# marbl/Mash

Hardware: AMD Instinct MI355X
Metric: pairwise Mash distances/sec (s=1000) (higher is better)
Workload: dtype u64; 1 GPU; mash triangle all-vs-all, 100000 clustered synthetic sketches, k=21 s=1000, 4999950000 pairs/step, per-table job (index build + discover + fill + merge each step), row-block sharded x1; parallelism=rowblock1, rccl_ranks=0

## Files before the change

mash_amd/csrc/compare_dense.hip:

```cpp
#ifdef MG_HIP_EMU
#include "hipemu.h"
#else
#include <hip/hip_runtime.h>
#define MG_DYN_SHARED(T, name)                                   \
    extern __shared__ __align__(16) unsigned char name##_raw[]; \
    T *name = reinterpret_cast<T *>(name##_raw)
#endif
#include <stdint.h>

#include <cstdlib>

#ifndef MG_HIP_EMU
#include <rocprim/device/device_radix_sort.hpp>
#include <rocprim/device/device_select.hpp>
#include <rocprim/iterator/counting_iterator.hpp>
#endif

#include "compare_internal.h"

namespace mg {

#ifndef MG_HIP_EMU
__global__ __launch_bounds__(256) void dn_neighbor_kernel(const uint64_t *hashes, uint64_t stride, const uint32_t *cnt, uint32_t n,
                                                          uint8_t *link)
{
    const uint32_t row = blockIdx.x * 4u + (threadIdx.x >> 6), lane = threadIdx.x & 63u;
    if (row >= n) return;
    uint32_t hit = 0;
    uint32_t ci = 0, cj = 0;
    if (row > 0) {
        ci = cnt[row];
        cj = cnt[row - 1];
        const uint32_t take = ci < 64u ? ci : 64u, span = cj < 256u ? cj : 256u;
        if (lane < take && span > 0) {
            const uint64_t v = hashes[(uint64_t)row * stride + lane];
            const uint64_t *q = hashes + (uint64_t)(row - 1) * stride;
            uint32_t lo = 0, hi = span;
            while (lo < hi) {
                const uint32_t mid = (lo + hi) >> 1;
                if (q[mid] < v) lo = mid + 1; else hi = mid;
            }
            hit = (lo < span && q[lo] == v) ? 1u : 0u;
        }
    }
    const uint32_t hits = (uint32_t)__popcll(__ballot(hit != 0));
    const uint32_t take = ci < 64u ? ci : 64u;
    if (lane == 0) link[row] = (row > 0 && take >= 16u && cj >= 16u && 2u * hits >= take) ? 1 : 0;
}

hipError_t launch_dense_neighbors(const uint64_t *hashes, uint64_t stride, const uint32_t *cnt, uint32_t n, uint8_t *link,
                                  hipStream_t stream)
{
    if (n == 0) return hipSuccess;
    hipLaunchKernelGGL(dn_neighbor_kernel, dim3((n + 3u) / 4u), dim3(256), 0, stream, hashes, stride, cnt, n, link);
    return hipGetLastError();
}

constexpr uint32_t DN_SUBLISTS = 1024;

__global__ __launch_bounds__(256) void dn_leaders_kernel(const uint32_t *sorted_rows, const uint32_t *gs_of, const uint32_t *gend,
                                                         const uint32_t *grp_of, const DenseGroup *groups, uint32_t E,
                                                         unsigned long long *key, uint32_t *val, uint32_t cap_sub, uint32_t *cnt)
{
    const uint32_t pos = blockIdx.x * 256u + threadIdx.x;
    bool lead = false;
    uint32_t g = 0xFFFFFFFFu, gs = 0;
    if (pos < E) {
        g = grp_of[sorted_rows[pos]];
        if (g != 0xFFFFFFFFu) {
            const uint32_t g0 = groups[g].g0, g1 = groups[g].g1;
            gs = gs_of[pos];
            const bool first = pos == gs || sorted_rows[pos - 1] < g0;
            const bool more = pos + 1u < gend[gs] && sorted_rows[pos + 1] < g1;
            lead = first && more;
        }
    }
    const uint64_t bal = __ballot(lead);
    if (bal == 0) return;
    const uint32_t lane = threadIdx.x & 63u, sub = blockIdx.x & (DN_SUBLISTS - 1u);
    uint32_t base = 0;
    if (lane == (uint32_t)__builtin_ctzll(bal)) base = atomicAdd(&cnt[sub], (uint32_t)__popcll(bal));
    base = (uint32_t)__builtin_amdgcn_readlane((int)base, __builtin_ctzll(bal));
    if (lead) {
        const uint32_t k = base + (uint32_t)__popcll(bal & ((1ull << lane) - 1ull));
        if (k < cap_sub) {
            const uint64_t slot = (uint64_t)sub * cap_sub + k;
            key[slot] = ((unsigned long long)g << 32) | gs;
            val[slot] = pos;
        }
    }
}

__global__ __launch_bounds__(DN_SUBLISTS) void dn_sublists_scan_kernel(const uint32_t *cnt, uint32_t cap_sub, uint32_t *off, uint32_t *total)
{
    __shared__ uint32_t s_w[DN_SUBLISTS / 64];
    const uint32_t t = threadIdx.x, lane = t & 63u, wid = t >> 6;
    const uint32_t want = cnt[t], c = want < cap_sub ? want : cap_sub;
    uint32_t incl = c;
#pragma unroll
    for (int d = 1; d < 64; d <<= 1) {
        const uint32_t x = __shfl_up(incl, d);
        if (lane >= (uint32_t)d) incl += x;
    }
    if (lane == 63u) s_w[wid] = incl;
    __syncthreads();
    uint32_t base = 0;
    for (uint32_t k = 0; k < wid; k++) base += s_w[k];
    off[t] = base + incl - c;
    if (t == DN_SUBLISTS - 1u) total[0] = base + incl;
    atomicMax(&total[1], want);
}

__global__ __launch_bounds__(256) void dn_sublists_copy_kernel(const unsigned long long *key, const uint32_t *val, const uint32_t *cnt,
                                                               const uint32_t *off, uint32_t cap_sub, unsigned long long *key_out,
                                                               uint32_t *val_out)
{
    const uint32_t sub = blockIdx.x;
    const uint32_t c = cnt[sub] < cap_sub ? cnt[sub] : cap_sub, o = off[sub];
    for (uint32_t k = threadIdx.x; k < c; k += 256u) {
        key_out[o + k] = key[(uint64_t)sub * cap_sub + k];
        val_out[o + k] = val[(uint64_t)sub * cap_sub + k];
    }
}

__global__ __launch_bounds__(256) void dn_universe_split_kernel(const unsigned long long *key_sorted, uint32_t m, uint32_t *ulist,
                                                                uint32_t *ustart, uint32_t *uend)
{
    const uint32_t i = blockIdx.x * 256u + threadIdx.x;
    if (i >= m) return;
    const unsigned long long k = key_sorted[i];
    const uint32_t g = (uint32_t)(k >> 32);
    ulist[i] = (uint32_t)k;
    if (i == 0 || (uint32_t)(key_sorted[i - 1] >> 32) != g) ustart[g] = i;
    if (i + 1u == m || (uint32_t)(key_sorted[i + 1] >> 32) != g) uend[g] = i + 1u;
}

size_t dense_universe_temp_bytes(uint32_t cap)
{
    size_t b = 0;
    rocprim::radix_sort_pairs(nullptr, b, (const unsigned long long *)nullptr, (unsigned long long *)nullptr, (const uint32_t *)nullptr,
                              (uint32_t *)nullptr, (size_t)cap, 0u, 64u, (hipStream_t) nullptr);
    return b;
}

uint32_t dense_sublists() { return DN_SUBLISTS; }

hipError_t dense_find_leaders(const uint32_t *sorted_rows, const uint32_t *gs_of, const uint32_t *gend, const uint32_t *grp_of,
                              const DenseGroup *groups, uint32_t E, unsigned long long *key, uint32_t *val, uint32_t cap_sub,
                              unsigned long long *key_out, uint32_t *val_out, uint32_t *cnt, uint32_t *off, uint32_t *total,
                              hipStream_t stream)
{
    if (E == 0) return hipSuccess;
    hipError_t e = hipMemsetAsync(cnt, 0, DN_SUBLISTS * 4, stream);
    if (e == hipSuccess) e = hipMemsetAsync(total, 0, 8, stream);
    if (e != hipSuccess) return e;
    hipLaunchKernelGGL(dn_leaders_kernel, dim3((E + 255u) / 256u), dim3(256), 0, stream, sorted_rows, gs_of, gend, grp_of, groups, E, key, val, cap_sub,
                       cnt);
    e = hipGetLastError();
    if (e != hipSuccess) return e;
    return dense_join_leaders(key, val, cap_sub, key_out, val_out, cnt, off, total, stream);
}

hipError_t dense_join_leaders(const unsigned long long *key, const uint32_t *val, uint32_t cap_sub, unsigned long long *key_out, uint32_t *val_out,
                              const uint32_t *cnt, uint32_t *off, uint32_t *total, hipStream_t stream)
{
    hipLaunchKernelGGL(dn_sublists_scan_kernel, dim3(1), dim3(DN_SUBLISTS), 0, stream, cnt, cap_sub, off, total);
    hipLaunchKernelGGL(dn_sublists_copy_kernel, dim3(DN_SUBLISTS), dim3(256), 0, stream, key, val, cnt, (const uint32_t *)off, cap_sub, key_out, val_out);
    return hipGetLastError();
}

hipError_t dense_sort_universes(const unsigned long long *key, const uint32_t *val, uint32_t m, void *temp, size_t temp_bytes,
                                unsigned long long *key_sorted, uint32_t *ulist, uint32_t *upos, uint32_t *ustart, uint32_t *uend,
                                uint32_t group_bits, hipStream_t stream)
{
    if (m == 0) return hipSuccess;
    hipError_t e = rocprim::radix_sort_pairs(temp, temp_bytes, key, key_sorted, val, upos, (size_t)m, 0u, 32u + group_bits, stream);
    if (e != hipSuccess) return e;
    hipLaunchKernelGGL(dn_universe_split_kernel, dim3((m + 255u) / 256u), dim3(256), 0, stream, (const unsigned long long *)key_sorted, m, ulist,
                       ustart, uend);
    return hipGetLastError();
}

#endif

constexpr uint32_t DN_CX_MASK = 0x7FFFu, DN_CX_FLAG = 0x8000u;

template <uint32_t DN_EK>
__global__ __launch_bounds__(256) void dn_encode_kernel(const uint32_t *off, const uint32_t *code_img, uint32_t *pos_img, uint32_t rs,
                                                        const uint32_t *grp_of, const DenseGroup *groups, const uint32_t *ulist,
                                                        const uint32_t *upos, unsigned long long *gdata, uint32_t wstride, uint16_t *ext,
                                                        uint32_t xs, uint32_t n, uint32_t ul_in_lds)
{
    MG_DYN_SHARED(uint32_t, lds);
    const uint32_t bid = blockIdx.x;
    const uint32_t row = (bid & ~63u) | ((bid & 7u) << 3) | ((bid >> 3) & 7u);
    const uint32_t tid = threadIdx.x, lane = tid & 63u, wid = tid >> 6;
    if (row >= n) return;
    const uint32_t g = grp_of[row];
    if (g == 0xFFFFFFFFu) return;
    const DenseGroup G = groups[g];
    const uint32_t W = G.W, u = G.u;
    uint32_t *mask32 = lds, *hist = lds + 2u * W, *gap8 = hist + W + 1u, *ovf = gap8 + 16u * W, *pl32 = ovf + W, *scr = pl32 + 8u * W;
    uint32_t *ull = lds + 28u * wstride + 9u;
    for (uint32_t i = tid; i < 28u * W + 1u; i += 256u) lds[i] = 0;
    const uint32_t *ulg = ulist + G.ustart, *up = upos + G.ustart;
    if (ul_in_lds)
        for (uint32_t i = tid; i < u; i += 256u) ull[i] = ulg[i];
    const uint32_t *ul = ul_in_lds ? ull : ulg;
    __syncthreads();
    const uint32_t cnt = off[row + 1] - off[row];
    uint16_t *xrow = ext + (uint64_t)(G.xrow0 + (row - G.g0)) * xs;
    uint32_t nx = 0;
    if constexpr (DN_EK == 1) {
        for (uint32_t base = 0; base < cnt; base += 256u) {
            const uint32_t p = base + tid;
            uint32_t idx = 0;
            bool extra = false;
            if (p < cnt) {
                const uint64_t img = (uint64_t)row * rs + p;
                const uint32_t gs = code_img[img] >> 1;
                uint32_t lo = 0, hi = u;
                while (lo < hi) {
                    const uint32_t mid = (lo + hi) >> 1;
                    if (ul[mid] < gs) lo = mid + 1; else hi = mid;
                }
                idx = lo;
                if (lo < u && ul[lo] == gs) {
                    atomicOr(&mask32[idx >> 5], 1u << (idx & 31u));
                    pos_img[img] = up[idx];
                } else {
                    extra = true;
                }
            }
            const uint64_t bal = __ballot(extra);
            const uint32_t before = (uint32_t)__popcll(bal & ((1ull << lane) - 1ull));
            if (lane == 0) scr[wid] = (uint32_t)__popcll(bal);
            __syncthreads();
            uint32_t woff = 0;
            for (uint32_t k = 0; k < wid; k++) woff += scr[k];
            const uint32_t total = scr[0] + scr[1] + scr[2] + scr[3];
            if (extra) {
                xrow[nx + woff + before] = (uint16_t)idx;
                atomicAdd(&hist[idx >> 6], 1u);
                atomicAdd(&gap8[idx >> 2], 1u << (8u * (idx & 3u)));
            }
            nx += total;
            __syncthreads();
        }
    } else {
        for (uint32_t base = 0; base < cnt; base += 256u * DN_EK) {
            const uint32_t p0 = base + tid * DN_EK;
            const uint32_t nv = p0 < cnt ? (cnt - p0 < DN_EK ? cnt - p0 : DN_EK) : 0u;
            uint32_t xidx[DN_EK];
            uint32_t nxt = 0;
            if (nv) {
                const uint64_t img0 = (uint64_t)row * rs + p0;
                const uint4 c0 = *reinterpret_cast<const uint4 *>(code_img + img0), c1 = *reinterpret_cast<const uint4 *>(code_img + img0 + 4u);
                const uint32_t code[DN_EK] = {c0.x, c0.y, c0.z, c0.w, c1.x, c1.y, c1.z, c1.w};
                uint4 *pp = reinterpret_cast<uint4 *>(pos_img + img0);
                const uint4 q0 = pp[0], q1 = pp[1];
                uint32_t pv[DN_EK] = {q0.x, q0.y, q0.z, q0.w, q1.x, q1.y, q1.z, q1.w};
                uint32_t pos = 0;
                {
                    const uint32_t gs0 = code[0] >> 1;
                    uint32_t lo = 0, hi = u;
                    while (lo < hi) {
                        const uint32_t mid = (lo + hi) >> 1;
                        if (ul[mid] < gs0) lo = mid + 1; else hi = mid;
                    }
                    pos = lo;
                }
    #pragma unroll
                for (uint32_t e = 0; e < DN_EK; e++) {
                    if (e < nv) {
                        const uint32_t gs = code[e] >> 1;
                        {
                            uint32_t lo = pos, hi = pos, step = 1;
                            while (hi < u && ul[hi] < gs) {
                                lo = hi + 1u;
                                hi += step;
                                step <<= 1;
                            }
                            hi = hi < u ? hi : u;
                            while (lo < hi) {
                                const uint32_t mid = (lo + hi) >> 1;
                                if (ul[mid] < gs) lo = mid + 1u; else hi = mid;
                            }
                            pos = lo;
                        }
                        if (pos < u && ul[pos] == gs) {
                            atomicOr(&mask32[pos >> 5], 1u << (pos & 31u));
                            pv[e] = up[pos];
                        } else {
    #pragma unroll
                            for (uint32_t j = 0; j < DN_EK; j++)
                                if (j == nxt) xidx[j] = pos;
                            nxt++;
                        }
                    }
                }
                pp[0] = make_uint4(pv[0], pv[1], pv[2], pv[3]);
                pp[1] = make_uint4(pv[4], pv[5], pv[6], pv[7]);
            }
            uint32_t incl = nxt;
    #pragma unroll
            for (uint32_t d = 1; d < 64u; d <<= 1) {
                const uint32_t y = __shfl_up(incl, d);
                if (lane >= d) incl += y;
            }
            if (lane == 63u) scr[wid] = incl;
            __syncthreads();
            uint32_t woff = 0;
            for (uint32_t k = 0; k < wid; k++) woff += scr[k];
            const uint32_t total = scr[0] + scr[1] + scr[2] + scr[3];
            const uint32_t at0 = nx + woff + incl - nxt;
    #pragma unroll
            for (uint32_t j = 0; j < DN_EK; j++) {
                if (j < nxt) {
                    const uint32_t idx = xidx[j];
                    xrow[at0 + j] = (uint16_t)idx;
                    atomicAdd(&hist[idx >> 6], 1u);
                    atomicAdd(&gap8[idx >> 2], 1u << (8u * (idx & 3u)));
                }
            }
            nx += total;
            __syncthreads();
        }
    }
    __syncthreads();
    const uint32_t jb = (row - G.g0) >> 7, bl = (row - G.g0) & 127u;
    const uint64_t bw = dense_block_words(W);
    unsigned long long *blk = gdata + G.data_off + (uint64_t)jb * bw;
    uint16_t *cxp = reinterpret_cast<uint16_t *>(blk + 128ull * W), *totp = cxp + (W + 1u) * 128u;
    unsigned long long *xpl = blk + dense_block_planes(W);
    for (uint32_t i = tid; i < 16u * W; i += 256u) {
        const uint32_t four = gap8[i], w = i >> 4, q = i & 15u;
        uint32_t bits[4] = {0u, 0u, 0u, 0u}, over = 0;
#pragma unroll
        for (uint32_t e = 0; e < 4u; e++) {
            const uint32_t c = (four >> (8u * e)) & 255u;
            over |= c >= 16u ? 1u : 0u;
#pragma unroll
            for (uint32_t j = 0; j < 4u; j++) bits[j] |= ((c >> j) & 1u) << ((4u * q + e) & 31u);
        }
        if (over || (q == 0 && hist[w] >= 256u)) ovf[w] = 1u;
#pragma unroll
        for (uint32_t j = 0; j < 4u; j++)
            if (bits[j]) atomicOr(&pl32[2u * (4u * w + j) + (q >> 3)], bits[j]);
    }
    __syncthreads();
    for (uint32_t i = tid; i < 4u * W; i += 256u) xpl[i * 128u + bl] = (unsigned long long)pl32[2u * i] | ((unsigned long long)pl32[2u * i + 1u] << 32);
    if (tid == 0) {
        uint32_t run = 0, all = 0;
        for (uint32_t w = 0; w <= W; w++) {
            cxp[w * 128u + bl] = (uint16_t)(run | ((w > 0 && ovf[w - 1u]) ? DN_CX_FLAG : 0u));
            totp[w * 128u + bl] = (uint16_t)all;
            if (w < W) {
                run += hist[w];
                all += hist[w] + (uint32_t)__popc(mask32[2u * w]) + (uint32_t)__popc(mask32[2u * w + 1u]);
            }
        }
    }
    for (uint32_t w = tid; w < W; w += 256u)
        blk[w * 128u + bl] = (unsigned long long)mask32[2u * w] | ((unsigned long long)mask32[2u * w + 1u] << 32);
}

hipError_t launch_dense_encode(const uint32_t *off, const uint32_t *code_img, uint32_t *pos_img, uint32_t rs, const uint32_t *grp_of,
                               const DenseGroup *groups, const uint32_t *ulist, const uint32_t *upos, unsigned long long *gdata,
                               uint16_t *ext, uint32_t xs, uint32_t n, uint32_t wmax, hipStream_t stream, int ul_mode)
{
    if (n == 0) return hipSuccess;
    const size_t fixed = ((size_t)28 * wmax + 9) * 4, with_ul = fixed + (size_t)wmax * 64 * 4;
    const bool ul_in_lds = ul_mode == 0 ? false : ul_mode == 1 ? with_ul <= 150 * 1024 : with_ul <= 40 * 1024;
    const size_t smem = ul_in_lds ? with_ul : fixed;
    auto go = [&](auto kern) -> hipError_t {
        hipError_t e = hipFuncSetAttribute(reinterpret_cast<const void *>(kern), hipFuncAttributeMaxDynamicSharedMemorySize, (int)smem);
        if (e != hipSuccess) return e;
        hipLaunchKernelGGL(kern, dim3((n + 63u) & ~63u), dim3(256), smem, stream, off, code_img, pos_img, rs, grp_of, groups, ulist, upos, gdata, wmax, ext, xs,
                           n, ul_in_lds ? 1u : 0u);
        return hipGetLastError();
    };
    return rs >= 4096u ? go(dn_encode_kernel<8>) : go(dn_encode_kernel<1>);
}



__device__ __forceinline__ uint32_t dn_count_add(uint32_t x, uint32_t acc)
{
#ifdef MG_HIP_EMU
    return (uint32_t)__popc(x) + acc;
#else
    uint32_t d;
    asm("v_bcnt_u32_b32 %0, %1, %2" : "=v"(d) : "v"(x), "v"(acc));
    return d;
#endif
}

__device__ __forceinline__ uint32_t dn_low_bits(uint32_t x, uint32_t y)
{
#ifdef MG_HIP_EMU
    return x & ((1u << y) - 1u);
#else
    return __builtin_amdgcn_ubfe(x, 0u, y);
#endif
}

template <uint32_t NP>
__device__ __forceinline__ uint32_t dn_descend(uint32_t base, uint32_t s, uint32_t u1, uint32_t A0, uint32_t B0, uint32_t A1, uint32_t B1,
                                               uint32_t A2, uint32_t B2, uint32_t A3, uint32_t B3)
{
    uint32_t pos = 0;
#pragma unroll
    for (uint32_t bit = 16u; bit != 0u; bit >>= 1) {
        const uint32_t y = pos + bit;
        uint32_t c = dn_count_add(dn_low_bits(B0, y), dn_count_add(dn_low_bits(A0, y), dn_count_add(dn_low_bits(u1, y), base)));
        if (NP >= 1u) c += 2u * dn_count_add(dn_low_bits(B1, y), (uint32_t)__popc(dn_low_bits(A1, y)));
        if (NP >= 3u)
            c += 4u * dn_count_add(dn_low_bits(B2, y), (uint32_t)__popc(dn_low_bits(A2, y))) +
                 8u * dn_count_add(dn_low_bits(B3, y), (uint32_t)__popc(dn_low_bits(A3, y)));
        pos = c < s ? y : pos;
    }
    return pos;
}

__device__ __forceinline__ uint32_t dn_resolve(unsigned long long un, unsigned long long mab, uint32_t fprev, uint32_t s, uint32_t w, bool lists,
                                               const unsigned long long *xpa, const unsigned long long *xpb, const uint16_t *xa,
                                               const uint16_t *xb, uint32_t ca0, uint32_t na, uint32_t cb0, uint32_t nb)
{
    if (__ballot(lists) == 0) {
        const unsigned long long a0 = xpa[512u * w], a1 = xpa[512u * w + 128u], a2 = xpa[512u * w + 256u], a3 = xpa[512u * w + 384u];
        const unsigned long long b0 = xpb[512u * w], b1 = xpb[512u * w + 128u], b2 = xpb[512u * w + 256u], b3 = xpb[512u * w + 384u];
        const bool p1 = __ballot((a1 | b1) != 0ull) != 0, p23 = __ballot((a2 | a3 | b2 | b3) != 0ull) != 0;
        const uint32_t ulo = (uint32_t)un, uhi = (uint32_t)(un >> 32);
        uint32_t c31 = dn_count_add((uint32_t)b0, dn_count_add((uint32_t)a0, dn_count_add(ulo & 0x7FFFFFFFu, fprev)));
        if (p1 || p23) c31 += 2u * dn_count_add((uint32_t)b1, (uint32_t)__popc((uint32_t)a1));
        if (p23)
            c31 += 4u * dn_count_add((uint32_t)b2, (uint32_t)__popc((uint32_t)a2)) + 8u * dn_count_add((uint32_t)b3, (uint32_t)__popc((uint32_t)a3));
        const bool upper = c31 < s;
        const uint32_t base = upper ? c31 + (ulo >> 31) : fprev;
        const uint32_t u1 = (upper ? uhi : ulo) << 1;
        const uint32_t A0 = upper ? (uint32_t)(a0 >> 32) : (uint32_t)a0, B0 = upper ? (uint32_t)(b0 >> 32) : (uint32_t)b0;
        uint32_t pos;
        if (!p1 && !p23) {
            pos = dn_descend<0>(base, s, u1, A0, B0, 0, 0, 0, 0, 0, 0);
        } else {
            const uint32_t A1 = upper ? (uint32_t)(a1 >> 32) : (uint32_t)a1, B1 = upper ? (uint32_t)(b1 >> 32) : (uint32_t)b1;
            if (!p23) {
                pos = dn_descend<1>(base, s, u1, A0, B0, A1, B1, 0, 0, 0, 0);
            } else {
                const uint32_t A2 = upper ? (uint32_t)(a2 >> 32) : (uint32_t)a2, B2 = upper ? (uint32_t)(b2 >> 32) : (uint32_t)b2;
                const uint32_t A3 = upper ? (uint32_t)(a3 >> 32) : (uint32_t)a3, B3 = upper ? (uint32_t)(b3 >> 32) : (uint32_t)b3;
                pos = dn_descend<3>(base, s, u1, A0, B0, A1, B1, A2, B2, A3, B3);
            }
        }
        const uint32_t mlo = (uint32_t)mab, mhi = (uint32_t)(mab >> 32);
        return upper ? dn_count_add(dn_low_bits(mhi, pos), (uint32_t)__popc(mlo)) : (uint32_t)__popc(dn_low_bits(mlo, pos));
    }
    uint32_t lo = 0, hi = 63;
    const uint32_t wbase = w << 6;
    while (lo < hi) {
        const uint32_t mid = (lo + hi) >> 1;
        uint32_t c = fprev + (uint32_t)__popcll(un & ((1ull << mid) - 1ull));
        for (uint32_t k = 0; k < na; k++) c += ((uint32_t)xa[ca0 + k] - wbase <= mid) ? 1u : 0u;
        for (uint32_t k = 0; k < nb; k++) c += ((uint32_t)xb[cb0 + k] - wbase <= mid) ? 1u : 0u;
        if (c >= s) hi = mid; else lo = mid + 1u;
    }
    return (uint32_t)__popcll(mab & ((1ull << lo) - 1ull));
}

template <uint32_t DN_ROWS, uint32_t DN_IL>
__global__ __launch_bounds__(128) void dn_pairs_kernel(const DenseTile *tiles, const DenseGroup *groups, const unsigned long long *gdata,
                                                       uint32_t use_lists,
                                                       const uint16_t *ext, uint32_t xs, uint32_t s, uint32_t row_begin, uint32_t row_end,
                                                       uint64_t out_base, const uint32_t *inv, uint2 *out, DenseList list)
{
    MG_DYN_SHARED(unsigned long long, dl);
    const DenseTile T = tiles[blockIdx.x];
    const DenseGroup G = groups[T.group];
    const uint32_t W = G.W, tid = threadIdx.x;
    const uint64_t bw = dense_block_words(W);
    const unsigned long long *Bm = gdata + G.data_off + (uint64_t)T.cblk * bw;
    const uint16_t *Bcx = reinterpret_cast<const uint16_t *>(Bm + 128ull * W);
    const uint16_t *Btot = Bcx + (W + 1u) * 128u;
    unsigned long long *Am = dl;
    uint16_t *Acx = reinterpret_cast<uint16_t *>(Am + (uint64_t)DN_ROWS * W);
    uint16_t *Atot = Acx + (W + 1u) * DN_ROWS;
    const uint32_t ra = T.row0 - G.g0;
    const unsigned long long *asrc = gdata + G.data_off + (uint64_t)(ra >> 7) * bw;
    const uint32_t la0 = ra & 127u;
    for (uint32_t i = tid; i < W * DN_ROWS; i += 128u) Am[i] = asrc[(i / DN_ROWS) * 128u + la0 + (i % DN_ROWS)];
    {
        const uint16_t *acs = reinterpret_cast<const uint16_t *>(asrc + 128ull * W);
        for (uint32_t i = tid; i < 2u * (W + 1u) * DN_ROWS; i += 128u) Acx[i] = acs[(i / DN_ROWS) * 128u + la0 + (i % DN_ROWS)];
    }
    __syncthreads();
    constexpr uint32_t DN_NB = DN_ROWS / DN_IL;
    uint16_t *Amax = Atot + (W + 1u) * DN_ROWS;
    for (uint32_t i = tid; i < DN_NB * (W + 1u); i += 128u) {
        const uint32_t bt = i / (W + 1u), w = i - bt * (W + 1u);
        uint32_t m = 0;
        for (uint32_t k = 0; k < DN_IL; k++)
            if (T.row0 + bt * DN_IL + k < G.g1) {
                const uint32_t v = Atot[w * DN_ROWS + bt * DN_IL + k];
                m = v > m ? v : m;
            }
        Amax[i] = (uint16_t)m;
    }
    __syncthreads();
    const uint32_t b = G.g0 + T.cblk * 128u + tid;
    const uint32_t lb = b < G.g1 ? tid : G.g1 - 1u - (G.g0 + T.cblk * 128u);
    const uint16_t *xb = ext + (uint64_t)(G.xrow0 + (b < G.g1 ? b - G.g0 : 0u)) * xs;
    const unsigned long long *xpb = Bm + dense_block_planes(W) + lb;
    const uint32_t colrow = inv ? inv[G.g0 + T.cblk * 128u + lb] : G.g0 + T.cblk * 128u + lb;
    const uint64_t tri_col = (colrow ? (uint64_t)colrow * (colrow - 1u) / 2u : 0ull) - out_base;
    for (uint32_t ai = 0; ai < DN_ROWS; ai += DN_IL) {
        if (T.row0 + ai >= G.g1 || T.row0 + ai >= row_end) break;
        const uint16_t *amax = Amax + (ai / DN_IL) * (W + 1u);
        uint32_t common[DN_IL], nle[DN_IL];
#pragma unroll
        for (uint32_t k = 0; k < DN_IL; k++) common[k] = nle[k] = 0;
        unsigned long long mb_next = Bm[lb];
        uint32_t tb_next = Btot[128u + lb];
        uint32_t wi = 0;
        for (; wi < W; wi++) {
            if (__ballot((uint32_t)amax[wi + 1u] + tb_next > s) != 0) break;
            const unsigned long long mb = mb_next;
            if (wi + 1u < W) {
                mb_next = Bm[(wi + 1u) * 128u + lb];
                tb_next = Btot[(wi + 2u) * 128u + lb];
            }
            const uint32_t mlo = (uint32_t)mb, mhi = (uint32_t)(mb >> 32);
#pragma unroll
            for (uint32_t k = 0; k < DN_IL; k++) {
                const unsigned long long am = Am[wi * DN_ROWS + ai + k];
                common[k] = dn_count_add((uint32_t)am & mlo, dn_count_add((uint32_t)(am >> 32) & mhi, common[k]));
            }
        }
        const uint32_t nfast = wi;
        for (; wi < W; wi++) {
            const unsigned long long mb = mb_next;
            const int32_t tbs = (int32_t)tb_next - (int32_t)s;
            if (wi + 1u < W) {
                mb_next = Bm[(wi + 1u) * 128u + lb];
                tb_next = Btot[(wi + 2u) * 128u + lb];
            }
            const uint32_t mlo = (uint32_t)mb, mhi = (uint32_t)(mb >> 32);
            bool any = false;
#pragma unroll
            for (uint32_t k = 0; k < DN_IL; k++) {
                const unsigned long long am = Am[wi * DN_ROWS + ai + k];
                const uint32_t cnew = dn_count_add((uint32_t)am & mlo, dn_count_add((uint32_t)(am >> 32) & mhi, common[k]));
                const bool before = (int32_t)Atot[(wi + 1u) * DN_ROWS + ai + k] + tbs <= (int32_t)cnew;
                common[k] = before ? cnew : common[k];
                nle[k] += before ? 1u : 0u;
                any = any || before;
            }
            if (__ballot(any) == 0) break;
        }
#pragma unroll
        for (uint32_t k = 0; k < DN_IL; k++) {
            const uint32_t a = T.row0 + ai + k;
            const bool present = a < G.g1 && a < row_end && a >= row_begin && G.g0 + T.cblk * 128u < a;
            if (!present) continue;
            const bool valid = b < a;
            uint32_t denom = s;
            const uint32_t w = nfast + nle[k];
            const bool need = valid && w < W;
            if (__ballot(need) != 0) {
                const uint32_t wc = need ? w : 0u;
                const unsigned long long ma = Am[wc * DN_ROWS + ai + k], mb = Bm[wc * 128u + lb];
                const uint32_t ca0 = Acx[wc * DN_ROWS + ai + k] & DN_CX_MASK, ca1r = Acx[(wc + 1u) * DN_ROWS + ai + k];
                const uint32_t cb0 = Bcx[wc * 128u + lb] & DN_CX_MASK, cb1r = Bcx[(wc + 1u) * 128u + lb];
                const uint32_t fprev = (uint32_t)Atot[wc * DN_ROWS + ai + k] + (uint32_t)Btot[wc * 128u + lb] - common[k];
                const bool lists = need && (use_lists || ((ca1r | cb1r) & DN_CX_FLAG) != 0);
                const uint32_t add = dn_resolve(ma | mb, ma & mb, fprev, s, wc, lists, asrc + dense_block_planes(W) + la0 + ai + k, xpb,
                                               ext + (uint64_t)(G.xrow0 + (a - G.g0)) * xs, xb, ca0, need ? (ca1r & DN_CX_MASK) - ca0 : 0u, cb0,
                                               need ? (cb1r & DN_CX_MASK) - cb0 : 0u);
                if (need) common[k] += add;
            }
            if (!valid) continue;
            if (w >= W) {
                const uint32_t total = (uint32_t)Atot[W * DN_ROWS + ai + k] + (uint32_t)Btot[W * 128u + lb] - common[k];
                denom = total < s ? total : s;
            }
            if (list.rc) {
                const uint32_t ra = a - list.row_first;
                const uint32_t at = list.row_base[ra] + list.row_cnt[ra] - (a - b);
                list.rc[at] = make_uint2(a, b);
                list.counts[at] = make_uint2(common[k], denom);
            } else {
                const uint32_t arow = inv ? inv[a] : a;
                const uint64_t tri_a = (uint64_t)arow * (arow - 1u) / 2u - out_base;
                out[arow > colrow ? tri_a + colrow : tri_col + arow] = make_uint2(common[k], denom);
            }
        }
    }
}

uint32_t dense_max_words() { return 400; }

size_t dense_pairs_lds(uint32_t W, uint32_t rows) { return (size_t)rows * W * 8 + (size_t)(W + 1u) * rows * 4 + (size_t)(W + 1u) * 8 * 2 + 16; }

uint32_t dense_rows_per_tile(uint64_t wave_rows) { return wave_rows / 32u >= 16384u ? 32u : 8u; }

hipError_t launch_dense_pairs(const DenseTile *tiles, uint32_t ntiles, uint32_t rows_per_tile, const DenseGroup *groups,
                              const unsigned long long *gdata, bool use_lists, const uint16_t *ext, uint32_t xs,
                              uint32_t s, uint32_t wmax, uint32_t row_begin, uint32_t row_end, uint64_t out_base, const uint32_t *inv, uint2 *out,
                              hipStream_t stream, const DenseList *list)
{
    if (ntiles == 0) return hipSuccess;
    const size_t smem = dense_pairs_lds(wmax, rows_per_tile);
    auto go = [&](auto kern) -> hipError_t {
        hipError_t e = hipFuncSetAttribute(reinterpret_cast<const void *>(kern), hipFuncAttributeMaxDynamicSharedMemorySize, (int)smem);
        if (e != hipSuccess) return e;
        hipLaunchKernelGGL(kern, dim3(ntiles), dim3(128), smem, stream, tiles, groups, gdata, use_lists ? 1u : 0u, ext, xs, s, row_begin, row_end,
                           out_base, inv, out, list ? *list : DenseList());
        return hipGetLastError();
    };
    const uint32_t il = 8;
    if (rows_per_tile == 32u) return il >= 16u ? go(dn_pairs_kernel<32, 16>) : il >= 8u ? go(dn_pairs_kernel<32, 8>) : go(dn_pairs_kernel<32, 4>);
    return il >= 8u ? go(dn_pairs_kernel<8, 8>) : go(dn_pairs_kernel<8, 4>);
}

#ifndef MG_HIP_EMU
constexpr uint32_t CL_FIRST = 4;

__global__ __launch_bounds__(256) void cl_emit_kernel(const uint64_t *hashes, uint64_t stride, const uint32_t *cnt, uint32_t n,
                                                      unsigned long long *key, uint32_t *row_out, uint32_t *label)
{
    const uint32_t i = blockIdx.x * 256u + threadIdx.x;
    if (i >= n * CL_FIRST) return;
    const uint32_t row = i / CL_FIRST, f = i % CL_FIRST;
    key[i] = f < cnt[row] ? (unsigned long long)hashes[(uint64_t)row * stride + f] : ~0ull;
    row_out[i] = row;
    if (f == 0) label[row] = row;
}

__global__ __launch_bounds__(256) void cl_minrow_kernel(const unsigned long long *key_sorted, const uint32_t *row_sorted, uint32_t m,
                                                        uint32_t *label)
{
    const uint32_t i = blockIdx.x * 256u + threadIdx.x;
    if (i >= m) return;
    const unsigned long long k = key_sorted[i];
    if (k == ~0ull) return;
    uint32_t lo = 0, hi = i;
    while (lo < hi) {
        const uint32_t mid = (lo + hi) >> 1;
        if (key_sorted[mid] < k) lo = mid + 1; else hi = mid;
    }
    atomicMin(&label[row_sorted[i]], row_sorted[lo]);
}

__global__ __launch_bounds__(256) void cl_jump_kernel(const uint32_t *in, uint32_t *out, uint32_t n)
{
    const uint32_t i = blockIdx.x * 256u + threadIdx.x;
    if (i < n) out[i] = in[in[i]];
}

__global__ __launch_bounds__(256) void cl_order_keys_kernel(const uint32_t *label, uint32_t n, uint32_t split, unsigned long long *key)
{
    const uint32_t i = blockIdx.x * 256u + threadIdx.x;
    if (i < n) key[i] = ((unsigned long long)(i >= split ? 1u : 0u) << 63) | ((unsigned long long)label[i] << 32) | i;
}

__global__ __launch_bounds__(256) void cl_split_keys_kernel(const unsigned long long *key_sorted, uint32_t n, uint32_t *inv, uint32_t *label_sorted)
{
    const uint32_t i = blockIdx.x * 256u + threadIdx.x;
    if (i < n) {
        inv[i] = (uint32_t)(key_sorted[i] & 0xFFFFFFFFull);
        label_sorted[i] = (uint32_t)(key_sorted[i] >> 32) & 0x7FFFFFFFu;
    }
}

size_t dense_cluster_temp_bytes(uint32_t n)
{
    size_t a = 0, b = 0;
    rocprim::radix_sort_pairs(nullptr, a, (const unsigned long long *)nullptr, (unsigned long long *)nullptr, (const uint32_t *)nullptr,
                              (uint32_t *)nullptr, (size_t)n * CL_FIRST, 0u, 64u, (hipStream_t) nullptr);
    rocprim::radix_sort_keys(nullptr, b, (const unsigned long long *)nullptr, (unsigned long long *)nullptr, (size_t)n, 0u, 64u,
                             (hipStream_t) nullptr);
    return a > b ? a : b;
}

hipError_t dense_cluster_rows(const uint64_t *hashes, uint64_t stride, const uint32_t *cnt, uint32_t n, void *temp, size_t temp_bytes,
                              unsigned long long *key_a, unsigned long long *key_b, uint32_t *row_a, uint32_t *row_b, uint32_t *lab_a,
                              uint32_t *lab_b, uint32_t *inv, uint32_t *label_sorted, hipStream_t stream, uint32_t split)
{
    if (n == 0) return hipSuccess;
    const uint32_t m = n * CL_FIRST;
    hipLaunchKernelGGL(cl_emit_kernel, dim3((m + 255u) / 256u), dim3(256), 0, stream, hashes, stride, cnt, n, key_a, row_a, lab_a);
    hipError_t e = hipGetLastError();
    if (e != hipSuccess) return e;
    e = rocprim::radix_sort_pairs(temp, temp_bytes, (const unsigned long long *)key_a, key_b, (const uint32_t *)row_a, row_b, (size_t)m, 0u, 64u,
                                  stream);
    if (e != hipSuccess) return e;
    hipLaunchKernelGGL(cl_minrow_kernel, dim3((m + 255u) / 256u), dim3(256), 0, stream, (const unsigned long long *)key_b, (const uint32_t *)row_b, m,
                       lab_a);
    hipLaunchKernelGGL(cl_jump_kernel, dim3((n + 255u) / 256u), dim3(256), 0, stream, (const uint32_t *)lab_a, lab_b, n);
    hipLaunchKernelGGL(cl_jump_kernel, dim3((n + 255u) / 256u), dim3(256), 0, stream, (const uint32_t *)lab_b, lab_a, n);
    hipLaunchKernelGGL(cl_order_keys_kernel, dim3((n + 255u) / 256u), dim3(256), 0, stream, (const uint32_t *)lab_a, n, split, key_a);
    e = hipGetLastError();
    if (e != hipSuccess) return e;
    e = rocprim::radix_sort_keys(temp, temp_bytes, (const unsigned long long *)key_a, key_b, (size_t)n, 0u, 64u, stream);
    if (e != hipSuccess) return e;
    hipLaunchKernelGGL(cl_split_keys_kernel, dim3((n + 255u) / 256u), dim3(256), 0, stream, (const unsigned long long *)key_b, n, inv, label_sorted);
    return hipGetLastError();
}

__global__ __launch_bounds__(256) void cl_gather_rows_kernel(const uint64_t *hashes, uint64_t stride, const uint32_t *inv, uint64_t *out)
{
    const uint32_t a = blockIdx.x;
    const uint64_t *src = hashes + (uint64_t)inv[a] * stride;
    uint64_t *dst = out + (uint64_t)a * stride;
    for (uint64_t p = threadIdx.x; p < stride; p += 256u) dst[p] = src[p];
}

hipError_t launch_dense_gather_rows(const uint64_t *hashes, uint64_t stride, const uint32_t *inv, uint32_t n, uint64_t *out, hipStream_t stream)
{
    if (n == 0) return hipSuccess;
    hipLaunchKernelGGL(cl_gather_rows_kernel, dim3(n), dim3(256), 0, stream, hashes, stride, inv, out);
    return hipGetLastError();
}

#endif

__global__ __launch_bounds__(256) void dn_group_rows_kernel(const DenseGroup *groups, uint32_t ng, uint32_t n, uint32_t *grp_of, uint4 *lead_rows)
{
    const uint32_t r = blockIdx.x * 256u + threadIdx.x;
    if (r >= n) return;
    uint32_t lo = 0, hi = ng;
    while (lo < hi) {
        const uint32_t mid = (lo + hi) >> 1;
        if (groups[mid].g0 <= r) lo = mid + 1u;
        else hi = mid;
    }
    uint32_t g = 0xFFFFFFFFu, g0 = 0, g1 = 0;
    if (lo > 0 && r < groups[lo - 1u].g1) {
        g = lo - 1u;
        g0 = groups[g].g0;
        g1 = groups[g].g1;
    }
    grp_of[r] = g;
    lead_rows[r] = make_uint4(g, g0, g1, 0u);
}

hipError_t launch_dense_group_rows(const DenseGroup *groups, uint32_t ng, uint32_t n, uint32_t *grp_of, uint32_t *lead_rows, hipStream_t stream)
{
    if (n == 0) return hipSuccess;
    hipLaunchKernelGGL(dn_group_rows_kernel, dim3((n + 255u) / 256u), dim3(256), 0, stream, groups, ng, n, grp_of, reinterpret_cast<uint4 *>(lead_rows));
    return hipGetLastError();
}

}
```

mash_amd/csrc/host_index.cpp:

```cpp
#include "host_internal.h"
#include "index_build.h"
#ifdef IX_PHASE_CLOCKS
namespace mg { void index_dump_clocks(); }
#endif
#include "sort_bits.h"

namespace {

const uint64_t kTilesLongestRun = 6144;
static const uint64_t kSplitMinRun = 128;

uint64_t longest_label_run(const uint32_t *lab_sorted, uint64_t n)
{
    if (!lab_sorted || n == 0) return 0;
    uint64_t run = 1, longest = 1;
    for (uint64_t a = 1; a < n; a++) {
        run = lab_sorted[a] == lab_sorted[a - 1] ? run + 1 : 1;
        longest = std::max(longest, run);
    }
    return longest;
}

struct Carve {
    unsigned char *base = nullptr;
    size_t at = 0;
    template <class T> T *take(size_t count)
    {
        const size_t from = (at + alignof(T) - 1) & ~(alignof(T) - 1);
        at = from + count * sizeof(T);
        return base ? reinterpret_cast<T *>(base + from) : nullptr;
    }
};

struct LeaderLists {
    DevBuf<unsigned long long> key, keyj;
    DevBuf<uint32_t> val, valj, cnt_sub, off_sub, nlead;
    uint32_t lists = mg::dense_sublists(), cap = 0, tot[2] = {0, 0};
    explicit LeaderLists(mg_ctx *c) : key(c), keyj(c), val(c), valj(c), cnt_sub(c), off_sub(c), nlead(c) {}

    hipError_t alloc(uint32_t room)
    {
        key.free(); val.free(); keyj.free(); valj.free();
        const uint64_t all = (uint64_t)lists * room;
        if (!(nlead.p && cnt_sub.p && off_sub.p) && (nlead.alloc(2) != hipSuccess || cnt_sub.alloc(lists) != hipSuccess || off_sub.alloc(lists) != hipSuccess))
            return hipErrorOutOfMemory;
        if (key.alloc(all) != hipSuccess || val.alloc(all) != hipSuccess || keyj.alloc(all) != hipSuccess || valj.alloc(all) != hipSuccess) return hipErrorOutOfMemory;
        cap = room;
        return hipSuccess;
    }
    hipError_t reset(hipStream_t st) { const hipError_t e = hipMemsetAsync(cnt_sub, 0, lists * 4, st); return e != hipSuccess ? e : hipMemsetAsync(nlead, 0, 8, st); }
    hipError_t join(hipStream_t st)
    {
        const hipError_t e = mg::dense_join_leaders(key, val, cap, keyj, valj, cnt_sub, off_sub, nlead, st);
        return e != hipSuccess ? e : hipMemcpyAsync(tot, nlead, 8, hipMemcpyDeviceToHost, st);
    }
    mg::IxLeaders view(const uint32_t *lead_rows) const { return mg::IxLeaders{lead_rows, key, val, cnt_sub, cap, lists}; }
    bool overflowed() const { return tot[1] > cap; }
};

struct SparseIndexBuild {
    mg_ctx *ctx;
    const mg_table *t;
    const uint32_t s;
    const bool clustered;
    const uint32_t split;
    mg_table::Sparse *sp;
    const uint64_t n;
    const std::chrono::steady_clock::time_point t_begin = std::chrono::steady_clock::now();
    bool stop = false;

    bool need_classes = false, dedup = true, want_dense = true, try_cluster = false, try_links = false;
    DevBuf<uint8_t> dc_cls, d_link;
    DevBuf<unsigned long long> dc_last, d_dig, d_dig_sorted, k_a, k_b;
    DevBuf<uint32_t> d_cnt, d_rows_sorted, d_flags, d_nflag, r_a, r_b, l_a, l_b, d_inv, d_lab;
    DevBuf<unsigned char> d_tmp_dup, d_tmp_cl;
    std::vector<uint8_t> hc_cls, link;
    std::vector<uint64_t> hc_last;
    std::vector<uint32_t> hc_nh, inv_v, lab_v;
    const uint32_t *inv = nullptr, *lab_sorted = nullptr;
    uint32_t nflag = 0, gate_suspects = 0;
    size_t tb_dup = 0, tb_cl = 0;
    bool cluster_q = false, links_q = false;

    const char *ix_mode = nullptr;
    bool ix_verify = false, ix_tiles = true;
    std::vector<uint32_t> cnt_true, cnt_perm;
    uint32_t max_cnt = 0;
    uint64_t maxv = 0, E_all = 0;
    double dens[65] = {0};
    double dens0 = 0;
    std::vector<uint32_t> rep;
    const uint64_t *H = nullptr;
    const uint32_t *rowmap = nullptr;
    uint64_t label_run = 0;
    mg::IxPlan early_plan;
    DevBuf<unsigned char> d_lb;
    bool lb_made = false;
    DevBuf<unsigned char> d_tcnt;
    bool cnt_made = false;
    bool cnt_stale = false;

    std::vector<uint32_t> cls_of, cls_off, cls_rows, cls_first;

    uint32_t E = 0, end_bit = 0, sort_begin_bit = 0;
    std::vector<mg::DenseGroup> cand_groups;
    std::vector<uint32_t> grp_of_h;
    DevBuf<mg::DenseGroup> d_groups;
    DevBuf<uint32_t> d_grp_of, d_lead_rows;
    LeaderLists lead;
    bool lead_ready = false, cand_prepared = false;
    mg::IxPlan plan;
    size_t temp_bytes = 0;
    DevBuf<unsigned char> temp;
    DevBuf<uint32_t> gs_of;
    DevBuf<unsigned long long> key64_a, key64_b;
    struct Stat { unsigned long long shared; uint32_t max_group, groups, bad, tie_overflow; uint32_t ixf[4]; } h_stat = {0, 0, 0, 0, 0, {0, 0, 0, 0}};
    DevBuf<Stat> d_stat;
    DevBuf<unsigned char> d_slots;
    bool want_order = true;
    std::vector<uint32_t> short_cnt;

    bool built = false;
    uint64_t dn_xrows = 0, dn_words = 0;

    SparseIndexBuild(mg_ctx *c, const mg_table *tab, uint32_t sketch_size, bool clustered_variant, mg_table::Sparse *index, uint32_t split_row)
        : ctx(c), t(tab), s(sketch_size), clustered(clustered_variant), split(split_row), sp(index), n(tab->n), dc_cls(c), d_link(c), dc_last(c), d_dig(c), d_dig_sorted(c),
          k_a(c), k_b(c), d_cnt(c), d_rows_sorted(c), d_flags(c), d_nflag(c), r_a(c), r_b(c), l_a(c), l_b(c), d_inv(c), d_lab(c), d_tmp_dup(c), d_tmp_cl(c), d_lb(c), d_tcnt(c),
          d_groups(c), d_grp_of(c), d_lead_rows(c), lead(c), temp(c), gs_of(c), key64_a(c), key64_b(c), d_stat(c), d_slots(c)
    {}

    int unusable(const char *why) { sp->usable = false; sp->why = why; stop = true; return MG_OK; }


    bool counts_with_offsets()
    {
        const char *o = ctx_opt(ctx, "MASHGPU_IX_COUNTS");
        if ((o && strcmp(o, "tiles") == 0) || !mg::index_offsets_counts_fits(early_plan.g)) return false;
        if (d_tcnt.alloc(early_plan.cnt_bytes) != hipSuccess || d_stat.alloc(1) != hipSuccess ||
            hipMemsetAsync(d_stat, 0, sizeof(Stat), ctx->stream) != hipSuccess) {
            (void)hipGetLastError();
            d_tcnt.free();
            return false;
        }
        return cnt_made = true;
    }

    hipError_t counts_to_device()
    {
            if (!cnt_stale) return hipSuccess;
            cnt_stale = false;
            return hipMemcpyAsync(d_cnt, cnt_true.data(), n * 4, hipMemcpyHostToDevice, ctx->stream);
    }

    template <class T> bool take(T **p, size_t count)
    {
        void *q = nullptr;
        if (ctx_malloc(ctx, &q, std::max<size_t>(count, 1) * sizeof(T)) != hipSuccess) return false;
        *p = static_cast<T *>(q);
        return true;
    }

    void drop()
    {
            for (void **q : {(void **)&sp->off, (void **)&sp->keys_sorted, (void **)&sp->gend, (void **)&sp->sorted_rows, (void **)&sp->code_img,
                             (void **)&sp->pos_img, (void **)&sp->short_rows, (void **)&sp->short_cnt, (void **)&sp->counters, (void **)&sp->order,
                             (void **)&sp->rep, (void **)&sp->cls_of, (void **)&sp->cls_off, (void **)&sp->cls_rows, (void **)&sp->cls_first})
                if (*q) { ctx_free(ctx, *q); *q = nullptr; }
    }

    int no_memory() { (void)hipGetLastError(); drop(); return unusable("no device memory for the index"); }
    int lost(hipError_t e) { drop(); return fail(ctx, MG_ERR_HIP, std::string("compare (index build): ") + hipGetErrorString(e)); }

    void drop_dense()
    {
        for (void **q : {(void **)&sp->dgroups, (void **)&sp->grp_of, (void **)&sp->gdata, (void **)&sp->ext, (void **)&sp->ulist, (void **)&sp->upos})
            if (*q) { ctx_free(ctx, *q); *q = nullptr; }
        sp->dgroups_host.clear();
    }

    struct TileScratch {
        DevBuf<unsigned char> start, big, pk, tc;
        explicit TileScratch(mg_ctx *c) : start(c), big(c), pk(c), tc(c) {}
    };

    hipError_t tiles(const TileScratch &w, int stages)
    {
        const mg::IxLeaders lv = lead.view(d_lead_rows);
        return mg::index_build_mapped(plan, H, rowmap, sp->off, d_lb, d_tcnt, w.start, w.big, w.pk, w.tc, sp->keys_sorted, sp->sorted_rows, sp->gend, gs_of, sp->code_img,
                               sp->pos_img, d_slots, &d_stat.p->shared, &d_stat.p->max_group, &d_stat.p->groups, d_stat.p->ixf, lead_ready ? &lv : nullptr,
                               ctx->stream, stages);
    }
    hipError_t sort_buckets(const TileScratch &w)
    {
        hipError_t e = tiles(w, 2);
        if (e == hipSuccess && lead_ready) e = lead.join(ctx->stream);
        return e != hipSuccess ? e : hipMemcpyAsync(&h_stat, d_stat, sizeof(Stat), hipMemcpyDeviceToHost, ctx->stream);
    }
    hipError_t row_order()
    {
        return mg::launch_sparse_row_order(sp->off, sp->code_img, sp->gend, sp->rep, (uint32_t)n, sp->rs, temp, temp_bytes, key64_a, key64_b, sp->order, ctx->stream);
    }

    int scan_rows();
    int copy_rows();
    int order_rows();
    int find_copies();
    int lay_out();
    void prepare_candidates();
    hipError_t tile_passes();
    int build_by_tiles();
    int build_by_sort();
    int check_build();
    bool search_leaders();
    bool sort_universes(std::vector<uint32_t> &us, std::vector<uint32_t> &ue);
    bool choose_groups(const std::vector<uint32_t> &us, const std::vector<uint32_t> &ue);
    int encode_groups();
    int dense_groups();
    int run();
};

int SparseIndexBuild::scan_rows()
{
    need_classes = t->cls.size() != n;
    dedup = !ctx_opt(ctx, "MASHGPU_SPARSE_NO_DEDUP");
    want_dense = true;
    if (const char *v = ctx_opt(ctx, "MASHGPU_COMPARE_DENSE")) want_dense = atoi(v) != 0;
    try_cluster = clustered && n >= 16;
    try_links = !try_cluster && want_dense && n >= 8 && s <= 16384;
    tb_dup = mg::sparse_dup_temp_bytes((uint32_t)n);
    tb_cl = mg::dense_cluster_temp_bytes((uint32_t)n);
    if (d_cnt.alloc(n) != hipSuccess || (need_classes && (dc_cls.alloc(n) != hipSuccess || dc_last.alloc(n) != hipSuccess)) ||
        (dedup && (d_dig.alloc(n) != hipSuccess || d_dig_sorted.alloc(n) != hipSuccess || d_rows_sorted.alloc(n) != hipSuccess ||
                   d_flags.alloc(n) != hipSuccess || d_nflag.alloc(1) != hipSuccess || d_tmp_dup.alloc(std::max<size_t>(tb_dup, 16)) != hipSuccess))) {
        (void)hipGetLastError();
        return unusable("no device memory for the index");
    }
    {
        hipError_t e = hipSuccess;
        if (need_classes) {
            hc_cls.resize(n);
            hc_last.resize(n);
            hc_nh.resize(n);
            e = mg::launch_row_classes(t->hashes, t->nhash, n, t->s, dc_cls, dc_last, ctx->stream);
        }
        if (e == hipSuccess) e = mg::launch_sparse_row_counts(t->nhash, (uint32_t)n, (uint32_t)std::min<uint64_t>(t->s, s), d_cnt, ctx->stream);
        if (e == hipSuccess && dedup) {
            e = mg::launch_sparse_row_gate(t->hashes, t->s, d_cnt, (uint32_t)n, d_dig, ctx->stream);
            if (e == hipSuccess)
                e = mg::launch_sparse_dup_suspects(d_dig, d_cnt, (uint32_t)n, d_tmp_dup, tb_dup, d_dig_sorted, d_rows_sorted, d_flags, d_nflag, ctx->stream);
        }
        if (e == hipSuccess && try_cluster) {
            if (k_a.alloc(4 * n) == hipSuccess && k_b.alloc(4 * n) == hipSuccess && r_a.alloc(4 * n) == hipSuccess && r_b.alloc(4 * n) == hipSuccess &&
                l_a.alloc(n) == hipSuccess && l_b.alloc(n) == hipSuccess && d_inv.alloc(n) == hipSuccess && d_lab.alloc(n) == hipSuccess &&
                d_tmp_cl.alloc(std::max<size_t>(tb_cl, 16)) == hipSuccess) {
                e = mg::dense_cluster_rows(t->hashes, t->s, d_cnt, (uint32_t)n, d_tmp_cl, tb_cl, k_a, k_b, r_a, r_b, l_a, l_b, d_inv, d_lab, ctx->stream, split);
                cluster_q = true;
            } else {
                (void)hipGetLastError();
            }
        }
        if (e == hipSuccess && try_links) {
            if (d_link.alloc(n) == hipSuccess) {
                link.resize(n);
                e = mg::launch_dense_neighbors(t->hashes, t->s, d_cnt, (uint32_t)n, d_link, ctx->stream);
                links_q = true;
            } else {
                (void)hipGetLastError();
            }
        }
        unsigned long long *p_last = nullptr;
        uint32_t *p_nh = nullptr, *p_inv = nullptr, *p_lab = nullptr, *p_nflag = nullptr;
        uint8_t *p_cls = nullptr, *p_link = nullptr;
        auto carve = [&](unsigned char *block) {
            Carve c{block};
            p_last = c.take<unsigned long long>(n); p_nh = c.take<uint32_t>(n); p_inv = c.take<uint32_t>(n); p_lab = c.take<uint32_t>(n);
            p_nflag = c.take<uint32_t>(2); p_cls = c.take<uint8_t>(n); p_link = c.take<uint8_t>(n);
            return c.at + 64;
        };
        unsigned char *pin = static_cast<unsigned char *>(ctx_pinned(ctx, carve(nullptr)));
        if (pin) {
            carve(pin);
        } else {
            p_nflag = &nflag;
            if (cluster_q) { inv_v.resize(n); lab_v.resize(n); p_inv = inv_v.data(); p_lab = lab_v.data(); }
            p_nh = hc_nh.data(); p_cls = hc_cls.data(); p_last = reinterpret_cast<unsigned long long *>(hc_last.data()); p_link = link.data();
        }
        if (e == hipSuccess && need_classes) {
            e = hipMemcpyAsync(p_nh, t->nhash, n * 4, hipMemcpyDeviceToHost, ctx->stream);
            if (e == hipSuccess) e = hipMemcpyAsync(p_cls, dc_cls, n, hipMemcpyDeviceToHost, ctx->stream);
            if (e == hipSuccess) e = hipMemcpyAsync(p_last, dc_last, n * 8, hipMemcpyDeviceToHost, ctx->stream);
        }
        if (e == hipSuccess && dedup) e = hipMemcpyAsync(p_nflag, d_nflag, 4, hipMemcpyDeviceToHost, ctx->stream);
        if (e == hipSuccess && cluster_q) {
            e = hipMemcpyAsync(p_inv, d_inv, n * 4, hipMemcpyDeviceToHost, ctx->stream);
            if (e == hipSuccess) e = hipMemcpyAsync(p_lab, d_lab, n * 4, hipMemcpyDeviceToHost, ctx->stream);
        }
        if (e == hipSuccess && links_q) e = hipMemcpyAsync(p_link, d_link, n, hipMemcpyDeviceToHost, ctx->stream);
        const hipError_t es = hipStreamSynchronize(ctx->stream);
        if (e == hipSuccess) e = es;
        if (e == hipSuccess && pin) {
            if (need_classes) {
                memcpy(hc_nh.data(), p_nh, n * 4);
                memcpy(hc_cls.data(), p_cls, n);
                memcpy(hc_last.data(), p_last, n * 8);
            }
            if (dedup) nflag = *p_nflag;
            if (links_q) memcpy(link.data(), p_link, n);
        }
        if (cluster_q) { inv = p_inv; lab_sorted = p_lab; }
        if (e != hipSuccess) return fail(ctx, MG_ERR_HIP, std::string("compare (index: rows, copies, order): ") + hipGetErrorString(e));
    }
    gate_suspects = nflag;
    if (need_classes) {
        t->cls.swap(hc_cls);
        t->last.swap(hc_last);
        t->nh.swap(hc_nh);
    }
    if (!links_q) link.clear();
    return MG_OK;
}

int SparseIndexBuild::order_rows()
{
    ix_mode = ctx_opt(ctx, "MASHGPU_SPARSE_INDEX");
    ix_verify = ix_mode && strcmp(ix_mode, "verify") == 0;
    ix_tiles = !ix_mode || strcmp(ix_mode, "sort") != 0;
    cnt_true.assign(n, 0);
    for (uint64_t i = 0; i < n; i++) {
        const uint32_t c = (uint32_t)std::min<uint64_t>(std::min<uint64_t>(t->nh[i], t->s), s);
        cnt_true[i] = c;
        E_all += c;
        max_cnt = std::max(max_cnt, c);
        if (c) {
            const uint64_t last = t->last[i];
            if (last == MG_HASH_PAD) return unusable("a hash equals the padding value");
            maxv = std::max(maxv, last);
            const double d = (double)c / ((double)last + 1.0);
            dens[64 - __builtin_clzll(last | 1ull)] += d;
            dens0 += d;
        }
    }
    H = t->hashes;
    bool keep_table_order = false;
    const uint64_t run = cluster_q ? longest_label_run(lab_sorted, n) : 0;
    if (cluster_q && split != 0 && lab_sorted && !ctx_opt(ctx, "MASHGPU_SPLIT_ALWAYS") && run * (uint64_t)s < kSplitMinRun * 1000ull) {
        keep_table_order = true;
        lab_sorted = nullptr;
    }
    if (cluster_q) {
        bool identity = true;
        for (uint64_t a = 0; a < n && identity; a++) identity = inv[a] == a;
        if (!identity && !keep_table_order) {
            const char *fc = ctx_opt(ctx, "MASHGPU_COMPARE_ROWCOPY");
            const bool copy_now = fc && atoi(fc) != 0;
            void *pi = nullptr, *ph = nullptr;
            if (ctx_malloc(ctx, &pi, n * 4) != hipSuccess || (copy_now && ctx_malloc(ctx, &ph, std::max<uint64_t>(n * t->s, 1) * 8) != hipSuccess)) {
                (void)hipGetLastError();
                ctx_free(ctx, pi);
                lab_sorted = nullptr;
            } else {
                sp->inv = static_cast<uint32_t *>(pi);
                sp->phashes = static_cast<uint64_t *>(ph);
                HIP_TRY(ctx, hipMemcpyAsync(sp->inv, d_inv, n * 4, hipMemcpyDeviceToDevice, ctx->stream));
                if (ix_tiles && !(dedup && nflag) && E_all > 0 && E_all < (1ull << 31) && run <= kTilesLongestRun) {
                    early_plan = mg::index_plan((uint32_t)n, (uint32_t)E_all, s, sp->rs, t->s, maxv, dens0, ix_verify);
                    if (early_plan.ok && d_lb.alloc(early_plan.lb_bytes) == hipSuccess) {
                        if (copy_now) HIP_TRY(ctx, mg::index_gather_rows(early_plan, t->hashes, sp->inv, d_cnt, sp->phashes, d_lb, ctx->stream));
                        else if (counts_with_offsets()) HIP_TRY(ctx, mg::index_offsets_counts(early_plan, t->hashes, sp->inv, d_cnt, d_lb, d_tcnt, d_stat.p->ixf, ctx->stream));
                        else HIP_TRY(ctx, mg::index_window_offsets(early_plan, t->hashes, sp->inv, d_cnt, d_lb, ctx->stream));
                        lb_made = true;
                    } else {
                        (void)hipGetLastError();
                    }
                }
                if (copy_now) {
                    if (!lb_made) HIP_TRY(ctx, mg::launch_dense_gather_rows(t->hashes, t->s, sp->inv, (uint32_t)n, sp->phashes, ctx->stream));
                    H = sp->phashes;
                } else {
                    rowmap = sp->inv;
                }
                cnt_perm.resize(n);
                for (uint64_t a = 0; a < n; a++) cnt_perm[a] = cnt_true[inv[a]];
                cnt_true.swap(cnt_perm);
                cnt_stale = true;
            }
        }
    } else {
        lab_sorted = nullptr;
    }
    label_run = lab_sorted ? run : 0;
    if (want_dense && n >= 8 && s <= 16384 && lab_sorted) {
        link.assign(n, 0);
        for (uint64_t a = 1; a < n; a++) link[a] = (a != split && lab_sorted[a] == lab_sorted[a - 1] && cnt_true[a] && cnt_true[a - 1]) ? 1 : 0;
    } else if (cluster_q && want_dense && n >= 8 && s <= 16384 && d_link.alloc(n) == hipSuccess) {
        const int rc = copy_rows();
        if (rc != MG_OK || stop) return rc;
        link.resize(n);
        HIP_TRY(ctx, counts_to_device());
        HIP_TRY(ctx, mg::launch_dense_neighbors(H, t->s, d_cnt, (uint32_t)n, d_link, ctx->stream));
        HIP_TRY(ctx, hipMemcpyAsync(link.data(), d_link, n, hipMemcpyDeviceToHost, ctx->stream));
        HIP_TRY(ctx, hipStreamSynchronize(ctx->stream));
    } else if (!links_q) {
        (void)hipGetLastError();
        link.clear();
    }
    return MG_OK;
}

int SparseIndexBuild::copy_rows()
{
    if (!rowmap) return MG_OK;
    void *ph = nullptr;
    if (ctx_malloc(ctx, &ph, std::max<uint64_t>(n * t->s, 1) * 8) != hipSuccess) return no_memory();
    sp->phashes = static_cast<uint64_t *>(ph);
    HIP_TRY(ctx, mg::launch_dense_gather_rows(t->hashes, t->s, rowmap, (uint32_t)n, sp->phashes, ctx->stream));
    H = sp->phashes;
    rowmap = nullptr;
    return MG_OK;
}

int SparseIndexBuild::find_copies()
{
    if (dedup && nflag) {
        const int rc = copy_rows();
        if (rc != MG_OK || stop) return rc;
        HIP_TRY(ctx, counts_to_device());
        HIP_TRY(ctx, mg::launch_sparse_row_digest(H, t->s, d_cnt, (uint32_t)n, d_dig, ctx->stream));
        HIP_TRY(ctx, mg::launch_sparse_dup_suspects(d_dig, d_cnt, (uint32_t)n, d_tmp_dup, tb_dup, d_dig_sorted, d_rows_sorted, d_flags, d_nflag, ctx->stream));
        HIP_TRY(ctx, hipMemcpyAsync(&nflag, d_nflag, 4, hipMemcpyDeviceToHost, ctx->stream));
        HIP_TRY(ctx, hipStreamSynchronize(ctx->stream));
        if (nflag) {
            std::vector<uint32_t> rows_sorted(n), flags(n);
            HIP_TRY(ctx, hipMemcpyAsync(rows_sorted.data(), d_rows_sorted, n * 4, hipMemcpyDeviceToHost, ctx->stream));
            HIP_TRY(ctx, hipMemcpyAsync(flags.data(), d_flags, n * 4, hipMemcpyDeviceToHost, ctx->stream));
            HIP_TRY(ctx, hipStreamSynchronize(ctx->stream));
            std::vector<uint2> pairs;
            pairs.reserve(nflag);
            for (uint64_t k = 1, g0 = 0; k < n; k++) {
                if (flags[k]) pairs.push_back(make_uint2(rows_sorted[k], rows_sorted[g0]));
                else g0 = k;
            }
            DevBuf<uint2> d_pairs(ctx);
            DevBuf<uint32_t> d_eq(ctx);
            if (d_pairs.alloc(pairs.size()) != hipSuccess || d_eq.alloc(pairs.size()) != hipSuccess) { (void)hipGetLastError(); return unusable("no device memory for the index"); }
            std::vector<uint32_t> eq(pairs.size());
            HIP_TRY(ctx, hipMemcpyAsync(d_pairs, pairs.data(), pairs.size() * sizeof(uint2), hipMemcpyHostToDevice, ctx->stream));
            HIP_TRY(ctx, mg::launch_sparse_row_equal(H, t->s, d_cnt, d_pairs, (uint32_t)pairs.size(), d_eq, ctx->stream));
            HIP_TRY(ctx, hipMemcpyAsync(eq.data(), d_eq, pairs.size() * 4, hipMemcpyDeviceToHost, ctx->stream));
            HIP_TRY(ctx, hipStreamSynchronize(ctx->stream));
            for (size_t k = 0; k < pairs.size(); k++)
                if (eq[k]) {
                    if (rep.empty()) { rep.resize(n); for (uint64_t i = 0; i < n; i++) rep[i] = (uint32_t)i; }
                    rep[pairs[k].x] = pairs[k].y;
                    sp->copies++;
                }
        }
    }
    if (sp->copies) {
        cls_of.assign(n, 0xFFFFFFFFu);
        std::vector<uint32_t> size(n, 0);
        for (uint64_t i = 0; i < n; i++) size[rep[i]]++;
        uint32_t ncls = 0, tot = 0;
        for (uint64_t i = 0; i < n; i++)
            if (size[i] >= 2) { cls_of[i] = ncls++; cls_off.push_back(tot); tot += size[i]; }
        cls_off.push_back(tot);
        cls_rows.resize(tot);
        std::vector<uint32_t> fillp(cls_off.begin(), cls_off.end() - 1);
        for (uint64_t i = 0; i < n; i++) {
            const uint32_t k = cls_of[rep[i]];
            if (k != 0xFFFFFFFFu) cls_rows[fillp[k]++] = (uint32_t)i;
        }
        cls_first.resize(tot);
        for (uint32_t k = 0; k < ncls; k++) {
            const uint64_t m = cls_off[k + 1] - cls_off[k];
            sp->cls_pairs += m * (m - 1) / 2;
            for (uint32_t u = cls_off[k]; u < cls_off[k + 1]; u++) cls_first[u] = cls_off[k];
        }
        sp->cls_members = tot;
        if (ncls == 1 && tot == n && cnt_true[0] > 0) sp->one_class = (uint32_t)cnt_true[0];
        if (sp->one_class && ctx->aside_all_copies) ctx->aside_all_copies(sp->one_class);
    }
    return MG_OK;
}

int SparseIndexBuild::lay_out()
{
    uint64_t E64 = 0;
    sp->off_host.resize(n + 1);
    for (uint64_t i = 0; i < n; i++) {
        sp->off_host[i] = (uint32_t)E64;
        const uint64_t c = cnt_true[i];
        if (rep.empty() || rep[i] == i) E64 += c;
        if (E64 >= (1ull << 31)) return unusable("2^31 entries or more");
        if (c < s) sp->short_rows_host.push_back((uint32_t)i);
        if (c == 0) sp->has_empty = true;
    }
    sp->off_host[n] = (uint32_t)E64;
    if (E64 == 0) return unusable("no hashes");
    E = (uint32_t)E64;
    sp->E = E;
    end_bit = (uint32_t)(64 - __builtin_clzll(maxv | 1ull));
    sort_begin_bit = mg::sparse_sort_begin_bit(E, end_bit, ctx_opt(ctx, "MASHGPU_SPARSE_SORT_BITS"), ctx_opt(ctx, "MASHGPU_SPARSE_SORT_ALL_BITS") != nullptr);
    if (sort_begin_bit > 0 && !ctx_opt(ctx, "MASHGPU_SPARSE_SORT_BITS")) sort_begin_bit = mg::sort_begin_bit_from_density(dens, end_bit, sort_begin_bit);
    const bool tiles_hopeless = ix_tiles && !ix_verify && lab_sorted && !ctx_opt(ctx, "MASHGPU_SPARSE_INDEX") &&
                                label_run > kTilesLongestRun;
    if (ix_tiles && !tiles_hopeless) plan = mg::index_plan((uint32_t)n, E, s, sp->rs, t->s, maxv, dens0, ix_verify);
    else if (tiles_hopeless) plan.why = "a clade of more rows than a bucket's sort takes";
    if (lb_made && !(plan.ok && memcmp(&plan.g, &early_plan.g, sizeof plan.g) == 0)) lb_made = cnt_made = false;
    temp_bytes = std::max(std::max(mg::sparse_order_temp_bytes((uint32_t)n), mg::sparse_order_slice_temp_bytes((uint32_t)n)),
                          mg::sparse_offsets_temp_bytes((uint32_t)n));
    want_order = !ctx_opt(ctx, "MASHGPU_SPARSE_NO_ORDER");
    bool ok = temp.alloc(std::max<size_t>(temp_bytes, 16)) == hipSuccess && gs_of.alloc(E) == hipSuccess && (d_stat.p || d_stat.alloc(1) == hipSuccess) &&
              d_slots.alloc(std::max(mg::sparse_stat_scratch_bytes(), mg::index_stat_scratch_bytes())) == hipSuccess &&
              (!want_order || (key64_a.alloc(n) == hipSuccess && key64_b.alloc(n) == hipSuccess));
    ok = ok && take(&sp->off, n + 1) && take(&sp->keys_sorted, E) && take(&sp->gend, E) && take(&sp->sorted_rows, E) &&
         take(&sp->code_img, (size_t)n * sp->rs + 64) && take(&sp->pos_img, (size_t)n * sp->rs) && take(&sp->counters, 4) &&
         (!want_order || take(&sp->order, n));
    const size_t nshort = sp->short_rows_host.size();
    short_cnt.assign(nshort, 0);
    for (size_t k = 0; k < nshort; k++) short_cnt[k] = cnt_true[sp->short_rows_host[k]];
    if (ok && nshort) ok = take(&sp->short_rows, nshort) && take(&sp->short_cnt, nshort);
    if (ok && sp->copies)
        ok = take(&sp->rep, n) && take(&sp->cls_of, n) && take(&sp->cls_off, cls_off.size()) && take(&sp->cls_rows, cls_rows.size()) &&
             take(&sp->cls_first, cls_first.size());
    if (!ok) return no_memory();
    hipError_t e = hipSuccess;
    auto upload = [&](uint32_t *dst, const std::vector<uint32_t> &v) {
        if (e == hipSuccess && !v.empty()) e = hipMemcpyAsync(dst, v.data(), v.size() * 4, hipMemcpyHostToDevice, ctx->stream);
    };
    if (sp->copies) { upload(sp->rep, rep); upload(sp->cls_of, cls_of); upload(sp->cls_off, cls_off); upload(sp->cls_rows, cls_rows); upload(sp->cls_first, cls_first); }
    if (!rep.empty()) upload(sp->off, sp->off_host);
    else if (e == hipSuccess) e = mg::launch_sparse_offsets(d_cnt, cnt_stale ? sp->inv : nullptr, (uint32_t)n, temp, sp->off, ctx->stream);
    upload(sp->short_rows, sp->short_rows_host); upload(sp->short_cnt, short_cnt);
    return e == hipSuccess ? MG_OK : lost(e);
}

void SparseIndexBuild::prepare_candidates()
{
    if (cand_prepared) return;
    cand_prepared = true;
    if (link.empty() || sp->copies != 0) return;
    for (uint64_t i = 1; i < n;) {
        if (!link[i]) { i++; continue; }
        uint64_t j = i;
        while (j < n && link[j]) j++;
        if (j - (i - 1) >= 8) {
            mg::DenseGroup g{};
            g.g0 = (uint32_t)(i - 1); g.g1 = (uint32_t)j;
            cand_groups.push_back(g);
        }
        i = j + 1;
    }
    if (cand_groups.empty()) return;
    const uint32_t ng = (uint32_t)cand_groups.size();
    grp_of_h.assign(n, 0xFFFFFFFFu);
    for (uint32_t g = 0; g < ng; g++)
        for (uint32_t r = cand_groups[g].g0; r < cand_groups[g].g1; r++) grp_of_h[r] = g;
    uint32_t room = std::max<uint32_t>(E / 4u / lead.lists + 64u, 256u);
    if (const char *ev = ctx_opt(ctx, "MASHGPU_DENSE_LEAD_CAP")) room = std::max<uint32_t>((uint32_t)atoi(ev), 1u);
    if (d_groups.alloc(ng) == hipSuccess && d_grp_of.alloc(n) == hipSuccess && d_lead_rows.alloc(4 * n) == hipSuccess && lead.alloc(room) == hipSuccess &&
        hipMemcpyAsync(d_groups, cand_groups.data(), ng * sizeof(mg::DenseGroup), hipMemcpyHostToDevice, ctx->stream) == hipSuccess &&
        mg::launch_dense_group_rows(d_groups, ng, (uint32_t)n, d_grp_of, d_lead_rows, ctx->stream) == hipSuccess && lead.reset(ctx->stream) == hipSuccess) {
        lead_ready = true;
    } else {
        (void)hipGetLastError();
        cand_groups.clear();
    }
}

hipError_t SparseIndexBuild::tile_passes()
{
    TileScratch w(ctx);
    if (!((lb_made || d_lb.alloc(plan.lb_bytes) == hipSuccess) && (cnt_made || d_tcnt.alloc(plan.cnt_bytes) == hipSuccess) && w.start.alloc(plan.start_bytes) == hipSuccess &&
          w.big.alloc(plan.big_bytes) == hipSuccess && w.pk.alloc(plan.pk_bytes) == hipSuccess && w.tc.alloc(plan.tc_bytes) == hipSuccess)) {
        (void)hipGetLastError();
        return hipSuccess;
    }
    hipError_t e = cnt_made ? hipSuccess : hipMemsetAsync(d_stat, 0, sizeof(Stat), ctx->stream);
    if (e == hipSuccess) e = tiles(w, cnt_made ? 1 | 8 | 16 : lb_made ? 1 | 8 : 1);
    DevBuf<uint32_t> d_swapped(ctx);
    if (e == hipSuccess && ctx_opt(ctx, "MASHGPU_IX_DEBUG_SWAP") && d_swapped.alloc(1) == hipSuccess) {
        e = hipMemsetAsync(d_swapped, 0, 4, ctx->stream);
        if (e == hipSuccess) e = mg::index_debug_swap(plan, w.pk, w.start, d_swapped, ctx->stream);
    }
    if (e == hipSuccess) prepare_candidates();
    if (e == hipSuccess && ctx->aside_at_sort) ctx->aside_at_sort();
    if (e == hipSuccess) e = sort_buckets(w);
    hipEvent_t ev_stats = nullptr;
    if (e == hipSuccess) e = hipEventCreateWithFlags(&ev_stats, hipEventDisableTiming);
    if (e == hipSuccess) e = hipEventRecord(ev_stats, ctx->stream);
    if (e == hipSuccess) e = tiles(w, 4);
    if (e == hipSuccess && want_order) e = row_order();
    const hipError_t ew = e == hipSuccess ? hipEventSynchronize(ev_stats) : hipStreamSynchronize(ctx->stream);
    if (e == hipSuccess) e = ew;
    if (ev_stats) (void)hipEventDestroy(ev_stats);
    built = e == hipSuccess && !h_stat.ixf[mg::IXF_DEGENERATE];
    if (built && lead_ready && lead.overflowed() && h_stat.ixf[mg::IXF_NBIG] == 0) {
        e = hipStreamSynchronize(ctx->stream);
        const uint32_t want_cap = lead.tot[1];
        if (e == hipSuccess && lead.alloc(want_cap) == hipSuccess) {
            e = lead.reset(ctx->stream);
            if (e == hipSuccess) e = hipMemsetAsync(d_stat.p, 0, offsetof(Stat, bad), ctx->stream);
            if (e == hipSuccess) e = sort_buckets(w);
            if (e == hipSuccess) e = hipStreamSynchronize(ctx->stream);
            built = e == hipSuccess && !h_stat.ixf[mg::IXF_DEGENERATE];
            if (ctx_opt(ctx, "MASHGPU_SPARSE_DBG"))
                fprintf(stderr, "compare dense: a list of leaders asked for %u entries: found again with that room (%u leaders)\n", want_cap, lead.tot[0]);
        } else {
            (void)hipGetLastError();
        }
    }
    if (ctx_opt(ctx, "MASHGPU_SPARSE_DBG"))
        fprintf(stderr, "compare sparse: index by tiles: shift %u, %u buckets (%u per window, %u windows), fullest %u, %u beyond the LDS (%u values streamed)%s\n",
                plan.g.shift, plan.g.Bp, plan.g.BW, plan.g.NW, h_stat.ixf[mg::IXF_MAXBUCKET], h_stat.ixf[mg::IXF_NBIG], h_stat.ixf[mg::IXF_NSTREAMED],
                h_stat.ixf[mg::IXF_DEGENERATE] ? " -- clumped values: sorted instead" : "");
    if (ctx_opt(ctx, "MASHGPU_SPARSE_DBG"))
        fprintf(stderr, "compare sparse: block counts %s\n", cnt_made ? "made with the window offsets (one read of the table)" : "by the tiles (K1)");
    return e;
}

int SparseIndexBuild::build_by_tiles()
{
    hipError_t e = hipSuccess;
    if (plan.ok) e = tile_passes();
    else if (ix_tiles && ctx_opt(ctx, "MASHGPU_SPARSE_DBG")) fprintf(stderr, "compare sparse: index by tiles refused: %s\n", plan.why);
    if (e != hipSuccess) return lost(e);
    sp->by_tiles = built;
    prepare_candidates();
#ifdef IX_PHASE_CLOCKS
    if (built && ctx_opt(ctx, "MASHGPU_IX_CLOCKS")) mg::index_dump_clocks();
#endif
    if (ix_verify && !built && !ctx_opt(ctx, "MASHGPU_SPARSE_INDEX_MAY_REFUSE"))
        return fail(ctx, MG_ERR_INVALID, std::string("index verify: the tile build refused this table (") + (plan.ok ? "bucket flags" : plan.why) + ")");
    return MG_OK;
}

int SparseIndexBuild::build_by_sort()
{
    if (built && !ix_verify) return MG_OK;
    const size_t sort_bytes = mg::sparse_sort_temp_bytes(E, end_bit, sort_begin_bit);
    DevBuf<unsigned char> temp_sort(ctx), d_ties(ctx);
    DevBuf<uint64_t> keys_a(ctx), v_keys(ctx);
    DevBuf<uint32_t> idx_a(ctx), idx_sorted(ctx), v_rows(ctx), v_gend(ctx), v_gs(ctx), v_code(ctx), v_pos(ctx);
    DevBuf<unsigned long long> d_diff(ctx);
    bool ok = temp_sort.alloc(std::max<size_t>(sort_bytes, 16)) == hipSuccess && keys_a.alloc(E) == hipSuccess && idx_a.alloc(E) == hipSuccess &&
              idx_sorted.alloc(E) == hipSuccess && d_ties.alloc(mg::sparse_tie_scratch_bytes()) == hipSuccess;
    if (ok && built)
        ok = v_keys.alloc(E) == hipSuccess && v_rows.alloc(E) == hipSuccess && v_gend.alloc(E) == hipSuccess && v_gs.alloc(E) == hipSuccess &&
             v_code.alloc((size_t)n * sp->rs + 64) == hipSuccess && v_pos.alloc((size_t)n * sp->rs) == hipSuccess && d_diff.alloc(16) == hipSuccess;
    if (!ok) return no_memory();
    const Stat tiles_stat = h_stat;
    uint64_t *o_keys = built ? v_keys.p : sp->keys_sorted;
    uint32_t *o_rows = built ? v_rows.p : sp->sorted_rows, *o_gend = built ? v_gend.p : sp->gend, *o_gs = built ? v_gs.p : gs_of.p,
             *o_code = built ? v_code.p : sp->code_img, *o_pos = built ? v_pos.p : sp->pos_img;
    hipError_t e = hipSuccess;
    for (uint32_t begin_bit = sort_begin_bit;; begin_bit = 0) {
        e = hipMemsetAsync(d_stat, 0, sizeof(Stat), ctx->stream);
        if (e == hipSuccess)
            e = mg::sparse_build_index(H, t->s, sp->off, (uint32_t)n, E, sp->rs, end_bit, temp_sort, sort_bytes, keys_a, idx_a, o_keys, idx_sorted,
                                       idx_a, o_gs, o_rows, o_gend, o_code, o_pos, d_slots, begin_bit, d_ties, &d_stat.p->shared,
                                       &d_stat.p->max_group, &d_stat.p->groups, &d_stat.p->bad, &d_stat.p->tie_overflow, ctx->stream, rowmap);
        if (e == hipSuccess && !built && want_order) e = row_order();
        if (e == hipSuccess) e = hipMemcpyAsync(&h_stat, d_stat, sizeof(Stat), hipMemcpyDeviceToHost, ctx->stream);
        if (e == hipSuccess) e = hipStreamSynchronize(ctx->stream);
        if (e != hipSuccess) return lost(e);
        if ((!h_stat.tie_overflow && !h_stat.bad) || begin_bit == 0) break;
        if (ctx_opt(ctx, "MASHGPU_SPARSE_DBG"))
            fprintf(stderr, "compare sparse: sort on bits [%u, %u) %s: every bit again\n", begin_bit, end_bit,
                    h_stat.bad ? "left values out of order" : "left ties the repair could not take");
    }
    if (!built) return MG_OK;
    unsigned long long diff[16];
    for (int k = 0; k < 8; k++) { diff[2 * k] = 0; diff[2 * k + 1] = ~0ull; }
    e = hipMemcpyAsync(d_diff, diff, sizeof diff, hipMemcpyHostToDevice, ctx->stream);
    const uint64_t img = (uint64_t)n * sp->rs;
    const struct { const char *name; const uint32_t *tiles, *sort, *ref; uint32_t mode; uint64_t words; } arrays[6] = {
        {"values (32-bit words)", (const uint32_t *)sp->keys_sorted, (const uint32_t *)v_keys.p, nullptr, 0, 2ull * E}, {"rows", sp->sorted_rows, v_rows, nullptr, 0, E},
        {"group starts", gs_of, v_gs, nullptr, 0, E}, {"group ends", sp->gend, v_gend, v_gs, 1, E}, {"code image", sp->code_img, v_code, nullptr, 0, img},
        {"position image", sp->pos_img, v_pos, v_code, 2, img}};
    for (int k = 0; k < 6 && e == hipSuccess; k++)
        e = mg::index_verify_words(arrays[k].tiles, arrays[k].sort, arrays[k].ref, arrays[k].mode, arrays[k].words, d_diff.p + 2 * k, ctx->stream);
    if (e == hipSuccess) e = hipMemcpyAsync(diff, d_diff, sizeof diff, hipMemcpyDeviceToHost, ctx->stream);
    if (e == hipSuccess) e = hipStreamSynchronize(ctx->stream);
    if (e != hipSuccess) return lost(e);
    std::string msg;
    for (int k = 0; k < 6; k++)
        if (diff[2 * k]) msg += std::string(msg.empty() ? "" : "; ") + arrays[k].name + ": " + std::to_string(diff[2 * k]) + " differ, first at " + std::to_string(diff[2 * k + 1]);
    if (h_stat.shared != tiles_stat.shared || h_stat.max_group != tiles_stat.max_group || h_stat.groups != tiles_stat.groups)
        msg += std::string(msg.empty() ? "" : "; ") + "statistics: shared " + std::to_string(tiles_stat.shared) + " / " + std::to_string(h_stat.shared) +
               ", largest group " + std::to_string(tiles_stat.max_group) + " / " + std::to_string(h_stat.max_group) + ", groups " +
               std::to_string(tiles_stat.groups) + " / " + std::to_string(h_stat.groups);
    if (!msg.empty()) {
        char geom[160];
        snprintf(geom, sizeof geom, " [n %llu, E %u, shift %u, %u buckets, %u per window, %u windows]", (unsigned long long)n, E, plan.g.shift, plan.g.Bp, plan.g.BW, plan.g.NW);
        sp->usable = false;
        return fail(ctx, MG_ERR_INVALID, "index verify: tiles / sort -- " + msg + geom);
    }
    return MG_OK;
}

int SparseIndexBuild::check_build()
{
    if (h_stat.bad) { drop(); return unusable("sort order inside a value not by row"); }
    sp->G = h_stat.groups;
    sp->shared = h_stat.shared;
    sp->max_group = h_stat.max_group;
    sp->build_ms = std::chrono::duration<double, std::milli>(std::chrono::steady_clock::now() - t_begin).count();
    sp->usable = true;
    return MG_OK;
}

bool SparseIndexBuild::search_leaders()
{
    for (int attempt = 0;; attempt++) {
        hipError_t e = mg::dense_find_leaders(sp->sorted_rows, gs_of, sp->gend, d_grp_of, d_groups, E, lead.key, lead.val, lead.cap, lead.keyj, lead.valj,
                                              lead.cnt_sub, lead.off_sub, lead.nlead, ctx->stream);
        if (e == hipSuccess) e = hipMemcpyAsync(lead.tot, lead.nlead, 8, hipMemcpyDeviceToHost, ctx->stream);
        if (e == hipSuccess) e = hipStreamSynchronize(ctx->stream);
        if (e != hipSuccess) return false;
        if (!lead.overflowed() || attempt >= 1) return true;
        if (lead.alloc(lead.tot[1]) != hipSuccess) return false;
    }
}

bool SparseIndexBuild::sort_universes(std::vector<uint32_t> &us, std::vector<uint32_t> &ue)
{
    const uint32_t ng = (uint32_t)cand_groups.size(), nlead = lead.tot[0];
    uint32_t gbits = 1;
    while ((1u << gbits) < ng) gbits++;
    const size_t tb = mg::dense_universe_temp_bytes(nlead);
    DevBuf<uint32_t> d_us(ctx), d_ue(ctx);
    DevBuf<unsigned long long> d_key2(ctx);
    DevBuf<unsigned char> d_utmp(ctx);
    bool ok = d_us.alloc(ng) == hipSuccess && d_ue.alloc(ng) == hipSuccess && d_key2.alloc(nlead) == hipSuccess && d_utmp.alloc(std::max<size_t>(tb, 16)) == hipSuccess;
    if (!ok || !take(&sp->ulist, nlead) || !take(&sp->upos, nlead)) return false;
    hipError_t e = hipMemsetAsync(d_us, 0, ng * 4, ctx->stream);
    if (e == hipSuccess) e = hipMemsetAsync(d_ue, 0, ng * 4, ctx->stream);
    if (e == hipSuccess) e = mg::dense_sort_universes(lead.keyj, lead.valj, nlead, d_utmp, tb, d_key2, sp->ulist, sp->upos, d_us, d_ue, gbits, ctx->stream);
    if (e == hipSuccess) e = hipMemcpyAsync(us.data(), d_us, ng * 4, hipMemcpyDeviceToHost, ctx->stream);
    if (e == hipSuccess) e = hipMemcpyAsync(ue.data(), d_ue, ng * 4, hipMemcpyDeviceToHost, ctx->stream);
    if (e == hipSuccess) e = hipStreamSynchronize(ctx->stream);
    return e == hipSuccess;
}

bool SparseIndexBuild::choose_groups(const std::vector<uint32_t> &us, const std::vector<uint32_t> &ue)
{
    const uint32_t kMaxWords = mg::dense_max_words();
    std::fill(grp_of_h.begin(), grp_of_h.end(), 0xFFFFFFFFu);
    for (uint32_t g = 0; g < (uint32_t)cand_groups.size(); g++) {
        mg::DenseGroup G = cand_groups[g];
        G.u = ue[g] > us[g] ? ue[g] - us[g] : 0u;
        G.ustart = us[g];
        G.W = (G.u >> 6) + 1u;
        if (G.u < 32u || G.W > kMaxWords) continue;
        G.xrow0 = (uint32_t)dn_xrows;
        G.data_off = dn_words;
        const uint64_t m = G.g1 - G.g0;
        dn_xrows += m;
        dn_words += ((m + 127) / 128) * mg::dense_block_words(G.W);
        sp->dn_wmax = std::max(sp->dn_wmax, G.W);
        for (uint32_t r = G.g0; r < G.g1; r++) grp_of_h[r] = (uint32_t)sp->dgroups_host.size();
        sp->dgroups_host.push_back(G);
    }
    return !sp->dgroups_host.empty();
}

int SparseIndexBuild::encode_groups()
{
    sp->dn_xs = ((s + 7u) & ~7u) + 8u;
    if (!take(&sp->dgroups, sp->dgroups_host.size()) || !take(&sp->grp_of, n) || !take(&sp->gdata, dn_words) || !take(&sp->ext, dn_xrows * sp->dn_xs)) {
        (void)hipGetLastError();
        sp->dgroups_host.clear();
        return MG_OK;
    }
    hipError_t e = hipMemcpyAsync(sp->dgroups, sp->dgroups_host.data(), sp->dgroups_host.size() * sizeof(mg::DenseGroup), hipMemcpyHostToDevice, ctx->stream);
    if (e == hipSuccess) e = hipMemcpyAsync(sp->grp_of, grp_of_h.data(), n * 4, hipMemcpyHostToDevice, ctx->stream);
    if (e == hipSuccess)
        e = mg::launch_dense_encode(sp->off, sp->code_img, sp->pos_img, sp->rs, sp->grp_of, sp->dgroups, sp->ulist, sp->upos, sp->gdata, sp->ext, sp->dn_xs,
                                    (uint32_t)n, sp->dn_wmax, ctx->stream, ctx_opt(ctx, "MASHGPU_DENSE_UL_LDS") ? atoi(ctx_opt(ctx, "MASHGPU_DENSE_UL_LDS")) : -1);
    sp->grp_of_host.swap(grp_of_h);
    if (e != hipSuccess) {
        drop();
        drop_dense();
        sp->usable = false;
        return fail(ctx, MG_ERR_HIP, std::string("compare (index build, dense groups): ") + hipGetErrorString(e));
    }
    sp->dn_lists = ctx_opt(ctx, "MASHGPU_DENSE_LISTS") != nullptr;
    return MG_OK;
}

int SparseIndexBuild::dense_groups()
{
    if (!cand_groups.empty()) {
        auto t_dense = std::chrono::steady_clock::now();
        if (built && lead_ready && lead.overflowed() && ctx_opt(ctx, "MASHGPU_SPARSE_DBG"))
            fprintf(stderr, "compare dense: a list of leaders asked for %u entries, room for %u: no dense groups for this table\n", lead.tot[1], lead.cap);
        std::vector<uint32_t> us(cand_groups.size(), 0), ue(cand_groups.size(), 0);
        const int rc = [&] {
            if (!lead_ready || (!built && !search_leaders())) return (int)MG_OK;
            if (lead.tot[0] == 0 || lead.overflowed()) return (int)MG_OK;
            return sort_universes(us, ue) && choose_groups(us, ue) ? encode_groups() : (int)MG_OK;
        }();
        if (rc != MG_OK) return rc;
        if (sp->dgroups_host.empty()) { (void)hipGetLastError(); drop_dense(); }
        sp->build_ms += std::chrono::duration<double, std::milli>(std::chrono::steady_clock::now() - t_dense).count();
        if (ctx_opt(ctx, "MASHGPU_SPARSE_DBG")) {
            uint64_t rows_in = 0;
            for (auto &G : sp->dgroups_host) rows_in += G.g1 - G.g0;
            fprintf(stderr, "compare dense: %zu chains of related rows, %zu groups kept (%llu rows, widest universe %u words)\n", cand_groups.size(),
                    sp->dgroups_host.size(), (unsigned long long)rows_in, sp->dn_wmax);
        }
    }
    if (ctx_opt(ctx, "MASHGPU_SPARSE_DBG")) {
        fprintf(stderr, "compare sparse: index of %llu rows (%llu copies of earlier rows), s %u: %u entries, %u distinct, shared %llu, largest run %u, %.2f ms\n",
                (unsigned long long)n, (unsigned long long)sp->copies, s, E, sp->G, (unsigned long long)sp->shared, sp->max_group, sp->build_ms);
        fprintf(stderr, "compare sparse: rows %s; the copy gate had %u suspects\n",
                !sp->inv ? "in the table's order" : sp->phashes ? "in clustered order, copied" : "in clustered order, read in place", gate_suspects);
    }
    return MG_OK;
}

int SparseIndexBuild::run()
{
    int rc = MG_OK;
    if ((rc = scan_rows()) != MG_OK || stop) return rc;
    if ((rc = order_rows()) != MG_OK || stop) return rc;
    if ((rc = find_copies()) != MG_OK || stop) return rc;
    if ((rc = lay_out()) != MG_OK || stop) return rc;
    if ((rc = build_by_tiles()) != MG_OK || stop) return rc;
    if ((rc = build_by_sort()) != MG_OK || stop) return rc;
    if ((rc = check_build()) != MG_OK || stop) return rc;
    return dense_groups();
}

}

int table_sparse_index(mg_ctx *ctx, const mg_table *t, uint32_t s, bool clustered, mg_table::Sparse **out, uint32_t split)
{
    if (!clustered) split = 0;
    for (mg_table::Sparse *sp : t->sparse)
        if (sp->s == s && sp->clustered == clustered && sp->split == split) { *out = sp; return MG_OK; }
    mg_table::Sparse *sp = new mg_table::Sparse;
    sp->s = s;
    sp->clustered = clustered;
    sp->split = split;
    t->sparse.push_back(sp);
    *out = sp;
    auto unusable = [&](const char *why) { sp->usable = false; sp->why = why; return MG_OK; };
    const uint64_t n = t->n;
    if (n == 0) return unusable("empty table");
    if (n >= (1ull << 31)) return unusable("too many rows");
    sp->rs = mg::sparse_img_stride(s);
    if (n * sp->rs >= (1ull << 32)) return unusable("image index beyond 32 bits");
    HIP_TRY(ctx, hipSetDevice(ctx->device));
    SparseIndexBuild build(ctx, t, s, clustered, sp, split);
    prof_begin(ctx, ctx->prof_index);
    struct ProfEnd { mg_ctx *c; ~ProfEnd() { prof_end(c, c->prof_index); } } prof_end_guard{ctx};
    return build.run();
}
```

mash_amd/csrc/index_build.h:

```cpp
#pragma once
#include <stdint.h>

namespace mg {

struct IxGeom {
    uint32_t n, nblk, E;
    uint32_t shift;
    uint32_t bw_log, BW;
    uint32_t NW, Bp;
    uint32_t rb;
    uint32_t npass;
    uint32_t wgrp;
    uint32_t nseq;
    uint32_t rs;
    uint32_t want_gs;
    uint64_t stride;
};

struct IxLeaders {
    const uint32_t *grp_of = nullptr;
    unsigned long long *key = nullptr;
    uint32_t *val = nullptr;
    uint32_t *cnt = nullptr;
    uint32_t cap_sub = 0, nsub = 0;
};

struct IxPlan {
    IxGeom g;
    bool ok = false;
    const char *why = "";
    size_t lb_bytes = 0, cnt_bytes = 0, start_bytes = 0, big_bytes = 0, pk_bytes = 0, tc_bytes = 0;
};

enum { IXF_NSTREAMED = 0, IXF_DEGENERATE = 1, IXF_MAXBUCKET = 2, IXF_NBIG = 3 };

IxPlan index_plan(uint32_t n, uint32_t E, uint32_t s, uint32_t rs, uint64_t stride, uint64_t maxv, double dens0, bool want_gs);
size_t index_stat_scratch_bytes();
hipError_t index_debug_swap(const IxPlan &plan, void *pk, const void *start, uint32_t *done, hipStream_t stream);
hipError_t index_build(const IxPlan &plan, const uint64_t *hashes, const uint32_t *off, void *lb, void *cnt, void *start, void *big, void *pk, void *tc,
                       uint64_t *keys_sorted, uint32_t *sorted_rows, uint32_t *gend, uint32_t *gs_of, uint32_t *code_img, uint32_t *pos_img,
                       void *stat_scratch, unsigned long long *incidences, uint32_t *max_group, uint32_t *groups, uint32_t *flags,
                       const IxLeaders *leaders, hipStream_t stream, int stages = 7);
hipError_t index_build_mapped(const IxPlan &plan, const uint64_t *hashes, const uint32_t *rowmap, const uint32_t *off, void *lb, void *cnt, void *start,
                              void *big, void *pk, void *tc, uint64_t *keys_sorted, uint32_t *sorted_rows, uint32_t *gend, uint32_t *gs_of,
                              uint32_t *code_img, uint32_t *pos_img, void *stat_scratch, unsigned long long *incidences, uint32_t *max_group,
                              uint32_t *groups, uint32_t *flags, const IxLeaders *leaders, hipStream_t stream, int stages = 7);
hipError_t index_window_offsets(const IxPlan &plan, const uint64_t *hashes, const uint32_t *rowmap, const uint32_t *cnt_table, void *lb, hipStream_t stream);
bool index_offsets_counts_fits(const IxGeom &g);
hipError_t index_offsets_counts(const IxPlan &plan, const uint64_t *hashes, const uint32_t *rowmap, const uint32_t *cnt_table, void *lb, void *cnt,
                                uint32_t *flags, hipStream_t stream);
hipError_t index_gather_rows(const IxPlan &plan, const uint64_t *hashes, const uint32_t *inv, const uint32_t *cnt_table, uint64_t *out, void *lb,
                             hipStream_t stream);

hipError_t index_verify_words(const uint32_t *a, const uint32_t *b, const uint32_t *cond, uint32_t mode, uint64_t count, unsigned long long *out2,
                              hipStream_t stream);

}
```

mash_amd/csrc/index_build.hip:

```cpp
#ifdef MG_HIP_EMU
#include "hipemu.h"
#else
#include <hip/hip_runtime.h>
#define MG_DYN_SHARED(T, name)                                   \
    extern __shared__ __align__(16) unsigned char name##_raw[]; \
    T *name = reinterpret_cast<T *>(name##_raw)
#endif
#include <stdint.h>

#include <cstdio>
#include <cstdlib>
#include <cstring>

#include "index_build.h"

#ifdef MG_HIP_EMU
#define IX_IN_LANE_ORDER(stmt)                                   \
    for (uint32_t l_ = 0; l_ < 64u; l_++) {                     \
        if ((threadIdx.x & 63u) == l_) { stmt; }                \
        hipemu::wave_sync();                                     \
    }
#else
#define IX_IN_LANE_ORDER(stmt) { stmt; }
#endif

namespace mg {

#if defined(IX_PHASE_CLOCKS) && !defined(MG_HIP_EMU)
__device__ unsigned long long ix_clk[64];
#define IX_CLK_BEGIN() unsigned long long clk_prev_ = threadIdx.x == 0 ? clock64() : 0ull
#define IX_CLK(i)                                                          \
    if (threadIdx.x == 0) {                                               \
        const unsigned long long t_ = clock64();                          \
        atomicAdd(&ix_clk[i], t_ - clk_prev_);                            \
        clk_prev_ = t_;                                                   \
    }
#else
#define IX_CLK_BEGIN() ((void)0)
#define IX_CLK(i) ((void)0)
#endif

constexpr uint32_t IX_RB = 512;
constexpr uint32_t IX_NT = 512;
constexpr uint32_t IX_M = 7;
constexpr uint32_t IX_PCAP = IX_NT * IX_M;
constexpr uint32_t IX_LPR = 8;
constexpr uint32_t IX_BW_MAX = 512;
constexpr uint32_t IX_CAP = 6144;
constexpr uint32_t IX_NT4 = 512;
constexpr uint32_t IX_SUBBITS = 13;
constexpr uint32_t IX_NSUB = 1u << IX_SUBBITS;
constexpr uint32_t IX_SUBLOW = IX_SUBBITS - 3u;
static_assert(IX_SUBBITS == 13 && IX_NT4 == 512, "the ticket slots hold 3 + 13 bits");
constexpr double IX_TMAX = 2560.0;
constexpr double IX_TILE_TARGET = 3072.0;
constexpr uint32_t IX_STAT_SLOTS = 1024;

struct IxStatSlot { unsigned long long inc; uint32_t max_group, groups; };


__device__ __forceinline__ uint32_t ix_block_scan_sum(uint32_t x, uint32_t *part, uint32_t &total)
{
    const uint32_t lane = threadIdx.x & 63u, wid = threadIdx.x >> 6, nw = blockDim.x >> 6;
    uint32_t incl = x;
#pragma unroll
    for (uint32_t d = 1; d < 64u; d <<= 1) {
        const uint32_t y = __shfl_up(incl, d);
        if (lane >= d) incl += y;
    }
    if (lane == 63u) part[wid] = incl;
    __syncthreads();
    uint32_t base = 0, tot = 0;
    for (uint32_t k = 0; k < nw; k++) {
        const uint32_t p = part[k];
        if (k < wid) base += p;
        tot += p;
    }
    __syncthreads();
    total = tot;
    return base + incl - x;
}

__device__ __forceinline__ uint32_t ix_block_scan_max(uint32_t x, uint32_t *part)
{
    const uint32_t lane = threadIdx.x & 63u, wid = threadIdx.x >> 6;
    uint32_t incl = x;
#pragma unroll
    for (uint32_t d = 1; d < 64u; d <<= 1) {
        const uint32_t y = __shfl_up(incl, d);
        if (lane >= d && y > incl) incl = y;
    }
    if (lane == 63u) part[wid] = incl;
    __syncthreads();
    uint32_t base = 0;
    for (uint32_t k = 0; k < wid; k++) base = part[k] > base ? part[k] : base;
    __syncthreads();
    const uint32_t before = __shfl_up(incl, 1u);
    uint32_t ex = lane > 0 ? before : 0u;
    return ex > base ? ex : base;
}

__device__ __forceinline__ bool ix_tile_id(const IxGeom &g, uint32_t &blk, uint32_t &w)
{
    const uint32_t per = gridDim.x >> 3;
    const uint32_t q = (blockIdx.x & 7u) * per + (blockIdx.x >> 3);
    if (q >= g.nseq) return false;
    const uint32_t gsz = g.nblk * g.wgrp;
    const uint32_t wg = q / gsz, rem = q - wg * gsz;
    blk = rem / g.wgrp;
    w = wg * g.wgrp + (rem - blk * g.wgrp);
    return w < g.NW;
}

__global__ __launch_bounds__(256) void ix_gather_offsets_kernel(IxGeom g, const uint64_t *__restrict__ H, const uint32_t *__restrict__ inv,
                                                                const uint32_t *__restrict__ cnt_table, uint64_t *__restrict__ out,
                                                                uint16_t *__restrict__ lb)
{
    const uint32_t a = blockIdx.x, tid = threadIdx.x;
    const uint32_t r = inv[a];
    const uint32_t cnt = cnt_table[r];
    const uint64_t *src = H + (uint64_t)r * g.stride;
    uint64_t *dst = out + (uint64_t)a * g.stride;
    uint16_t *o = lb + (uint64_t)a * (g.NW + 1u);
    const uint32_t wsh = g.shift + g.bw_log;
    for (uint64_t p = tid; p < g.stride; p += 256u) {
        const uint64_t v = src[p];
        dst[p] = v;
        if (p < cnt) {
            const int w = (int)(uint32_t)(v >> wsh);
            const int wp = p > 0 ? (int)(uint32_t)(src[p - 1] >> wsh) : -1;
            for (int x = wp + 1; x <= w; x++) o[x] = (uint16_t)p;
        }
    }
    const int wl = cnt > 0 ? (int)(uint32_t)(src[cnt - 1] >> wsh) : -1;
    for (uint32_t x = (uint32_t)(wl + 1) + tid; x <= g.NW; x += 256u) o[x] = (uint16_t)cnt;
}

__global__ __launch_bounds__(256) void ix_window_offsets_kernel(IxGeom g, const uint64_t *H, const uint32_t *rowmap, const uint32_t *off,
                                                                const uint32_t *cnt_table, uint16_t *lb)
{
    const uint32_t row = blockIdx.x * 4u + (threadIdx.x >> 6), lane = threadIdx.x & 63u;
    if (row < g.n) {
        const uint32_t trow = rowmap ? rowmap[row] : row;
        const uint32_t cnt = cnt_table ? cnt_table[trow] : off[row + 1] - off[row];
        const uint64_t *src = H + (uint64_t)trow * g.stride;
        uint16_t *out = lb + (uint64_t)row * (g.NW + 1u);
        const uint32_t wsh = g.shift + g.bw_log;
        for (uint32_t p = lane; p < cnt; p += 64u) {
            const int w = (int)(uint32_t)(src[p] >> wsh);
            const int wp = p > 0 ? (int)(uint32_t)(src[p - 1] >> wsh) : -1;
            for (int x = wp + 1; x <= w; x++) out[x] = (uint16_t)p;
        }
        const int wl = cnt > 0 ? (int)(uint32_t)(src[cnt - 1] >> wsh) : -1;
        for (uint32_t x = (uint32_t)(wl + 1) + lane; x <= g.NW; x += 64u) out[x] = (uint16_t)cnt;
    }
}

constexpr uint32_t IX_ROUNDS = IX_RB / (IX_NT / IX_LPR);

__global__ __launch_bounds__(IX_NT) void ix_tile_count_kernel(IxGeom g, const uint64_t *__restrict__ H, const uint32_t *__restrict__ rowmap,
                                                              const uint16_t *__restrict__ lb, uint32_t *__restrict__ cnt)
{
    __shared__ uint32_t s_hist[IX_BW_MAX];
    uint32_t blk = 0, w = 0;
    if (!ix_tile_id(g, blk, w)) return;
    const uint32_t tid = threadIdx.x, sub = tid % IX_LPR;
    const uint32_t row0 = blk * IX_RB, nrows = g.n - row0 < IX_RB ? g.n - row0 : IX_RB;
    if (tid < g.BW) s_hist[tid] = 0;
    uint32_t lo[IX_ROUNDS], hi[IX_ROUNDS], tr[IX_ROUNDS];
    const uint32_t trow0 = rowmap ? rowmap[row0] : row0;
#pragma unroll
    for (uint32_t it = 0; it < IX_ROUNDS; it++) {
        const uint32_t r = it * (IX_NT / IX_LPR) + tid / IX_LPR, rc = r < nrows ? r : 0u;
        const uint16_t *p = lb + (uint64_t)(row0 + rc) * (g.NW + 1u) + w;
        const uint32_t a = p[0], b = p[1];
        tr[it] = rowmap ? rowmap[row0 + rc] : row0 + rc;
        lo[it] = a;
        hi[it] = r < nrows ? b : a;
    }
    uint64_t v[IX_ROUNDS];
#pragma unroll
    for (uint32_t it = 0; it < IX_ROUNDS; it++) {
        const bool in = lo[it] + sub < hi[it];
        v[it] = H[in ? (uint64_t)tr[it] * g.stride + lo[it] + sub : (uint64_t)trow0 * g.stride];
    }
    __syncthreads();
#pragma unroll
    for (uint32_t it = 0; it < IX_ROUNDS; it++) {
        if (lo[it] + sub < hi[it]) {
            atomicAdd(&s_hist[(uint32_t)(v[it] >> g.shift) & (g.BW - 1u)], 1u);
            const uint64_t *src = H + (uint64_t)tr[it] * g.stride;
            for (uint32_t k = lo[it] + sub + IX_LPR; k < hi[it]; k += IX_LPR) atomicAdd(&s_hist[(uint32_t)(src[k] >> g.shift) & (g.BW - 1u)], 1u);
        }
    }
    __syncthreads();
    if (tid < g.BW) cnt[(uint64_t)blk * g.Bp + (uint64_t)w * g.BW + tid] = s_hist[tid];
}

constexpr uint32_t IXOC_NT = 1024;
constexpr uint32_t IXOC_UN = 16;
constexpr uint32_t IXOC_SCRATCH = 64;
constexpr uint32_t IXOC_LDS_MAX = 160u * 1024u;
static_assert(IXOC_LDS_MAX <= 160u * 1024u, "a CU of gfx950 has 160 KB of LDS: the counters of one workgroup must fit it");
static_assert(IX_RB % (IXOC_NT / 64u) == 0, "every wave takes the same number of rows of a full block");

__host__ __device__ inline uint32_t ixoc_words(uint32_t Bp) { return (Bp + 1u) >> 1; }
__host__ __device__ inline uint64_t ixoc_lds_bytes(uint32_t Bp) { return (uint64_t)ixoc_words(Bp) * 4u + IXOC_SCRATCH; }

template <uint32_t MODE>
__device__ __forceinline__ uint32_t ixoc_stream_rows(const IxGeom &g, const uint64_t *__restrict__ H, const uint32_t *__restrict__ rowmap,
                                                     const uint32_t *__restrict__ cnt_table, uint16_t *__restrict__ lb, uint32_t *s_w, uint32_t row0,
                                                     uint32_t nrows)
{
    const uint32_t lane = threadIdx.x & 63u, wave = threadIdx.x >> 6, nw = blockDim.x >> 6;
    const uint32_t wsh = g.shift + g.bw_log;
    uint32_t entries = 0;
    if (wave >= nrows) return 0;
    auto table_row = [&](uint32_t r) -> uint32_t { return rowmap ? rowmap[row0 + r] : row0 + r; };
    uint32_t trow = table_row(wave);
    uint32_t trow_n = table_row(wave + nw < nrows ? wave + nw : wave);
    uint32_t cnt = cnt_table[trow];
    for (uint32_t r = wave; r < nrows; r += nw) {
        const uint32_t cnt_n = cnt_table[trow_n];
        const uint32_t trow_nn = table_row(r + 2u * nw < nrows ? r + 2u * nw : r);
        const uint64_t *src = H + (uint64_t)trow * g.stride;
        uint16_t *out = lb + (uint64_t)(row0 + r) * (g.NW + 1u);
        entries += cnt;
        int wlast = -1;
        for (uint32_t p0 = 0; p0 < cnt; p0 += 64u * IXOC_UN) {
            uint64_t v[IXOC_UN];
#pragma unroll
            for (uint32_t u = 0; u < IXOC_UN; u++) {
                const uint32_t p = p0 + 64u * u + lane;
                v[u] = src[p < cnt ? p : 0u];
            }
#pragma unroll
            for (uint32_t u = 0; u < IXOC_UN; u++) {
                const uint32_t c0 = p0 + 64u * u, p = c0 + lane;
                const int w = (int)(uint32_t)(v[u] >> wsh);
                int wp = __shfl_up(w, 1u);
                if (lane == 0) wp = wlast;
                const int wl = __shfl(w, cnt - 1u - c0 < 64u ? cnt - 1u - c0 : 63u);
                if (c0 < cnt) wlast = wl;
                if (p < cnt) {
                    if (MODE == 0)
                        for (int x = wp + 1; x <= w; x++) out[x] = (uint16_t)p;
                    const uint32_t b = (uint32_t)(v[u] >> g.shift);
                    if (b < g.Bp) {
                        if (MODE == 0) atomicAdd(&s_w[b >> 1], 1u << (16u * (b & 1u)));
                        else if ((b & 1u) == MODE - 1u) atomicAdd(&s_w[b >> 1], 1u);
                    }
                }
            }
        }
        if (MODE == 0)
            for (uint32_t x = (uint32_t)(wlast + 1) + lane; x <= g.NW; x += 64u) out[x] = (uint16_t)cnt;
        trow = trow_n;
        trow_n = trow_nn;
        cnt = cnt_n;
    }
    return entries;
}

__global__ __launch_bounds__(IXOC_NT) void ix_offsets_counts_kernel(IxGeom g, const uint64_t *__restrict__ H, const uint32_t *__restrict__ rowmap,
                                                                    const uint32_t *__restrict__ cnt_table, uint16_t *__restrict__ lb,
                                                                    uint32_t *__restrict__ cnt, uint32_t *flags)
{
    MG_DYN_SHARED(uint32_t, s_w);
    const uint32_t nwords = ixoc_words(g.Bp);
    uint32_t *s_part = s_w + nwords;
    const uint32_t tid = threadIdx.x, blk = blockIdx.x;
    const uint32_t row0 = blk * IX_RB, nrows = g.n - row0 < IX_RB ? g.n - row0 : IX_RB;
    uint32_t *o = cnt + (uint64_t)blk * g.Bp;
    for (uint32_t x = tid; x < nwords; x += IXOC_NT) s_w[x] = 0;
    __syncthreads();
    const uint32_t mine = ixoc_stream_rows<0>(g, H, rowmap, cnt_table, lb, s_w, row0, nrows);
    __syncthreads();
    uint32_t sum = 0;
    for (uint32_t x = tid; x < nwords; x += IXOC_NT) sum += (s_w[x] & 0xFFFFu) + (s_w[x] >> 16);
    uint32_t counted = 0, entries = 0;
    (void)ix_block_scan_sum(sum, s_part, counted);
    (void)ix_block_scan_sum((tid & 63u) == 0 ? mine : 0u, s_part, entries);
    if (counted == entries) {
        for (uint32_t b = tid; b < g.Bp; b += IXOC_NT) o[b] = (s_w[b >> 1] >> (16u * (b & 1u))) & 0xFFFFu;
        return;
    }
    if (tid == 0) flags[IXF_DEGENERATE] = 1u;
    for (uint32_t half = 0; half < 2u; half++) {
        __syncthreads();
        for (uint32_t x = tid; x < nwords; x += IXOC_NT) s_w[x] = 0;
        __syncthreads();
        if (half == 0) (void)ixoc_stream_rows<1>(g, H, rowmap, cnt_table, lb, s_w, row0, nrows);
        else (void)ixoc_stream_rows<2>(g, H, rowmap, cnt_table, lb, s_w, row0, nrows);
        __syncthreads();
        for (uint32_t b = half + 2u * tid; b < g.Bp; b += 2u * IXOC_NT) o[b] = s_w[b >> 1];
    }
}

__global__ __launch_bounds__(256) void ix_col_scan_kernel(IxGeom g, uint32_t *cnt, uint32_t *tot)
{
    const uint32_t b = blockIdx.x * 256u + threadIdx.x;
    if (b < g.Bp) {
        uint32_t run = 0;
        for (uint32_t blk0 = 0; blk0 < g.nblk; blk0 += 16u) {
            uint32_t c[16];
#pragma unroll
            for (uint32_t k = 0; k < 16u; k++) c[k] = blk0 + k < g.nblk ? cnt[(uint64_t)(blk0 + k) * g.Bp + b] : 0u;
#pragma unroll
            for (uint32_t k = 0; k < 16u; k++)
                if (blk0 + k < g.nblk) {
                    cnt[(uint64_t)(blk0 + k) * g.Bp + b] = run;
                    run += c[k];
                }
        }
        tot[b] = run;
    }
}

__global__ __launch_bounds__(1024) void ix_bucket_scan_kernel(IxGeom g, uint32_t *start, uint32_t *flags, uint32_t *biglist)
{
    __shared__ uint32_t s_part[16], s_max[16];
    const uint32_t tid = threadIdx.x;
    uint32_t carry = 0, mx = 0;
    for (uint32_t base = 0; base < g.Bp; base += 4096u) {
        const uint32_t b = base + 4u * tid;
        uint32_t c[4], sum = 0;
#pragma unroll
        for (uint32_t k = 0; k < 4u; k++) {
            c[k] = b + k < g.Bp ? start[b + k] : 0u;
            sum += c[k];
            mx = c[k] > mx ? c[k] : mx;
            if (c[k] > IX_CAP) biglist[atomicAdd(&flags[IXF_NBIG], 1u)] = b + k;
        }
        uint32_t total = 0;
        uint32_t run = carry + ix_block_scan_sum(sum, s_part, total);
#pragma unroll
        for (uint32_t k = 0; k < 4u; k++) {
            if (b + k < g.Bp) start[b + k] = run;
            run += c[k];
        }
        carry += total;
    }
    if (tid == 0) start[g.Bp] = carry;
#pragma unroll
    for (uint32_t d = 32; d > 0; d >>= 1) {
        const uint32_t o = __shfl_xor(mx, d);
        mx = o > mx ? o : mx;
    }
    if ((tid & 63u) == 0) s_max[tid >> 6] = mx;
    __syncthreads();
    if (tid == 0) {
        uint32_t m = 0;
        for (uint32_t k = 0; k < 16u; k++) m = s_max[k] > m ? s_max[k] : m;
        flags[IXF_MAXBUCKET] = m;
    }
}

__device__ __forceinline__ uint32_t *ix_tile_sort(uint32_t *src, uint32_t *dst, uint16_t *cnt, uint32_t *part, uint32_t np, uint32_t npass)
{
    const uint32_t tid = threadIdx.x, i0 = tid * IX_M;
    for (uint32_t pass = 0; pass < npass; pass++) {
        const uint32_t sh = 12u + 4u * pass;
#pragma unroll
        for (uint32_t d = 0; d < 16u; d++) cnt[d * IX_NT + tid] = 0;
        uint32_t e[IX_M];
#pragma unroll
        for (uint32_t k = 0; k < IX_M; k++) {
            e[k] = i0 + k < np ? src[i0 + k] : 0xFFFFFFFFu;
            if (i0 + k < np) cnt[((e[k] >> sh) & 15u) * IX_NT + tid]++;
        }
        __syncthreads();
        uint32_t c16[16], sum = 0;
#pragma unroll
        for (uint32_t x = 0; x < 16u; x++) {
            c16[x] = cnt[16u * tid + x];
            sum += c16[x];
        }
        uint32_t total = 0;
        uint32_t run = ix_block_scan_sum(sum, part, total);
#pragma unroll
        for (uint32_t x = 0; x < 16u; x++) {
            cnt[16u * tid + x] = (uint16_t)run;
            run += c16[x];
        }
        __syncthreads();
#pragma unroll
        for (uint32_t k = 0; k < IX_M; k++)
            if (i0 + k < np) {
                uint16_t *c = &cnt[((e[k] >> sh) & 15u) * IX_NT + tid];
                dst[*c] = e[k];
                *c = (uint16_t)(*c + 1u);
            }
        __syncthreads();
        uint32_t *t = src;
        src = dst;
        dst = t;
    }
    return src;
}

constexpr uint32_t IXL_PACK = 0, IXL_PA = IXL_PACK + IX_PCAP * 8u, IXL_PB = IXL_PA + IX_PCAP * 4u, IXL_CNT = IXL_PB + IX_PCAP * 4u,
                   IXL_ROWPRE = IXL_CNT + 16u * IX_NT * 2u, IXL_LO = IXL_ROWPRE + (IX_RB + 2u) * 4u, IXL_HIST = IXL_LO + IX_RB * 2u,
                   IXL_GBASE = IXL_HIST + (IX_BW_MAX + 2u) * 4u, IXL_PART = IXL_GBASE + IX_BW_MAX * 4u, IXL_BYTES = IXL_PART + 64u;

__global__ __launch_bounds__(IX_NT, 4) void ix_tile_partition_kernel(IxGeom g, const uint64_t *__restrict__ H, const uint32_t *__restrict__ rowmap,
                                                                  const uint16_t *__restrict__ lb,
                                                                  const uint32_t *__restrict__ colpre, const uint32_t *__restrict__ start,
                                                                  const uint32_t *__restrict__ flags, uint64_t *__restrict__ pk,
                                                                  uint32_t *__restrict__ slot_img)
{
    MG_DYN_SHARED(unsigned char, lds);
    uint64_t *s_pack = reinterpret_cast<uint64_t *>(lds + IXL_PACK);
    uint32_t *s_pa = reinterpret_cast<uint32_t *>(lds + IXL_PA), *s_pb = reinterpret_cast<uint32_t *>(lds + IXL_PB);
    uint16_t *s_cnt = reinterpret_cast<uint16_t *>(lds + IXL_CNT);
    uint32_t *s_rowpre = reinterpret_cast<uint32_t *>(lds + IXL_ROWPRE);
    uint16_t *s_lo = reinterpret_cast<uint16_t *>(lds + IXL_LO);
    uint32_t *s_hist = reinterpret_cast<uint32_t *>(lds + IXL_HIST);
    uint32_t *s_gbase = reinterpret_cast<uint32_t *>(lds + IXL_GBASE);
    uint32_t *s_part = reinterpret_cast<uint32_t *>(lds + IXL_PART);
    uint32_t *s_trow = reinterpret_cast<uint32_t *>(lds + IXL_CNT);
    static_assert(IX_RB * 4u <= 16u * IX_NT * 2u && IX_RB == IX_NT, "the block's row map fits the sort's counters, a row per work-item");
    uint32_t blk = 0, w = 0;
    if (!ix_tile_id(g, blk, w)) return;
    const uint32_t tid = threadIdx.x, sub = tid % IX_LPR;
    IX_CLK_BEGIN();
    const uint32_t row0 = blk * IX_RB, nrows = g.n - row0 < IX_RB ? g.n - row0 : IX_RB;
    uint32_t len = 0, gb = 0, trow = 0;
    if (tid < g.BW) {
        const uint32_t bg = w * g.BW + tid;
        gb = start[bg] + colpre[(uint64_t)blk * g.Bp + bg];
    }
    if (tid < nrows) {
        trow = rowmap ? rowmap[row0 + tid] : row0 + tid;
        const uint16_t *p = lb + (uint64_t)(row0 + tid) * (g.NW + 1u) + w;
        const uint32_t lo = p[0];
        len = (uint32_t)p[1] - lo;
        s_lo[tid] = (uint16_t)lo;
    }
    uint32_t total = 0;
    const uint32_t pre = ix_block_scan_sum(len, s_part, total);
    if (total == 0) return;
    s_rowpre[tid] = pre;
    s_trow[tid] = trow;
    if (tid == IX_NT - 1u) s_rowpre[IX_NT] = total;
    if (tid < g.BW) {
        s_gbase[tid] = gb;
        s_hist[tid] = 0;
    }
    __syncthreads();
    IX_CLK(0);
    const uint64_t lowmask = (1ull << g.shift) - 1ull;
    for (uint32_t i0 = 0; i0 < total; i0 += IX_PCAP) {
        const uint32_t np = total - i0 < IX_PCAP ? total - i0 : IX_PCAP;
        uint32_t at[IX_ROUNDS];
        uint64_t v[IX_ROUNDS];
#pragma unroll
        for (uint32_t it = 0; it < IX_ROUNDS; it++) {
            const uint32_t r = it * (IX_NT / IX_LPR) + tid / IX_LPR, rc = r < nrows ? r : 0u;
            const uint32_t rp = s_rowpre[rc], ln = r < nrows ? s_rowpre[rc + 1u] - rp : 0u;
            const uint32_t i = rp + sub;
            const bool in = sub < ln && i >= i0 && i < i0 + np;
            at[it] = in ? i - i0 : 0xFFFFFFFFu;
            v[it] = H[in ? (uint64_t)s_trow[rc] * g.stride + s_lo[rc] + sub : (uint64_t)s_trow[0] * g.stride];
        }
#pragma unroll
        for (uint32_t it = 0; it < IX_ROUNDS; it++) {
            const uint32_t r = it * (IX_NT / IX_LPR) + tid / IX_LPR;
            if (at[it] != 0xFFFFFFFFu) {
                const uint32_t bl = (uint32_t)(v[it] >> g.shift) & (g.BW - 1u);
                atomicAdd(&s_hist[bl], 1u);
                s_pack[at[it]] = ((v[it] & lowmask) << g.rb) | (uint64_t)(row0 + r);
                s_pa[at[it]] = (bl << 12) | at[it];
            }
        }
#pragma unroll 1
        for (uint32_t r = tid / IX_LPR; r < nrows; r += IX_NT / IX_LPR) {
            const uint32_t rp = s_rowpre[r], ln = s_rowpre[r + 1u] - rp;
            if (ln <= IX_LPR || rp + ln <= i0 || rp >= i0 + np) continue;
            const uint64_t *src = H + (uint64_t)s_trow[r] * g.stride + s_lo[r];
            for (uint32_t k = sub + IX_LPR; k < ln; k += IX_LPR) {
                const uint32_t i = rp + k;
                if (i < i0 || i >= i0 + np) continue;
                const uint64_t x = src[k];
                const uint32_t bl = (uint32_t)(x >> g.shift) & (g.BW - 1u);
                atomicAdd(&s_hist[bl], 1u);
                s_pack[i - i0] = ((x & lowmask) << g.rb) | (uint64_t)(row0 + r);
                s_pa[i - i0] = (bl << 12) | (i - i0);
            }
        }
        __syncthreads();
        IX_CLK(1);
        uint32_t *srt = ix_tile_sort(s_pa, s_pb, s_cnt, s_part, np, g.npass);
        IX_CLK(2);
        uint32_t *s_slot = srt == s_pa ? s_pb : s_pa;
        {
            const uint32_t c = tid < g.BW ? s_hist[tid] : 0u;
            uint32_t tot = 0;
            const uint32_t ex = ix_block_scan_sum(c, s_part, tot);
            if (tid < g.BW) s_hist[tid] = ex;
            if (tid == 0) s_hist[g.BW] = np;
        }
        __syncthreads();
        IX_CLK(3);
        for (uint32_t j = tid; j < np; j += IX_NT) {
            const uint32_t e = srt[j], b = e >> 12, idx = e & 4095u;
            const uint32_t slot = s_gbase[b] + (j - s_hist[b]);
            pk[slot] = s_pack[idx];
            s_slot[idx] = slot;
        }
        __syncthreads();
        IX_CLK(4);
        {
            uint32_t sl[IX_ROUNDS], lo8[IX_ROUNDS];
#pragma unroll
            for (uint32_t it = 0; it < IX_ROUNDS; it++) {
                const uint32_t r = it * (IX_NT / IX_LPR) + tid / IX_LPR;
                sl[it] = s_slot[at[it] != 0xFFFFFFFFu ? at[it] : 0u];
                lo8[it] = s_lo[r < nrows ? r : 0u];
            }
#pragma unroll
            for (uint32_t it = 0; it < IX_ROUNDS; it++) {
                const uint32_t r = it * (IX_NT / IX_LPR) + tid / IX_LPR;
                if (at[it] != 0xFFFFFFFFu) slot_img[(uint64_t)(row0 + r) * g.rs + lo8[it] + sub] = sl[it];
            }
        }
#pragma unroll 1
        for (uint32_t r = tid / IX_LPR; r < nrows; r += IX_NT / IX_LPR) {
            const uint32_t rp = s_rowpre[r], ln = s_rowpre[r + 1u] - rp;
            if (ln <= IX_LPR || rp + ln <= i0 || rp >= i0 + np) continue;
            const uint64_t at0 = (uint64_t)(row0 + r) * g.rs + s_lo[r];
            for (uint32_t k = sub + IX_LPR; k < ln; k += IX_LPR) {
                const uint32_t i = rp + k;
                if (i >= i0 && i < i0 + np) slot_img[at0 + k] = s_slot[i - i0];
            }
        }
        IX_CLK(5);
        uint32_t add = 0;
        if (tid < g.BW) add = s_hist[tid + 1] - s_hist[tid];
        __syncthreads();
        if (tid < g.BW) {
            s_gbase[tid] += add;
            s_hist[tid] = 0;
        }
        s_trow[tid] = trow;
        __syncthreads();
    }
}

constexpr uint32_t IX5_CH = 32;
constexpr uint32_t IX5_UNR = 4;

__global__ __launch_bounds__(256) void ix_images_kernel(IxGeom g, const uint32_t *__restrict__ off, const uint32_t *__restrict__ flags,
                                                        const uint2 *__restrict__ tc, uint32_t *__restrict__ code_img, uint32_t *pos_img, uint32_t nchunk)
{
    const uint32_t per = gridDim.x >> 3;
    const uint32_t q = (blockIdx.x & 7u) * per + (blockIdx.x >> 3);
    if (q >= g.nblk * nchunk) return;
    const uint32_t blk = q / nchunk, ch = q - blk * nchunk;
    const uint32_t tid = threadIdx.x, quad = tid & 7u, rsub = tid >> 3;
    const uint32_t p0 = ch * IX5_CH + quad * 4u;
    const uint32_t row0 = blk * IX_RB, nrows = g.n - row0 < IX_RB ? g.n - row0 : IX_RB;
    uint32_t cnt_n[IX5_UNR];
    uint32_t sl_n[IX5_UNR][4];
    auto slots = [&](uint32_t rb) {
#pragma unroll
        for (uint32_t u = 0; u < IX5_UNR; u++) {
            const uint32_t r = rb + 32u * u;
            const uint32_t row = row0 + (r < nrows ? r : 0u);
            const uint32_t c = r < nrows ? off[row + 1u] - off[row] : 0u;
            cnt_n[u] = c;
            const uint32_t *src = pos_img + (uint64_t)row * g.rs + (p0 < c ? p0 : 0u);
            sl_n[u][0] = src[0];
            sl_n[u][1] = src[1];
            sl_n[u][2] = src[2];
            sl_n[u][3] = src[3];
        }
    };
    if (rsub < nrows) slots(rsub);
    for (uint32_t rb = rsub; rb < nrows; rb += 32u * IX5_UNR) {
        uint32_t cnt[IX5_UNR];
        uint32_t sl[IX5_UNR][4];
#pragma unroll
        for (uint32_t u = 0; u < IX5_UNR; u++) {
            cnt[u] = cnt_n[u];
#pragma unroll
            for (uint32_t e = 0; e < 4u; e++) sl[u][e] = sl_n[u][e];
        }
        uint2 cp[IX5_UNR][4];
#pragma unroll
        for (uint32_t u = 0; u < IX5_UNR; u++)
#pragma unroll
            for (uint32_t e = 0; e < 4u; e++) cp[u][e] = tc[p0 + e < cnt[u] ? sl[u][e] : 0u];
        if (rb + 32u * IX5_UNR < nrows) slots(rb + 32u * IX5_UNR);
#pragma unroll
        for (uint32_t u = 0; u < IX5_UNR; u++) {
            const uint32_t r = rb + 32u * u;
            if (r < nrows && p0 < g.rs) {
                const uint64_t at = (uint64_t)(row0 + r) * g.rs + p0;
#pragma unroll
                for (uint32_t e = 0; e < 4u; e++) {
                    code_img[at + e] = p0 + e < cnt[u] ? cp[u][e].x : 0xFFFFFFFFu;
                    if (p0 + e < cnt[u]) pos_img[at + e] = cp[u][e].y;
                }
            }
        }
    }
}

__device__ __forceinline__ uint32_t ix_subshift(const IxGeom &g) { return g.shift >= IX_SUBBITS ? g.shift + g.rb - IX_SUBBITS : g.rb; }

constexpr uint32_t IX4_PK = 0, IX4_JX = IX4_PK + IX_CAP * 8u, IX4_H = IX4_JX + IX_CAP * 2u, IX4_MIX = IX4_H + IX_NSUB * 2u,
                   IX4_PART = IX4_MIX + IX_NSUB / 8u, IX4_BYTES = IX4_PART + 64u;

template <bool PART> struct IxBodyPtr { using In = const uint64_t *__restrict__; using Keys = uint64_t *__restrict__; using Rows = uint32_t *__restrict__; };
template <> struct IxBodyPtr<true> { using In = const uint64_t *; using Keys = uint64_t *; using Rows = uint32_t *; };

template <uint32_t PER, bool PART>
__device__ __forceinline__ bool ix_bucket_sort_body(const IxGeom &g, typename IxBodyPtr<PART>::In src, const uint32_t *arr, uint32_t tcbase, uint32_t subshift,
                                                    typename IxBodyPtr<PART>::Keys keys_sorted, typename IxBodyPtr<PART>::Rows sorted_rows, uint32_t *__restrict__ gend,
                                                    uint32_t *__restrict__ gs_of, uint2 *__restrict__ tc, IxStatSlot *stat, uint32_t *flags,
                                                    const IxLeaders &lead, uint64_t *s_pk, uint16_t *s_jx, uint32_t *s_h, uint32_t *s_mixed,
                                                    uint32_t *s_part, uint32_t b, uint32_t G0, uint32_t N)
{
    const uint32_t tid = threadIdx.x, lane = tid & 63u, wave = tid >> 6;
    IX_CLK_BEGIN();
    for (uint32_t x = tid; x < IX_NSUB / 2u; x += IX_NT4) s_h[x] = 0;
    if (tid < IX_NSUB / 32u) s_mixed[tid] = 0;
    uint64_t v[PER];
    uint32_t sa[PER];
    uint32_t am[PART ? PER : 1u];
#pragma unroll
    for (uint32_t k = 0; k < PER; k++) {
        const uint32_t j = tid + k * IX_NT4;
        const bool in = j < N;
        const uint64_t x = src[in ? j : 0u];
        v[k] = x;
        if constexpr (PART) am[k] = arr[in ? j : 0u];
        const uint32_t sub0 = (uint32_t)(x >> subshift) & (IX_NSUB - 1u);
        if (in) s_jx[j] = (uint16_t)(((sub0 >> IX_SUBLOW) << 13) | (sub0 & ((1u << IX_SUBLOW) - 1u)));
    }
    __syncthreads();
    IX_CLK(32);
    uint16_t *s_tk = s_jx;
    for (uint32_t j0 = 0; j0 < N; j0 += 256u) {
        uint32_t tag[4];
#pragma unroll
        for (uint32_t u = 0; u < 4u; u++) {
            const uint32_t j = j0 + 64u * u + lane;
            tag[u] = j < N ? (uint32_t)s_tk[j] : 0xFFFFu;
        }
        uint32_t old[4];
#pragma unroll
        for (uint32_t u = 0; u < 4u; u++) {
            const uint32_t j = j0 + 64u * u + lane;
            const bool mine = (tag[u] >> 13) == wave && j < N;
            const uint32_t sub = (wave << IX_SUBLOW) | (tag[u] & ((1u << IX_SUBLOW) - 1u));
            const uint32_t h16 = (sub & 1u) * 16u;
            uint32_t o = 0;
            IX_IN_LANE_ORDER(if (mine) o = atomicAdd(&s_h[sub >> 1], 1u << h16));
            old[u] = (o >> h16) & 0xFFFFu;
        }
#pragma unroll
        for (uint32_t u = 0; u < 4u; u++) {
            const uint32_t j = j0 + 64u * u + lane;
            if ((tag[u] >> 13) == wave && j < N) s_tk[j] = (uint16_t)((wave << 13) | old[u]);
        }
    }
    __syncthreads();
    IX_CLK(33);
    {
        uint32_t wv[8], sum = 0;
#pragma unroll
        for (uint32_t x = 0; x < 8u; x++) {
            wv[x] = s_h[8u * tid + x];
            sum += (wv[x] & 0xFFFFu) + (wv[x] >> 16);
        }
        uint32_t total = 0;
        uint32_t run = ix_block_scan_sum(sum, s_part, total);
#pragma unroll
        for (uint32_t x = 0; x < 8u; x++) {
            const uint32_t lo = wv[x] & 0xFFFFu, hi = wv[x] >> 16;
            s_h[8u * tid + x] = run | ((run + lo) << 16);
            run += lo + hi;
        }
    }
    const uint16_t *cs = reinterpret_cast<const uint16_t *>(s_h);
#pragma unroll
    for (uint32_t k = 0; k < PER; k++) {
        const uint32_t j = tid + k * IX_NT4;
        sa[k] = (uint32_t)s_tk[j < N ? j : 0u] & 0x1FFFu;
    }
    __syncthreads();
    IX_CLK(34);
#pragma unroll
    for (uint32_t k = 0; k < PER; k++) {
        const uint32_t j = tid + k * IX_NT4;
        if (j < N) {
            const uint32_t sub = (uint32_t)(v[k] >> subshift) & (IX_NSUB - 1u);
            const uint32_t q = (uint32_t)cs[sub] + sa[k];
            s_pk[q] = v[k];
            s_jx[q] = (uint16_t)j;
        }
    }
    __syncthreads();
    IX_CLK(35);
    {
        uint32_t diff = 0;
#pragma unroll
        for (uint32_t k = 0; k < PER; k++) {
            const uint32_t q = tid + k * IX_NT4;
            const uint64_t me = s_pk[q < N ? q : 0u];
            const uint32_t sub = (uint32_t)(me >> subshift) & (IX_NSUB - 1u);
            if (q < N && (s_pk[cs[sub]] >> g.rb) != (me >> g.rb)) diff |= 1u << k;
        }
        if (diff) {
#pragma unroll
            for (uint32_t k = 0; k < PER; k++)
                if ((diff >> k) & 1u) {
                    const uint32_t sub = (uint32_t)(s_pk[tid + k * IX_NT4] >> subshift) & (IX_NSUB - 1u);
                    atomicOr(&s_mixed[sub >> 5], 1u << (sub & 31u));
                }
        }
    }
    __syncthreads();
#pragma unroll
    for (uint32_t k = 0; k < PER; k++) {
        const uint32_t q = tid + k * IX_NT4;
        const bool in = q < N;
        const uint32_t qc = in ? q : 0u;
        const uint64_t me = s_pk[qc];
        const uint32_t jv = s_jx[qc];
        const uint32_t sub = (uint32_t)(me >> subshift) & (IX_NSUB - 1u);
        uint32_t nq = qc;
        if (in && ((s_mixed[sub >> 5] >> (sub & 31u)) & 1u)) {
            const uint32_t a = cs[sub], e = sub + 1u < IX_NSUB ? (uint32_t)cs[sub + 1u] : N;
            {
                uint32_t r = 0;
                if (subshift - g.rb <= 32u) {
                    const uint32_t low = (uint32_t)(me >> g.rb);
                    for (uint32_t x = a; x < e; x++) {
                        const uint32_t lx = (uint32_t)(s_pk[x] >> g.rb);
                        r += (lx < low || (lx == low && x < qc)) ? 1u : 0u;
                    }
                } else {
                    const uint64_t low = me >> g.rb;
                    for (uint32_t x = a; x < e; x++) {
                        const uint64_t lx = s_pk[x] >> g.rb;
                        r += (lx < low || (lx == low && x < qc)) ? 1u : 0u;
                    }
                }
                nq = a + r;
            }
        }
        v[k] = me;
        sa[k] = nq | (jv << 16);
    }
    __syncthreads();
#pragma unroll
    for (uint32_t k = 0; k < PER; k++) {
        const uint32_t q = tid + k * IX_NT4;
        if (q < N) {
            s_pk[sa[k] & 0xFFFFu] = v[k];
            s_jx[sa[k] & 0xFFFFu] = (uint16_t)(sa[k] >> 16);
        }
    }
    __syncthreads();
    IX_CLK(36);
    uint16_t *inv = reinterpret_cast<uint16_t *>(s_h);
    unsigned long long *s_hb = reinterpret_cast<unsigned long long *>(s_mixed);
    int unordered = 0;
#pragma unroll
    for (uint32_t k = 0; k < PER; k++) {
        const uint32_t q = tid + k * IX_NT4;
        const bool in = q < N;
        const uint32_t qc = in ? q : 0u;
        const uint64_t w = s_pk[qc], prev = s_pk[qc > 0 ? qc - 1u : 0u];
        const bool head = in && (q == 0 || (w >> g.rb) != (prev >> g.rb));
        if (in && q > 0 && w <= prev) unordered = 1;
        if (in) inv[s_jx[q]] = (uint16_t)q;
        const unsigned long long bal = __ballot(head);
        if (lane == 0 && q < N) s_hb[q >> 6] = bal;
    }
    unordered = __syncthreads_or(unordered);
    if (unordered) {
        if (tid == 0) flags[IXF_DEGENERATE] = 1u;
        return false;
    }
    IX_CLK(37);
    auto group_start = [&](uint32_t q) -> uint32_t {
        uint32_t w = q >> 6;
        unsigned long long m = s_hb[w] & (~0ull >> (63u - (q & 63u)));
        while (m == 0) m = s_hb[--w];
        return (w << 6) + 63u - (uint32_t)__builtin_clzll(m);
    };
    auto is_head = [&](uint32_t q) -> bool { return (s_hb[q >> 6] >> (q & 63u)) & 1ull; };
    const uint64_t rowmask = (1ull << g.rb) - 1ull;
    const uint64_t vbase = (uint64_t)b << g.shift;
    unsigned long long inc = 0;
    uint32_t heads = 0, glen = 0, lmask = 0;
    uint32_t gsr[PER], grpr[PER], g0r[PER], g1r[PER];
#pragma unroll
    for (uint32_t k = 0; k < PER; k++) {
        const uint32_t q = tid + k * IX_NT4;
        const bool in = q < N;
        const uint32_t qc = in ? q : 0u;
        const uint32_t gs = group_start(qc);
        const bool last = qc + 1u == N || is_head(qc + 1u);
        gsr[k] = gs;
        const bool look = lead.grp_of != nullptr && in && !(last && qc == gs);
        const uint32_t *gp = lead.grp_of + 4ull * (uint32_t)(s_pk[qc] & rowmask);
        grpr[k] = look ? gp[0] : 0xFFFFFFFFu;
        g0r[k] = look ? gp[1] : 0u;
        g1r[k] = look ? gp[2] : 0u;
        inc += in ? q - gs : 0u;
        heads += (in && q == gs) ? 1u : 0u;
        const uint32_t len = (in && last) ? q + 1u - gs : 0u;
        glen = len > glen ? len : glen;
    }
#pragma unroll
    for (uint32_t k = 0; k < PER; k++) {
        const uint32_t q = tid + k * IX_NT4;
        if (q < N) {
            const uint64_t w = s_pk[q];
            const uint32_t gs = gsr[k];
            const bool last = q + 1u == N || is_head(q + 1u);
            keys_sorted[G0 + q] = vbase | (w >> g.rb);
            sorted_rows[G0 + q] = (uint32_t)(w & rowmask);
            if (gs_of) gs_of[G0 + q] = G0 + gs;
            if (last) gend[G0 + gs] = G0 + q + 1u;
            if (grpr[k] != 0xFFFFFFFFu) {
                const bool first = q == gs || (uint32_t)(s_pk[q - 1u] & rowmask) < g0r[k];
                const bool more = !last && (uint32_t)(s_pk[q + 1u] & rowmask) < g1r[k];
                if (first && more) lmask |= 1u << k;
            }
        }
    }
    IX_CLK(38);
#pragma unroll
    for (uint32_t d = 32; d > 0; d >>= 1) {
        inc += __shfl_xor(inc, d);
        heads += __shfl_xor(heads, d);
        const uint32_t o = __shfl_xor(glen, d);
        glen = o > glen ? o : glen;
    }
    __shared__ unsigned long long s_inc[IX_NT4 / 64];
    __shared__ uint32_t s_len[IX_NT4 / 64], s_heads[IX_NT4 / 64];
    if (lane == 0) {
        s_inc[wave] = inc;
        s_len[wave] = glen;
        s_heads[wave] = heads;
    }
    uint32_t ltotal = 0, lbase = 0;
    if (lead.grp_of) lbase = ix_block_scan_sum((uint32_t)__popc(lmask), s_part, ltotal);
    else __syncthreads();
    if (tid == 0) {
        if (ltotal) s_part[15] = atomicAdd(&lead.cnt[b & (lead.nsub - 1u)], ltotal);
        unsigned long long t = 0;
        uint32_t m = 0, h = 0;
        for (uint32_t k = 0; k < IX_NT4 / 64u; k++) {
            t += s_inc[k];
            m = s_len[k] > m ? s_len[k] : m;
            h += s_heads[k];
        }
        IxStatSlot *sl = stat + (b & (IX_STAT_SLOTS - 1u));
        if (t) atomicAdd(&sl->inc, t);
        if (m > 1u) atomicMax(&sl->max_group, m);
        atomicAdd(&sl->groups, h);
    }
    IX_CLK(39);
#pragma unroll
    for (uint32_t k = 0; k < PER; k++) {
        const uint32_t j = tid + k * IX_NT4;
        if (j < N) {
            const uint32_t q = inv[j], gs = group_start(q);
            const bool last = q + 1u == N || is_head(q + 1u);
            const uint32_t shared = (gs == q && last) ? 0u : 1u;
            uint32_t at = j;
            if constexpr (PART) at = am[k];
            tc[tcbase + at] = make_uint2(((G0 + gs) << 1) | shared, G0 + q);
        }
    }
    IX_CLK(40);
    if (ltotal) {
        __syncthreads();
        const uint32_t sub = b & (lead.nsub - 1u);
        uint32_t at = s_part[15] + lbase;
#pragma unroll
        for (uint32_t k = 0; k < PER; k++) {
            if ((lmask >> k) & 1u) {
                const uint32_t q = tid + k * IX_NT4;
                if (at < lead.cap_sub) {
                    const uint64_t slot = (uint64_t)sub * lead.cap_sub + at;
                    lead.key[slot] = ((unsigned long long)grpr[k] << 32) | (unsigned long long)(G0 + gsr[k]);
                    lead.val[slot] = G0 + q;
                }
                at++;
            }
        }
    }
    IX_CLK(41);
    return true;
}

__global__ __launch_bounds__(IX_NT4, 4) void ix_bucket_sort_kernel(IxGeom g, const uint64_t *pk, const uint32_t *start, uint64_t *keys_sorted,
                                                                uint32_t *sorted_rows, uint32_t *gend, uint32_t *gs_of, uint2 *tc,
                                                                IxStatSlot *stat, uint32_t *flags, IxLeaders lead)
{
    MG_DYN_SHARED(unsigned char, lds);
    uint64_t *s_pk = reinterpret_cast<uint64_t *>(lds + IX4_PK);
    uint16_t *s_jx = reinterpret_cast<uint16_t *>(lds + IX4_JX);
    uint32_t *s_h = reinterpret_cast<uint32_t *>(lds + IX4_H);
    uint32_t *s_mixed = reinterpret_cast<uint32_t *>(lds + IX4_MIX);
    uint32_t *s_part = reinterpret_cast<uint32_t *>(lds + IX4_PART);
    const uint32_t b = blockIdx.x;
    const uint32_t G0 = start[b], N = start[b + 1] - G0;
    if (N == 0 || N > IX_CAP) return;
    const uint32_t per = (N + IX_NT4 - 1u) / IX_NT4;
    const uint32_t subshift = ix_subshift(g);
#define IX_BODY(P)                                                                                                                          \
    (void)ix_bucket_sort_body<P, false>(g, pk + G0, nullptr, G0, subshift, keys_sorted, sorted_rows, gend, gs_of, tc, stat, flags, lead, s_pk, s_jx, \
                                        s_h, s_mixed, s_part, b, G0, N)
    if (per <= 3u) IX_BODY(3);
    else if (per <= 4u) IX_BODY(4);
    else if (per <= 5u) IX_BODY(5);
    else if (per <= 6u) IX_BODY(6);
    else if (per <= 8u) IX_BODY(8);
    else IX_BODY(12);
#undef IX_BODY
}

constexpr uint32_t IXB_CS1 = IX4_BYTES, IXB_CS2 = IXB_CS1 + IX_NSUB * 4u, IXB_BYTES = IXB_CS2 + IX_NSUB * 4u;
constexpr uint32_t IXB_CH = 4096;
constexpr uint32_t IXB_W = 0, IXB_ARR = IXB_W + IXB_CH * 8u, IXB_TAG = IXB_ARR + IXB_CH * 4u;
static_assert(IXB_TAG + IXB_CH * 2u <= IX4_H, "the staging area lies in the body's entry arrays");

struct IxOut {
    uint64_t *keys_sorted;
    uint32_t *sorted_rows, *gend, *gs_of;
    uint2 *tc;
    IxStatSlot *stat;
    uint32_t *flags;
};

__device__ __forceinline__ uint32_t ix_big_first(const uint32_t *cs, uint32_t k) { return k ? cs[k - 1u] : 0u; }

__device__ __forceinline__ void ix_big_split(const uint64_t *src_w, const uint32_t *src_arr, uint64_t *dst_w, uint32_t *dst_arr, uint32_t count,
                                             uint32_t sshift, uint32_t *cs, unsigned char *lds, uint32_t *s_part)
{
    uint64_t *s_w = reinterpret_cast<uint64_t *>(lds + IXB_W);
    uint32_t *s_arr = reinterpret_cast<uint32_t *>(lds + IXB_ARR);
    uint16_t *s_tag = reinterpret_cast<uint16_t *>(lds + IXB_TAG);
    const uint32_t tid = threadIdx.x, lane = tid & 63u, wave = tid >> 6;
    for (uint32_t x = tid; x < IX_NSUB; x += IX_NT4) cs[x] = 0;
    __syncthreads();
    for (uint32_t j = tid; j < count; j += IX_NT4) atomicAdd(&cs[(uint32_t)(src_w[j] >> sshift) & (IX_NSUB - 1u)], 1u);
    __syncthreads();
    {
        constexpr uint32_t W = IX_NSUB / IX_NT4;
        uint32_t c[W], sum = 0;
#pragma unroll
        for (uint32_t x = 0; x < W; x++) {
            c[x] = cs[W * tid + x];
            sum += c[x];
        }
        uint32_t total = 0;
        uint32_t run = ix_block_scan_sum(sum, s_part, total);
#pragma unroll
        for (uint32_t x = 0; x < W; x++) {
            cs[W * tid + x] = run;
            run += c[x];
        }
    }
    for (uint32_t j0 = 0; j0 < count; j0 += IXB_CH) {
        __syncthreads();
        for (uint32_t x = tid; x < IXB_CH; x += IX_NT4) {
            const uint32_t j = j0 + x, jc = j < count ? j : 0u;
            const uint64_t w = src_w[jc];
            const uint32_t sub0 = (uint32_t)(w >> sshift) & (IX_NSUB - 1u);
            s_w[x] = w;
            s_arr[x] = src_arr ? src_arr[jc] : j;
            s_tag[x] = (uint16_t)(((sub0 >> IX_SUBLOW) << 13) | (sub0 & ((1u << IX_SUBLOW) - 1u)));
        }
        __syncthreads();
        const uint32_t xe = count - j0 < IXB_CH ? count - j0 : IXB_CH;
        for (uint32_t x0 = 0; x0 < xe; x0 += 256u) {
            uint32_t tag[4];
#pragma unroll
            for (uint32_t u = 0; u < 4u; u++) tag[u] = s_tag[x0 + 64u * u + lane];
#pragma unroll
            for (uint32_t u = 0; u < 4u; u++) {
                const uint32_t x = x0 + 64u * u + lane;
                const bool mine = (tag[u] >> 13) == wave && x < xe;
                const uint32_t sub = (wave << IX_SUBLOW) | (tag[u] & ((1u << IX_SUBLOW) - 1u));
                uint32_t at = 0;
                IX_IN_LANE_ORDER(if (mine) at = atomicAdd(&cs[sub], 1u));
                if (mine) {
                    dst_w[at] = s_w[x];
                    dst_arr[at] = s_arr[x];
                }
            }
        }
    }
    __threadfence();
    __syncthreads();
}

__device__ __forceinline__ bool ix_big_one_value(const IxGeom &g, const uint64_t *src_w, uint32_t m)
{
    const uint64_t low0 = src_w[0] >> g.rb;
    int bad = 0;
    for (uint32_t q = threadIdx.x; q < m; q += IX_NT4) bad |= (src_w[q] >> g.rb) != low0 ? 1 : 0;
    return __syncthreads_or(bad) == 0;
}

__device__ __forceinline__ bool ix_big_value(const IxGeom &g, const uint64_t *src_w, const uint32_t *src_arr, const IxOut &o, const IxLeaders &lead,
                                             uint32_t *s_row, uint32_t *s_part, uint32_t b, uint32_t tcbase, uint32_t gs, uint32_t m)
{
    const uint32_t tid = threadIdx.x;
    const uint64_t rowmask = (1ull << g.rb) - 1ull;
    const uint64_t vbase = (uint64_t)b << g.shift;
    int bad = 0;
    for (uint32_t q0 = 0; q0 < m; q0 += IX_NT4) {
        const uint32_t q = q0 + tid;
        const bool in = q < m, more_after = q + 1u < m;
        const uint64_t w = src_w[in ? q : 0u];
        const uint32_t ar = src_arr[in ? q : 0u];
        const uint32_t next_row = (uint32_t)(src_w[more_after ? q + 1u : 0u] & rowmask);
        const uint32_t row = (uint32_t)(w & rowmask);
        s_row[tid + 1u] = row;
        __syncthreads();
        const uint32_t prev_row = s_row[tid];
        if (in && q > 0 && prev_row >= row) bad = 1;
        bool isl = false;
        uint32_t grp = 0xFFFFFFFFu;
        if (lead.grp_of != nullptr && in) {
            const uint32_t *gp = lead.grp_of + 4ull * row;
            grp = gp[0];
            const bool first = q == 0 || prev_row < gp[1];
            isl = grp != 0xFFFFFFFFu && first && more_after && next_row < gp[2];
        }
        __syncthreads();
        if (tid == IX_NT4 - 1u) s_row[0] = row;
        if (in) {
            o.keys_sorted[gs + q] = vbase | (w >> g.rb);
            o.sorted_rows[gs + q] = row;
            if (o.gs_of) o.gs_of[gs + q] = gs;
            o.tc[tcbase + ar] = make_uint2((gs << 1) | 1u, gs + q);
        }
        if (lead.grp_of != nullptr) {
            uint32_t ltotal = 0;
            const uint32_t lbase = ix_block_scan_sum(isl ? 1u : 0u, s_part, ltotal);
            if (ltotal) {
                const uint32_t sub = b & (lead.nsub - 1u);
                if (tid == 0) s_part[15] = atomicAdd(&lead.cnt[sub], ltotal);
                __syncthreads();
                const uint32_t at = s_part[15] + lbase;
                if (isl && at < lead.cap_sub) {
                    const uint64_t slot = (uint64_t)sub * lead.cap_sub + at;
                    lead.key[slot] = ((unsigned long long)grp << 32) | (unsigned long long)gs;
                    lead.val[slot] = gs + q;
                }
                __syncthreads();
            }
        }
    }
    bad = __syncthreads_or(bad);
    if (bad) {
        if (tid == 0) o.flags[IXF_DEGENERATE] = 1u;
        return false;
    }
    if (tid == 0) {
        o.gend[gs] = gs + m;
        atomicAdd(&o.flags[IXF_NSTREAMED], 1u);
        IxStatSlot *sl = o.stat + (b & (IX_STAT_SLOTS - 1u));
        atomicAdd(&sl->inc, (unsigned long long)m * (unsigned long long)(m - 1u) / 2ull);
        atomicMax(&sl->max_group, m);
        atomicAdd(&sl->groups, 1u);
    }
    return true;
}

template <int LEVEL>
__device__ bool ix_big_walk(const IxGeom &g, const uint64_t *src_w, const uint32_t *src_arr, uint64_t *alt_w, uint32_t *alt_arr, uint32_t gpos,
                            uint32_t count, uint32_t sshift, const uint32_t *cs, uint32_t *cs_next, const IxOut &o, const IxLeaders &lead,
                            unsigned char *lds, uint32_t b, uint32_t tcbase)
{
    uint64_t *s_pk = reinterpret_cast<uint64_t *>(lds + IX4_PK);
    uint16_t *s_jx = reinterpret_cast<uint16_t *>(lds + IX4_JX);
    uint32_t *s_h = reinterpret_cast<uint32_t *>(lds + IX4_H);
    uint32_t *s_mixed = reinterpret_cast<uint32_t *>(lds + IX4_MIX);
    uint32_t *s_part = reinterpret_cast<uint32_t *>(lds + IX4_PART);
    const uint32_t sshift_next = sshift - g.rb >= IX_SUBBITS ? sshift - IX_SUBBITS : g.rb;
    uint32_t sub = 0;
    while (sub < IX_NSUB) {
        const uint32_t a = ix_big_first(cs, sub);
        if (a == count) break;
        uint32_t lo = sub, hi = IX_NSUB;
        if (count - a <= IX_CAP) lo = hi;
        while (hi - lo > 1u) {
            const uint32_t mid = (lo + hi) >> 1;
            if (ix_big_first(cs, mid) - a <= IX_CAP) lo = mid;
            else hi = mid;
        }
        bool ok = true;
        if (lo == sub) {
            const uint32_t m = cs[sub] - a;
            if (ix_big_one_value(g, src_w + a, m)) {
                ok = ix_big_value(g, src_w + a, src_arr + a, o, lead, reinterpret_cast<uint32_t *>(lds + IX4_PK), s_part, b, tcbase, gpos + a, m);
            } else if (LEVEL == 1 && sshift > g.rb) {
                if constexpr (LEVEL == 1) {
                    ix_big_split(src_w + a, src_arr + a, alt_w + a, alt_arr + a, m, sshift_next, cs_next, lds, s_part);
                    ok = ix_big_walk<2>(g, alt_w + a, alt_arr + a, nullptr, nullptr, gpos + a, m, sshift_next, cs_next, nullptr, o, lead, lds, b, tcbase);
                }
            } else {
                if (threadIdx.x == 0) o.flags[IXF_DEGENERATE] = 1u;
                ok = false;
            }
            sub++;
        } else {
            const uint32_t cnt = ix_big_first(cs, lo) - a;
            if (cnt)
                ok = ix_bucket_sort_body<IX_CAP / IX_NT4, true>(g, src_w + a, src_arr + a, tcbase, lo == sub + 1u ? sshift_next : sshift, o.keys_sorted,
                                                                o.sorted_rows, o.gend, o.gs_of, o.tc, o.stat, o.flags, lead, s_pk, s_jx, s_h, s_mixed, s_part,
                                                                b, gpos + a, cnt);
            sub = lo;
        }
        if (!ok) return false;
        __syncthreads();
    }
    return true;
}

__global__ __launch_bounds__(IX_NT4, 2) void ix_big_bucket_kernel(IxGeom g, uint64_t *pk, const uint32_t *start, const uint32_t *biglist,
                                                               uint64_t *keys_sorted, uint32_t *sorted_rows, uint32_t *gend, uint32_t *gs_of, uint2 *tc,
                                                               IxStatSlot *stat, uint32_t *flags, IxLeaders lead)
{
    MG_DYN_SHARED(unsigned char, lds);
    uint32_t *s_part = reinterpret_cast<uint32_t *>(lds + IX4_PART);
    uint32_t *cs1 = reinterpret_cast<uint32_t *>(lds + IXB_CS1), *cs2 = reinterpret_cast<uint32_t *>(lds + IXB_CS2);
    const IxOut o{keys_sorted, sorted_rows, gend, gs_of, tc, stat, flags};
    const uint32_t nbig = flags[IXF_NBIG];
    const uint32_t sshift = ix_subshift(g);
    for (uint32_t i = blockIdx.x; i < nbig; i += gridDim.x) {
        const uint32_t b = biglist[i];
        const uint32_t G0 = start[b], N = start[b + 1] - G0;
        ix_big_split(pk + G0, nullptr, keys_sorted + G0, sorted_rows + G0, N, sshift, cs1, lds, s_part);
        if (!ix_big_walk<1>(g, keys_sorted + G0, sorted_rows + G0, pk + G0, gend + G0, G0, N, sshift, cs1, cs2, o, lead, lds, b, G0)) return;
        __syncthreads();
    }
}

__global__ __launch_bounds__(256) void ix_stat_reduce_kernel(const IxStatSlot *stat, unsigned long long *incidences, uint32_t *max_group, uint32_t *groups)
{
    unsigned long long inc = 0;
    uint32_t m = 0, gr = 0;
    for (uint32_t i = threadIdx.x; i < IX_STAT_SLOTS; i += 256u) {
        inc += stat[i].inc;
        m = stat[i].max_group > m ? stat[i].max_group : m;
        gr += stat[i].groups;
    }
    if (inc) atomicAdd(incidences, inc);
    if (m) atomicMax(max_group, m);
    if (gr) atomicAdd(groups, gr);
}

__global__ __launch_bounds__(256) void ix_fill_u32_kernel(uint32_t *p, uint64_t count, uint32_t v)
{
    const uint64_t stride = (uint64_t)gridDim.x * 256u;
    for (uint64_t i = (uint64_t)blockIdx.x * 256u + threadIdx.x; i < count; i += stride) p[i] = v;
}

__global__ __launch_bounds__(256) void ix_verify_kernel(const uint32_t *a, const uint32_t *b, const uint32_t *cond, uint32_t mode, uint64_t count,
                                                        unsigned long long *out)
{
    const uint64_t stride = (uint64_t)gridDim.x * 256u;
    for (uint64_t i = (uint64_t)blockIdx.x * 256u + threadIdx.x; i < count; i += stride) {
        if (mode == 1u && cond[i] != (uint32_t)i) continue;
        if (mode == 2u && cond[i] == 0xFFFFFFFFu) continue;
        if (a[i] != b[i]) {
            atomicAdd(&out[0], 1ull);
            atomicMin(&out[1], (unsigned long long)i);
        }
    }
}

hipError_t index_verify_words(const uint32_t *a, const uint32_t *b, const uint32_t *cond, uint32_t mode, uint64_t count, unsigned long long *out2,
                              hipStream_t stream)
{
    if (count == 0) return hipSuccess;
    uint64_t blocks = (count + 1023u) / 1024u;
    if (blocks > 8192u) blocks = 8192u;
    hipLaunchKernelGGL(ix_verify_kernel, dim3((uint32_t)blocks), dim3(256), 0, stream, a, b, cond, mode, count, out2);
    return hipGetLastError();
}


size_t index_stat_scratch_bytes() { return sizeof(IxStatSlot) * IX_STAT_SLOTS; }

#if defined(IX_PHASE_CLOCKS) && !defined(MG_HIP_EMU)
void index_dump_clocks()
{
    unsigned long long h[64];
    if (hipMemcpyFromSymbol(h, HIP_SYMBOL(ix_clk), sizeof h) != hipSuccess) return;
    static const char *k3[] = {"prologue (lb, scan, gbase)", "loads + pack", "tile sort", "bucket scan", "pk + slots to LDS", "slot image"};
    static const char *k4[] = {"zero + load", "tickets", "counter scan + ticket read", "scatter", "mixed mark + fix-up + write back", "heads + inverse", "out by position + leaders", "statistics + leaders' scan", "tc by arrival", "leaders out"};
    unsigned long long t3 = 0, t4 = 0;
    for (int i = 0; i < 6; i++) t3 += h[i];
    for (int i = 0; i < 10; i++) t4 += h[32 + i];
    for (int i = 0; i < 6; i++) fprintf(stderr, "ix clocks K3 %-34s %6.2f %%\n", k3[i], 100.0 * h[i] / (t3 ? t3 : 1));
    for (int i = 0; i < 10; i++) fprintf(stderr, "ix clocks K4 %-34s %6.2f %%\n", k4[i], 100.0 * h[32 + i] / (t4 ? t4 : 1));
    memset(h, 0, sizeof h);
    (void)hipMemcpyToSymbol(HIP_SYMBOL(ix_clk), h, sizeof h);
}
#endif

IxPlan index_plan(uint32_t n, uint32_t E, uint32_t s, uint32_t rs, uint64_t stride, uint64_t maxv, double dens0, bool want_gs)
{
    IxPlan p;
    IxGeom &g = p.g;
    g = IxGeom{};
    if (n == 0 || E == 0) { p.why = "empty"; return p; }
    if (s > 65535u) { p.why = "sketch size beyond 16-bit positions"; return p; }
    g.n = n;
    g.E = E;
    g.rs = rs;
    g.stride = stride;
    g.want_gs = want_gs ? 1u : 0u;
    g.nblk = (n + IX_RB - 1u) / IX_RB;
    g.rb = 1;
    while (g.rb < 32u && (1ull << g.rb) < (uint64_t)n) g.rb++;
    if (!(dens0 > 0.0)) { p.why = "no density"; return p; }
    uint32_t shift = 0;
    while (shift < 63u && dens0 * (double)(1ull << (shift + 1u)) <= IX_TMAX) shift++;
    if (shift > 64u - g.rb) shift = 64u - g.rb;
    if (shift > 63u) shift = 63u;
    g.shift = shift;
    const uint64_t B = (maxv >> shift) + 1ull;
    if (B > (1ull << 22)) { p.why = "too many buckets (values far from evenly spread)"; return p; }
    uint32_t bw_log = 0;
    while (bw_log < 9u && (1ull << (bw_log + 1u)) <= IX_BW_MAX && shift + bw_log + 1u <= 63u && (1ull << bw_log) < B &&
           (double)E * (double)(2u << bw_log) / ((double)g.nblk * (double)B) <= IX_TILE_TARGET)
        bw_log++;
    g.bw_log = bw_log;
    g.BW = 1u << bw_log;
    g.NW = (uint32_t)((B + g.BW - 1u) / g.BW);
    g.Bp = g.NW * g.BW;
    g.npass = (bw_log + 3u) / 4u;
    g.wgrp = 8;
    const uint64_t nseq = (uint64_t)((g.NW + g.wgrp - 1u) / g.wgrp) * g.wgrp * g.nblk;
    if (nseq >= (1ull << 30)) { p.why = "too many tiles"; return p; }
    g.nseq = (uint32_t)nseq;
    p.lb_bytes = (size_t)n * (g.NW + 1u) * 2u;
    p.cnt_bytes = (size_t)g.nblk * g.Bp * 4u;
    p.start_bytes = ((size_t)g.Bp + 1u) * 4u;
    p.pk_bytes = (size_t)E * 8u;
    p.tc_bytes = (size_t)E * 8u;
    p.big_bytes = ((size_t)E / IX_CAP + 2u) * 4u;
    if (p.lb_bytes > ((size_t)2 << 30) || p.cnt_bytes > ((size_t)2 << 30)) { p.why = "scratch of the tiles too large"; return p; }
    p.ok = true;
    return p;
}

hipError_t index_gather_rows(const IxPlan &plan, const uint64_t *hashes, const uint32_t *inv, const uint32_t *cnt_table, uint64_t *out, void *lb_v,
                             hipStream_t stream)
{
    if (!plan.ok) return hipErrorInvalidValue;
    hipLaunchKernelGGL(ix_gather_offsets_kernel, dim3(plan.g.n), dim3(256), 0, stream, plan.g, hashes, inv, cnt_table, out, static_cast<uint16_t *>(lb_v));
    return hipGetLastError();
}

__global__ __launch_bounds__(64) void ix_debug_swap_kernel(IxGeom g, uint64_t *pk, const uint32_t *start, uint32_t *done)
{
    if (threadIdx.x != 0) return;
    for (uint32_t b = 0; b < g.Bp; b++) {
        const uint32_t a = start[b], e = start[b + 1];
        if (e - a < 2u || e - a > IX_CAP) continue;
        for (uint32_t j = a; j + 1u < e; j++) {
            if ((pk[j] >> g.rb) == (pk[j + 1] >> g.rb)) {
                const uint64_t t = pk[j];
                pk[j] = pk[j + 1];
                pk[j + 1] = t;
                done[0] = 1u;
                return;
            }
        }
    }
}

hipError_t index_debug_swap(const IxPlan &plan, void *pk_v, const void *start_v, uint32_t *done, hipStream_t stream)
{
    if (!plan.ok) return hipErrorInvalidValue;
    hipLaunchKernelGGL(ix_debug_swap_kernel, dim3(1), dim3(64), 0, stream, plan.g, static_cast<uint64_t *>(pk_v), static_cast<const uint32_t *>(start_v), done);
    return hipGetLastError();
}

hipError_t index_window_offsets(const IxPlan &plan, const uint64_t *hashes, const uint32_t *rowmap, const uint32_t *cnt_table, void *lb_v, hipStream_t stream)
{
    if (!plan.ok) return hipErrorInvalidValue;
    hipLaunchKernelGGL(ix_window_offsets_kernel, dim3((plan.g.n + 3u) / 4u), dim3(256), 0, stream, plan.g, hashes, rowmap, (const uint32_t *)nullptr, cnt_table,
                       static_cast<uint16_t *>(lb_v));
    return hipGetLastError();
}

bool index_offsets_counts_fits(const IxGeom &g) { return ixoc_lds_bytes(g.Bp) <= IXOC_LDS_MAX; }

hipError_t index_offsets_counts(const IxPlan &plan, const uint64_t *hashes, const uint32_t *rowmap, const uint32_t *cnt_table, void *lb_v, void *cnt_v,
                                uint32_t *flags, hipStream_t stream)
{
    if (!plan.ok || !index_offsets_counts_fits(plan.g)) return hipErrorInvalidValue;
    const uint32_t lds = (uint32_t)ixoc_lds_bytes(plan.g.Bp);
    const hipError_t e = hipFuncSetAttribute(reinterpret_cast<const void *>(ix_offsets_counts_kernel), hipFuncAttributeMaxDynamicSharedMemorySize, (int)lds);
    if (e != hipSuccess) return e;
    hipLaunchKernelGGL(ix_offsets_counts_kernel, dim3(plan.g.nblk), dim3(IXOC_NT), lds, stream, plan.g, hashes, rowmap, cnt_table, static_cast<uint16_t *>(lb_v),
                       static_cast<uint32_t *>(cnt_v), flags);
    return hipGetLastError();
}

hipError_t index_build(const IxPlan &plan, const uint64_t *hashes, const uint32_t *off, void *lb_v, void *cnt_v, void *start_v, void *big_v, void *pk_v, void *tc_v,
                       uint64_t *keys_sorted, uint32_t *sorted_rows, uint32_t *gend, uint32_t *gs_of, uint32_t *code_img, uint32_t *pos_img,
                       void *stat_scratch, unsigned long long *incidences, uint32_t *max_group, uint32_t *groups, uint32_t *flags,
                       const IxLeaders *leaders, hipStream_t stream, int stages)
{
    return index_build_mapped(plan, hashes, nullptr, off, lb_v, cnt_v, start_v, big_v, pk_v, tc_v, keys_sorted, sorted_rows, gend, gs_of, code_img, pos_img,
                              stat_scratch, incidences, max_group, groups, flags, leaders, stream, stages);
}

hipError_t index_build_mapped(const IxPlan &plan, const uint64_t *hashes, const uint32_t *rowmap, const uint32_t *off, void *lb_v, void *cnt_v, void *start_v,
                              void *big_v, void *pk_v, void *tc_v, uint64_t *keys_sorted, uint32_t *sorted_rows, uint32_t *gend, uint32_t *gs_of,
                              uint32_t *code_img, uint32_t *pos_img, void *stat_scratch, unsigned long long *incidences, uint32_t *max_group,
                              uint32_t *groups, uint32_t *flags, const IxLeaders *leaders, hipStream_t stream, int stages)
{
    if (!plan.ok) return hipErrorInvalidValue;
    const IxGeom g = plan.g;
    uint16_t *lb = static_cast<uint16_t *>(lb_v);
    uint32_t *cnt = static_cast<uint32_t *>(cnt_v), *start = static_cast<uint32_t *>(start_v);
    uint64_t *pk = static_cast<uint64_t *>(pk_v);
    uint2 *tc = static_cast<uint2 *>(tc_v);
    hipError_t e = hipSuccess;
    if (stages & 1) {
        e = hipFuncSetAttribute(reinterpret_cast<const void *>(ix_tile_partition_kernel), hipFuncAttributeMaxDynamicSharedMemorySize, (int)IXL_BYTES);
        if (e != hipSuccess) return e;
        const uint32_t tiles = 8u * ((g.nseq + 7u) / 8u);
        if (!(stages & (8 | 16))) hipLaunchKernelGGL(ix_window_offsets_kernel, dim3((g.n + 3u) / 4u), dim3(256), 0, stream, g, hashes, rowmap, off,
                                                     (const uint32_t *)nullptr, lb);
        if (!(stages & 16)) hipLaunchKernelGGL(ix_tile_count_kernel, dim3(tiles), dim3(IX_NT), 0, stream, g, hashes, rowmap, (const uint16_t *)lb, cnt);
        hipLaunchKernelGGL(ix_col_scan_kernel, dim3((g.Bp + 255u) / 256u), dim3(256), 0, stream, g, cnt, start);
        hipLaunchKernelGGL(ix_bucket_scan_kernel, dim3(1), dim3(1024), 0, stream, g, start, flags, static_cast<uint32_t *>(big_v));
        e = hipGetLastError();
        if (e != hipSuccess) return e;
        hipLaunchKernelGGL(ix_tile_partition_kernel, dim3(tiles), dim3(IX_NT), IXL_BYTES, stream, g, hashes, rowmap, (const uint16_t *)lb, (const uint32_t *)cnt,
                           (const uint32_t *)start, (const uint32_t *)flags, pk, pos_img);
        e = hipGetLastError();
        if (e != hipSuccess) return e;
    }
    if (stages & 2) {
        e = hipFuncSetAttribute(reinterpret_cast<const void *>(ix_bucket_sort_kernel), hipFuncAttributeMaxDynamicSharedMemorySize, (int)IX4_BYTES);
        if (e == hipSuccess) e = hipFuncSetAttribute(reinterpret_cast<const void *>(ix_big_bucket_kernel), hipFuncAttributeMaxDynamicSharedMemorySize, (int)IXB_BYTES);
        if (e != hipSuccess) return e;
        e = hipMemsetAsync(stat_scratch, 0, index_stat_scratch_bytes(), stream);
        if (e != hipSuccess) return e;
        hipLaunchKernelGGL(ix_bucket_sort_kernel, dim3(g.Bp), dim3(IX_NT4), IX4_BYTES, stream, g, (const uint64_t *)pk, (const uint32_t *)start, keys_sorted,
                           sorted_rows, gend, g.want_gs ? gs_of : (uint32_t *)nullptr, tc, static_cast<IxStatSlot *>(stat_scratch), flags,
                           leaders ? *leaders : IxLeaders());
        hipLaunchKernelGGL(ix_big_bucket_kernel, dim3(256), dim3(IX_NT4), IXB_BYTES, stream, g, pk, (const uint32_t *)start,
                           (const uint32_t *)big_v, keys_sorted, sorted_rows, gend, g.want_gs ? gs_of : (uint32_t *)nullptr, tc,
                           static_cast<IxStatSlot *>(stat_scratch), flags, leaders ? *leaders : IxLeaders());
        hipLaunchKernelGGL(ix_stat_reduce_kernel, dim3(1), dim3(256), 0, stream, static_cast<const IxStatSlot *>(stat_scratch), incidences, max_group, groups);
    }
    if (!(stages & 4)) return hipGetLastError();
    {
        const uint32_t nchunk = (g.rs + IX5_CH - 1u) / IX5_CH;
        const uint32_t pieces = 8u * ((g.nblk * nchunk + 7u) / 8u);
        hipLaunchKernelGGL(ix_images_kernel, dim3(pieces), dim3(256), 0, stream, g, off, (const uint32_t *)flags, (const uint2 *)tc, code_img, pos_img, nchunk);
    }
    return hipGetLastError();
}

}
```

Before: 450.1 billion pairs/s.

## Summarize index rows on device and overlap bulk row copies with planning

Adds a two-kernel device reduction that computes per-row summary statistics (total entries, max count, max last hash, density bins, longest label run, identity/pad flags). The host waits only for this small summary record, so it can plan and start the mapped index build while the bulk row arrays are still copying back. The row arrays are packed into one device allocation so they return in a single copy, and the host loops for longest run and densities move to the GPU. This adds events, a second code path with a host fallback, and a risk of floating-point differences in the density sums.

```diff
diff --git a/mash_amd/csrc/compare_dense.hip b/mash_amd/csrc/compare_dense.hip
--- a/mash_amd/csrc/compare_dense.hip
+++ b/mash_amd/csrc/compare_dense.hip
@@ -741,7 +741,7 @@
         g1 = groups[g].g1;
     }
     grp_of[r] = g;
-    lead_rows[r] = make_uint4(g, g0, g1, 0u);
+    if (lead_rows) lead_rows[r] = make_uint4(g, g0, g1, 0u);
 }
 
 hipError_t launch_dense_group_rows(const DenseGroup *groups, uint32_t ng, uint32_t n, uint32_t *grp_of, uint32_t *lead_rows, hipStream_t stream)
diff --git a/mash_amd/csrc/host_index.cpp b/mash_amd/csrc/host_index.cpp
--- a/mash_amd/csrc/host_index.cpp
+++ b/mash_amd/csrc/host_index.cpp
@@ -10,17 +10,6 @@
 const uint64_t kTilesLongestRun = 6144;
 static const uint64_t kSplitMinRun = 128;
 
-uint64_t longest_label_run(const uint32_t *lab_sorted, uint64_t n)
-{
-    if (!lab_sorted || n == 0) return 0;
-    uint64_t run = 1, longest = 1;
-    for (uint64_t a = 1; a < n; a++) {
-        run = lab_sorted[a] == lab_sorted[a - 1] ? run + 1 : 1;
-        longest = std::max(longest, run);
-    }
-    return longest;
-}
-
 struct Carve {
     unsigned char *base = nullptr;
     size_t at = 0;
@@ -29,6 +18,23 @@
         const size_t from = (at + alignof(T) - 1) & ~(alignof(T) - 1);
         at = from + count * sizeof(T);
         return base ? reinterpret_cast<T *>(base + from) : nullptr;
+    }
+};
+
+struct RowArrays {
+    unsigned long long *last = nullptr;
+    uint32_t *inv = nullptr, *lab = nullptr;
+    uint8_t *cls = nullptr, *link = nullptr;
+    size_t bytes = 0;
+    RowArrays() = default;
+    RowArrays(unsigned char *base, uint64_t n, bool classes, bool cluster, bool links)
+    {
+        Carve c{base};
+        if (classes) last = c.take<unsigned long long>(n);
+        if (cluster) { inv = c.take<uint32_t>(n); lab = c.take<uint32_t>(n); }
+        if (classes) cls = c.take<uint8_t>(n);
+        if (links) link = c.take<uint8_t>(n);
+        bytes = c.at;
     }
 };
 
@@ -70,10 +76,23 @@
     bool stop = false;
 
     bool need_classes = false, dedup = true, want_dense = true, try_cluster = false, try_links = false;
-    DevBuf<uint8_t> dc_cls, d_link;
-    DevBuf<unsigned long long> dc_last, d_dig, d_dig_sorted, k_a, k_b;
-    DevBuf<uint32_t> d_cnt, d_rows_sorted, d_flags, d_nflag, r_a, r_b, l_a, l_b, d_inv, d_lab;
+    DevBuf<unsigned char> d_bulk;
+    uint8_t *dc_cls = nullptr, *d_link = nullptr;
+    unsigned long long *dc_last = nullptr;
+    uint32_t *d_inv = nullptr, *d_lab = nullptr;
+    DevBuf<uint8_t> d_link_own;
+    DevBuf<unsigned long long> d_dig, d_dig_sorted, k_a, k_b;
+    DevBuf<uint32_t> d_cnt, d_rows_sorted, d_flags, d_nflag, r_a, r_b, l_a, l_b;
     DevBuf<unsigned char> d_tmp_dup, d_tmp_cl;
+    bool summary_knob = true;
+    bool two_stage = false;
+    bool sum_dev = false;
+    DevBuf<unsigned char> d_sum;
+    hipEvent_t ev_rec = nullptr, ev_bulk = nullptr;
+    mg::IxRowSummary rec;
+    RowArrays pa;
+    uint32_t *p_nh = nullptr, *p_us = nullptr, *p_ue = nullptr;
+    uint64_t p_groups = 0;
     std::vector<uint8_t> hc_cls, link;
     std::vector<uint64_t> hc_last;
     std::vector<uint32_t> hc_nh, inv_v, lab_v;
@@ -124,10 +143,15 @@
     uint64_t dn_xrows = 0, dn_words = 0;
 
     SparseIndexBuild(mg_ctx *c, const mg_table *tab, uint32_t sketch_size, bool clustered_variant, mg_table::Sparse *index, uint32_t split_row)
-        : ctx(c), t(tab), s(sketch_size), clustered(clustered_variant), split(split_row), sp(index), n(tab->n), dc_cls(c), d_link(c), dc_last(c), d_dig(c), d_dig_sorted(c),
-          k_a(c), k_b(c), d_cnt(c), d_rows_sorted(c), d_flags(c), d_nflag(c), r_a(c), r_b(c), l_a(c), l_b(c), d_inv(c), d_lab(c), d_tmp_dup(c), d_tmp_cl(c), d_lb(c), d_tcnt(c),
+        : ctx(c), t(tab), s(sketch_size), clustered(clustered_variant), split(split_row), sp(index), n(tab->n), d_bulk(c), d_link_own(c), d_dig(c), d_dig_sorted(c),
+          k_a(c), k_b(c), d_cnt(c), d_rows_sorted(c), d_flags(c), d_nflag(c), r_a(c), r_b(c), l_a(c), l_b(c), d_tmp_dup(c), d_tmp_cl(c), d_sum(c), d_lb(c), d_tcnt(c),
           d_groups(c), d_grp_of(c), d_lead_rows(c), lead(c), temp(c), gs_of(c), key64_a(c), key64_b(c), d_stat(c), d_slots(c)
     {}
+    ~SparseIndexBuild()
+    {
+        if (ev_rec) (void)hipEventDestroy(ev_rec);
+        if (ev_bulk) (void)hipEventDestroy(ev_bulk);
+    }
 
     int unusable(const char *why) { sp->usable = false; sp->why = why; stop = true; return MG_OK; }
 
@@ -202,6 +226,8 @@
     }
 
     int scan_rows();
+    int rows_arrived();
+    int map_rows(uint64_t run);
     int copy_rows();
     int order_rows();
     int find_copies();
@@ -212,8 +238,9 @@
     int build_by_sort();
     int check_build();
     bool search_leaders();
-    bool sort_universes(std::vector<uint32_t> &us, std::vector<uint32_t> &ue);
-    bool choose_groups(const std::vector<uint32_t> &us, const std::vector<uint32_t> &ue);
+    bool sort_universes(uint32_t *us, uint32_t *ue);
+    bool choose_groups(const uint32_t *us, const uint32_t *ue);
+    void rows_of_groups();
     int encode_groups();
     int dense_groups();
     int run();
@@ -229,7 +256,18 @@
     try_links = !try_cluster && want_dense && n >= 8 && s <= 16384;
     tb_dup = mg::sparse_dup_temp_bytes((uint32_t)n);
     tb_cl = mg::dense_cluster_temp_bytes((uint32_t)n);
-    if (d_cnt.alloc(n) != hipSuccess || (need_classes && (dc_cls.alloc(n) != hipSuccess || dc_last.alloc(n) != hipSuccess)) ||
+    if (const char *v = ctx_opt(ctx, "MASHGPU_IX_SUMMARY")) summary_knob = strcmp(v, "host") != 0;
+    bool room_cl = try_cluster, room_lk = try_links;
+    RowArrays da(nullptr, n, need_classes, room_cl, room_lk);
+    if (d_bulk.alloc(std::max<size_t>(da.bytes, 16)) != hipSuccess) {
+        (void)hipGetLastError();
+        room_cl = room_lk = false;
+        da = RowArrays(nullptr, n, need_classes, false, false);
+        if (d_bulk.alloc(std::max<size_t>(da.bytes, 16)) != hipSuccess) { (void)hipGetLastError(); return unusable("no device memory for the index"); }
+    }
+    da = RowArrays(d_bulk.p, n, need_classes, room_cl, room_lk);
+    dc_last = da.last; dc_cls = da.cls; d_inv = da.inv; d_lab = da.lab; d_link = da.link;
+    if (d_cnt.alloc(n) != hipSuccess ||
         (dedup && (d_dig.alloc(n) != hipSuccess || d_dig_sorted.alloc(n) != hipSuccess || d_rows_sorted.alloc(n) != hipSuccess ||
                    d_flags.alloc(n) != hipSuccess || d_nflag.alloc(1) != hipSuccess || d_tmp_dup.alloc(std::max<size_t>(tb_dup, 16)) != hipSuccess))) {
         (void)hipGetLastError();
@@ -249,73 +287,101 @@
             if (e == hipSuccess)
                 e = mg::launch_sparse_dup_suspects(d_dig, d_cnt, (uint32_t)n, d_tmp_dup, tb_dup, d_dig_sorted, d_rows_sorted, d_flags, d_nflag, ctx->stream);
         }
-        if (e == hipSuccess && try_cluster) {
+        if (e == hipSuccess && room_cl) {
             if (k_a.alloc(4 * n) == hipSuccess && k_b.alloc(4 * n) == hipSuccess && r_a.alloc(4 * n) == hipSuccess && r_b.alloc(4 * n) == hipSuccess &&
-                l_a.alloc(n) == hipSuccess && l_b.alloc(n) == hipSuccess && d_inv.alloc(n) == hipSuccess && d_lab.alloc(n) == hipSuccess &&
-                d_tmp_cl.alloc(std::max<size_t>(tb_cl, 16)) == hipSuccess) {
+                l_a.alloc(n) == hipSuccess && l_b.alloc(n) == hipSuccess && d_tmp_cl.alloc(std::max<size_t>(tb_cl, 16)) == hipSuccess) {
                 e = mg::dense_cluster_rows(t->hashes, t->s, d_cnt, (uint32_t)n, d_tmp_cl, tb_cl, k_a, k_b, r_a, r_b, l_a, l_b, d_inv, d_lab, ctx->stream, split);
                 cluster_q = true;
             } else {
                 (void)hipGetLastError();
             }
         }
-        if (e == hipSuccess && try_links) {
-            if (d_link.alloc(n) == hipSuccess) {
-                link.resize(n);
-                e = mg::launch_dense_neighbors(t->hashes, t->s, d_cnt, (uint32_t)n, d_link, ctx->stream);
-                links_q = true;
-            } else {
-                (void)hipGetLastError();
-            }
-        }
-        unsigned long long *p_last = nullptr;
-        uint32_t *p_nh = nullptr, *p_inv = nullptr, *p_lab = nullptr, *p_nflag = nullptr;
-        uint8_t *p_cls = nullptr, *p_link = nullptr;
+        if (e == hipSuccess && room_lk) {
+            link.resize(n);
+            e = mg::launch_dense_neighbors(t->hashes, t->s, d_cnt, (uint32_t)n, d_link, ctx->stream);
+            links_q = true;
+        }
+        uint32_t *p_nflag = nullptr;
+        mg::IxRowSummary *p_rec = nullptr;
+        unsigned char *p_bulk = nullptr;
+        p_groups = n / 8 + 1;
         auto carve = [&](unsigned char *block) {
             Carve c{block};
-            p_last = c.take<unsigned long long>(n); p_nh = c.take<uint32_t>(n); p_inv = c.take<uint32_t>(n); p_lab = c.take<uint32_t>(n);
-            p_nflag = c.take<uint32_t>(2); p_cls = c.take<uint8_t>(n); p_link = c.take<uint8_t>(n);
+            p_rec = c.take<mg::IxRowSummary>(1);
+            p_bulk = reinterpret_cast<unsigned char *>(c.take<unsigned long long>(da.bytes / 8 + 1));
+            p_nh = c.take<uint32_t>(n); p_nflag = c.take<uint32_t>(2); p_us = c.take<uint32_t>(p_groups); p_ue = c.take<uint32_t>(p_groups);
             return c.at + 64;
         };
         unsigned char *pin = static_cast<unsigned char *>(ctx_pinned(ctx, carve(nullptr)));
         if (pin) {
             carve(pin);
+            pa = RowArrays(p_bulk, n, need_classes, room_cl, room_lk);
         } else {
             p_nflag = &nflag;
-            if (cluster_q) { inv_v.resize(n); lab_v.resize(n); p_inv = inv_v.data(); p_lab = lab_v.data(); }
-            p_nh = hc_nh.data(); p_cls = hc_cls.data(); p_last = reinterpret_cast<unsigned long long *>(hc_last.data()); p_link = link.data();
-        }
+            p_groups = 0;
+            if (cluster_q) { inv_v.resize(n); lab_v.resize(n); pa.inv = inv_v.data(); pa.lab = lab_v.data(); }
+            p_nh = hc_nh.data(); pa.cls = hc_cls.data(); pa.last = reinterpret_cast<unsigned long long *>(hc_last.data()); pa.link = link.data();
+        }
+        if (e == hipSuccess && pin && summary_knob && d_sum.alloc(1024 + mg::index_row_summary_scratch_bytes((uint32_t)n)) == hipSuccess &&
+            hipEventCreateWithFlags(&ev_rec, hipEventDisableTiming) == hipSuccess && hipEventCreateWithFlags(&ev_bulk, hipEventDisableTiming) == hipSuccess) {
+            mg::IxRowSummary *d_rec = reinterpret_cast<mg::IxRowSummary *>(d_sum.p);
+            e = mg::index_row_summary(d_cnt, need_classes ? dc_last : nullptr, t->hashes, t->nhash, t->s, cluster_q ? d_inv : nullptr, cluster_q ? d_lab : nullptr,
+                                      dedup ? d_nflag.p : nullptr, (uint32_t)n, d_sum.p + 1024, d_rec, ctx->stream);
+            if (e == hipSuccess) e = hipMemcpyAsync(p_rec, d_rec, sizeof(mg::IxRowSummary), hipMemcpyDeviceToHost, ctx->stream);
+            if (e == hipSuccess) e = hipEventRecord(ev_rec, ctx->stream);
+            if (e == hipSuccess && da.bytes) e = hipMemcpyAsync(p_bulk, d_bulk, da.bytes, hipMemcpyDeviceToHost, ctx->stream);
+            if (e == hipSuccess && need_classes) e = hipMemcpyAsync(p_nh, t->nhash, n * 4, hipMemcpyDeviceToHost, ctx->stream);
+            if (e == hipSuccess) e = hipEventRecord(ev_bulk, ctx->stream);
+            const hipError_t ew = e == hipSuccess ? hipEventSynchronize(ev_rec) : hipStreamSynchronize(ctx->stream);
+            if (e == hipSuccess) e = ew;
+            if (e != hipSuccess) return fail(ctx, MG_ERR_HIP, std::string("compare (index: rows, copies, order): ") + hipGetErrorString(e));
+            rec = *p_rec;
+            nflag = rec.suspects;
+            gate_suspects = nflag;
+            two_stage = true;
+            if (cluster_q) { inv = pa.inv; lab_sorted = pa.lab; }
+            return MG_OK;
+        }
+        (void)hipGetLastError();
         if (e == hipSuccess && need_classes) {
             e = hipMemcpyAsync(p_nh, t->nhash, n * 4, hipMemcpyDeviceToHost, ctx->stream);
-            if (e == hipSuccess) e = hipMemcpyAsync(p_cls, dc_cls, n, hipMemcpyDeviceToHost, ctx->stream);
-            if (e == hipSuccess) e = hipMemcpyAsync(p_last, dc_last, n * 8, hipMemcpyDeviceToHost, ctx->stream);
+            if (e == hipSuccess) e = hipMemcpyAsync(pa.cls, dc_cls, n, hipMemcpyDeviceToHost, ctx->stream);
+            if (e == hipSuccess) e = hipMemcpyAsync(pa.last, dc_last, n * 8, hipMemcpyDeviceToHost, ctx->stream);
         }
         if (e == hipSuccess && dedup) e = hipMemcpyAsync(p_nflag, d_nflag, 4, hipMemcpyDeviceToHost, ctx->stream);
         if (e == hipSuccess && cluster_q) {
-            e = hipMemcpyAsync(p_inv, d_inv, n * 4, hipMemcpyDeviceToHost, ctx->stream);
-            if (e == hipSuccess) e = hipMemcpyAsync(p_lab, d_lab, n * 4, hipMemcpyDeviceToHost, ctx->stream);
-        }
-        if (e == hipSuccess && links_q) e = hipMemcpyAsync(p_link, d_link, n, hipMemcpyDeviceToHost, ctx->stream);
+            e = hipMemcpyAsync(pa.inv, d_inv, n * 4, hipMemcpyDeviceToHost, ctx->stream);
+            if (e == hipSuccess) e = hipMemcpyAsync(pa.lab, d_lab, n * 4, hipMemcpyDeviceToHost, ctx->stream);
+        }
+        if (e == hipSuccess && links_q) e = hipMemcpyAsync(pa.link, d_link, n, hipMemcpyDeviceToHost, ctx->stream);
         const hipError_t es = hipStreamSynchronize(ctx->stream);
         if (e == hipSuccess) e = es;
-        if (e == hipSuccess && pin) {
-            if (need_classes) {
-                memcpy(hc_nh.data(), p_nh, n * 4);
-                memcpy(hc_cls.data(), p_cls, n);
-                memcpy(hc_last.data(), p_last, n * 8);
-            }
-            if (dedup) nflag = *p_nflag;
-            if (links_q) memcpy(link.data(), p_link, n);
-        }
-        if (cluster_q) { inv = p_inv; lab_sorted = p_lab; }
         if (e != hipSuccess) return fail(ctx, MG_ERR_HIP, std::string("compare (index: rows, copies, order): ") + hipGetErrorString(e));
+        if (dedup) nflag = *p_nflag;
+        if (cluster_q) { inv = pa.inv; lab_sorted = pa.lab; }
+        if (!pin) pa = RowArrays();
     }
     gate_suspects = nflag;
+    return rows_arrived();
+}
+
+int SparseIndexBuild::rows_arrived()
+{
+    if (two_stage) {
+        two_stage = false;
+        HIP_TRY(ctx, hipEventSynchronize(ev_bulk));
+    }
     if (need_classes) {
+        if (pa.cls) {
+            memcpy(hc_nh.data(), p_nh, n * 4);
+            memcpy(hc_cls.data(), pa.cls, n);
+            memcpy(hc_last.data(), pa.last, n * 8);
+        }
         t->cls.swap(hc_cls);
         t->last.swap(hc_last);
         t->nh.swap(hc_nh);
     }
+    if (links_q && pa.link) memcpy(link.data(), pa.link, n);
     if (!links_q) link.clear();
     return MG_OK;
 }
@@ -325,65 +391,57 @@
     ix_mode = ctx_opt(ctx, "MASHGPU_SPARSE_INDEX");
     ix_verify = ix_mode && strcmp(ix_mode, "verify") == 0;
     ix_tiles = !ix_mode || strcmp(ix_mode, "sort") != 0;
+    H = t->hashes;
+    auto keeps_table_order = [&](uint64_t run) {
+        return cluster_q && split != 0 && !ctx_opt(ctx, "MASHGPU_SPLIT_ALWAYS") && run * (uint64_t)s < kSplitMinRun * 1000ull;
+    };
+    bool mapped = false;
+    if (two_stage) {
+        const uint64_t run = cluster_q ? rec.label_run : 0;
+        if (cluster_q && !rec.inv_identity && !rec.pad_hit && !keeps_table_order(run) && ix_tiles && !(dedup && nflag) && rec.E_all > 0 &&
+            rec.E_all < (1ull << 31) && run <= kTilesLongestRun &&
+            mg::index_plan((uint32_t)n, (uint32_t)rec.E_all, s, sp->rs, t->s, rec.maxv, rec.dens0, ix_verify).ok) {
+            sum_dev = true;
+            E_all = rec.E_all; max_cnt = rec.max_cnt; maxv = rec.maxv; dens0 = rec.dens0;
+            memcpy(dens, rec.dens, sizeof dens);
+            const int rc = map_rows(run);
+            if (rc != MG_OK) return rc;
+            mapped = true;
+        }
+        const int rc = rows_arrived();
+        if (rc != MG_OK) return rc;
+    }
     cnt_true.assign(n, 0);
-    for (uint64_t i = 0; i < n; i++) {
-        const uint32_t c = (uint32_t)std::min<uint64_t>(std::min<uint64_t>(t->nh[i], t->s), s);
-        cnt_true[i] = c;
-        E_all += c;
-        max_cnt = std::max(max_cnt, c);
-        if (c) {
-            const uint64_t last = t->last[i];
-            if (last == MG_HASH_PAD) return unusable("a hash equals the padding value");
-            maxv = std::max(maxv, last);
-            const double d = (double)c / ((double)last + 1.0);
-            dens[64 - __builtin_clzll(last | 1ull)] += d;
-            dens0 += d;
-        }
-    }
-    H = t->hashes;
+    const uint64_t cap = std::min<uint64_t>(t->s, s);
+    if (sum_dev) {
+        for (uint64_t i = 0; i < n; i++) cnt_true[i] = (uint32_t)std::min<uint64_t>(t->nh[i], cap);
+    } else {
+        mg::IxRowSummary hs;
+        mg::index_row_summary_host(t->nh.data(), cap, t->last.data(), nullptr, nullptr, n, cnt_true.data(), &hs);
+        if (hs.pad_hit) return unusable("a hash equals the padding value");
+        E_all = hs.E_all; max_cnt = hs.max_cnt; maxv = hs.maxv; dens0 = hs.dens0;
+        memcpy(dens, hs.dens, sizeof dens);
+    }
+    const uint64_t run = !cluster_q ? 0 : sum_dev ? rec.label_run : mg::index_longest_run(lab_sorted, n);
     bool keep_table_order = false;
-    const uint64_t run = cluster_q ? longest_label_run(lab_sorted, n) : 0;
-    if (cluster_q && split != 0 && lab_sorted && !ctx_opt(ctx, "MASHGPU_SPLIT_ALWAYS") && run * (uint64_t)s < kSplitMinRun * 1000ull) {
+    if (lab_sorted && keeps_table_order(run)) {
         keep_table_order = true;
         lab_sorted = nullptr;
     }
     if (cluster_q) {
-        bool identity = true;
-        for (uint64_t a = 0; a < n && identity; a++) identity = inv[a] == a;
-        if (!identity && !keep_table_order) {
-            const char *fc = ctx_opt(ctx, "MASHGPU_COMPARE_ROWCOPY");
-            const bool copy_now = fc && atoi(fc) != 0;
-            void *pi = nullptr, *ph = nullptr;
-            if (ctx_malloc(ctx, &pi, n * 4) != hipSuccess || (copy_now && ctx_malloc(ctx, &ph, std::max<uint64_t>(n * t->s, 1) * 8) != hipSuccess)) {
-                (void)hipGetLastError();
-                ctx_free(ctx, pi);
-                lab_sorted = nullptr;
-            } else {
-                sp->inv = static_cast<uint32_t *>(pi);
-                sp->phashes = static_cast<uint64_t *>(ph);
-                HIP_TRY(ctx, hipMemcpyAsync(sp->inv, d_inv, n * 4, hipMemcpyDeviceToDevice, ctx->stream));
-                if (ix_tiles && !(dedup && nflag) && E_all > 0 && E_all < (1ull << 31) && run <= kTilesLongestRun) {
-                    early_plan = mg::index_plan((uint32_t)n, (uint32_t)E_all, s, sp->rs, t->s, maxv, dens0, ix_verify);
-                    if (early_plan.ok && d_lb.alloc(early_plan.lb_bytes) == hipSuccess) {
-                        if (copy_now) HIP_TRY(ctx, mg::index_gather_rows(early_plan, t->hashes, sp->inv, d_cnt, sp->phashes, d_lb, ctx->stream));
-                        else if (counts_with_offsets()) HIP_TRY(ctx, mg::index_offsets_counts(early_plan, t->hashes, sp->inv, d_cnt, d_lb, d_tcnt, d_stat.p->ixf, ctx->stream));
-                        else HIP_TRY(ctx, mg::index_window_offsets(early_plan, t->hashes, sp->inv, d_cnt, d_lb, ctx->stream));
-                        lb_made = true;
-                    } else {
-                        (void)hipGetLastError();
-                    }
-                }
-                if (copy_now) {
-                    if (!lb_made) HIP_TRY(ctx, mg::launch_dense_gather_rows(t->hashes, t->s, sp->inv, (uint32_t)n, sp->phashes, ctx->stream));
-                    H = sp->phashes;
-                } else {
-                    rowmap = sp->inv;
-                }
-                cnt_perm.resize(n);
-                for (uint64_t a = 0; a < n; a++) cnt_perm[a] = cnt_true[inv[a]];
-                cnt_true.swap(cnt_perm);
-                cnt_stale = true;
+        if (!mapped) {
+            bool identity = true;
+            for (uint64_t a = 0; a < n && identity; a++) identity = inv[a] == a;
+            if (!identity && !keep_table_order) {
+                const int rc = map_rows(run);
+                if (rc != MG_OK) return rc;
             }
+        }
+        if (sp->inv) {
+            cnt_perm.resize(n);
+            for (uint64_t a = 0; a < n; a++) cnt_perm[a] = cnt_true[inv[a]];
+            cnt_true.swap(cnt_perm);
+            cnt_stale = true;
         }
     } else {
         lab_sorted = nullptr;
@@ -392,7 +450,8 @@
     if (want_dense && n >= 8 && s <= 16384 && lab_sorted) {
         link.assign(n, 0);
         for (uint64_t a = 1; a < n; a++) link[a] = (a != split && lab_sorted[a] == lab_sorted[a - 1] && cnt_true[a] && cnt_true[a - 1]) ? 1 : 0;
-    } else if (cluster_q && want_dense && n >= 8 && s <= 16384 && d_link.alloc(n) == hipSuccess) {
+    } else if (cluster_q && want_dense && n >= 8 && s <= 16384 && d_link_own.alloc(n) == hipSuccess) {
+        d_link = d_link_own;
         const int rc = copy_rows();
         if (rc != MG_OK || stop) return rc;
         link.resize(n);
@@ -403,6 +462,44 @@
     } else if (!links_q) {
         (void)hipGetLastError();
         link.clear();
+    }
+    if (ctx_opt(ctx, "MASHGPU_SPARSE_DBG"))
+        fprintf(stderr, "compare sparse: rows summed by the %s (%llu entries, fullest row %u, longest label run %llu)\n",
+                sum_dev ? "device: the plan from its record, the host's passes behind K0" : "host's loop", (unsigned long long)E_all, max_cnt,
+                (unsigned long long)label_run);
+    return MG_OK;
+}
+
+int SparseIndexBuild::map_rows(uint64_t run)
+{
+    const char *fc = ctx_opt(ctx, "MASHGPU_COMPARE_ROWCOPY");
+    const bool copy_now = fc && atoi(fc) != 0;
+    void *pi = nullptr, *ph = nullptr;
+    if (ctx_malloc(ctx, &pi, n * 4) != hipSuccess || (copy_now && ctx_malloc(ctx, &ph, std::max<uint64_t>(n * t->s, 1) * 8) != hipSuccess)) {
+        (void)hipGetLastError();
+        ctx_free(ctx, pi);
+        lab_sorted = nullptr;
+        return MG_OK;
+    }
+    sp->inv = static_cast<uint32_t *>(pi);
+    sp->phashes = static_cast<uint64_t *>(ph);
+    HIP_TRY(ctx, hipMemcpyAsync(sp->inv, d_inv, n * 4, hipMemcpyDeviceToDevice, ctx->stream));
+    if (ix_tiles && !(dedup && nflag) && E_all > 0 && E_all < (1ull << 31) && run <= kTilesLongestRun) {
+        early_plan = mg::index_plan((uint32_t)n, (uint32_t)E_all, s, sp->rs, t->s, maxv, dens0, ix_verify);
+        if (early_plan.ok && d_lb.alloc(early_plan.lb_bytes) == hipSuccess) {
+            if (copy_now) HIP_TRY(ctx, mg::index_gather_rows(early_plan, t->hashes, sp->inv, d_cnt, sp->phashes, d_lb, ctx->stream));
+            else if (counts_with_offsets()) HIP_TRY(ctx, mg::index_offsets_counts(early_plan, t->hashes, sp->inv, d_cnt, d_lb, d_tcnt, d_stat.p->ixf, ctx->stream));
+            else HIP_TRY(ctx, mg::index_window_offsets(early_plan, t->hashes, sp->inv, d_cnt, d_lb, ctx->stream));
+            lb_made = true;
+        } else {
+            (void)hipGetLastError();
+        }
+    }
+    if (copy_now) {
+        if (!lb_made) HIP_TRY(ctx, mg::launch_dense_gather_rows(t->hashes, t->s, sp->inv, (uint32_t)n, sp->phashes, ctx->stream));
+        H = sp->phashes;
+    } else {
+        rowmap = sp->inv;
     }
     return MG_OK;
 }
@@ -723,7 +820,7 @@
     }
 }
 
-bool SparseIndexBuild::sort_universes(std::vector<uint32_t> &us, std::vector<uint32_t> &ue)
+bool SparseIndexBuild::sort_universes(uint32_t *us, uint32_t *ue)
 {
     const uint32_t ng = (uint32_t)cand_groups.size(), nlead = lead.tot[0];
     uint32_t gbits = 1;
@@ -737,16 +834,15 @@
     hipError_t e = hipMemsetAsync(d_us, 0, ng * 4, ctx->stream);
     if (e == hipSuccess) e = hipMemsetAsync(d_ue, 0, ng * 4, ctx->stream);
     if (e == hipSuccess) e = mg::dense_sort_universes(lead.keyj, lead.valj, nlead, d_utmp, tb, d_key2, sp->ulist, sp->upos, d_us, d_ue, gbits, ctx->stream);
-    if (e == hipSuccess) e = hipMemcpyAsync(us.data(), d_us, ng * 4, hipMemcpyDeviceToHost, ctx->stream);
-    if (e == hipSuccess) e = hipMemcpyAsync(ue.data(), d_ue, ng * 4, hipMemcpyDeviceToHost, ctx->stream);
+    if (e == hipSuccess) e = hipMemcpyAsync(us, d_us, ng * 4, hipMemcpyDeviceToHost, ctx->stream);
+    if (e == hipSuccess) e = hipMemcpyAsync(ue, d_ue, ng * 4, hipMemcpyDeviceToHost, ctx->stream);
     if (e == hipSuccess) e = hipStreamSynchronize(ctx->stream);
     return e == hipSuccess;
 }
 
-bool SparseIndexBuild::choose_groups(const std::vector<uint32_t> &us, const std::vector<uint32_t> &ue)
+bool SparseIndexBuild::choose_groups(const uint32_t *us, const uint32_t *ue)
 {
     const uint32_t kMaxWords = mg::dense_max_words();
-    std::fill(grp_of_h.begin(), grp_of_h.end(), 0xFFFFFFFFu);
     for (uint32_t g = 0; g < (uint32_t)cand_groups.size(); g++) {
         mg::DenseGroup G = cand_groups[g];
         G.u = ue[g] > us[g] ? ue[g] - us[g] : 0u;
@@ -759,10 +855,16 @@
         dn_xrows += m;
         dn_words += ((m + 127) / 128) * mg::dense_block_words(G.W);
         sp->dn_wmax = std::max(sp->dn_wmax, G.W);
-        for (uint32_t r = G.g0; r < G.g1; r++) grp_of_h[r] = (uint32_t)sp->dgroups_host.size();
         sp->dgroups_host.push_back(G);
     }
     return !sp->dgroups_host.empty();
+}
+
+void SparseIndexBuild::rows_of_groups()
+{
+    std::fill(grp_of_h.begin(), grp_of_h.end(), 0xFFFFFFFFu);
+    for (uint32_t g = 0; g < (uint32_t)sp->dgroups_host.size(); g++)
+        for (uint32_t r = sp->dgroups_host[g].g0; r < sp->dgroups_host[g].g1; r++) grp_of_h[r] = g;
 }
 
 int SparseIndexBuild::encode_groups()
@@ -774,10 +876,16 @@
         return MG_OK;
     }
     hipError_t e = hipMemcpyAsync(sp->dgroups, sp->dgroups_host.data(), sp->dgroups_host.size() * sizeof(mg::DenseGroup), hipMemcpyHostToDevice, ctx->stream);
-    if (e == hipSuccess) e = hipMemcpyAsync(sp->grp_of, grp_of_h.data(), n * 4, hipMemcpyHostToDevice, ctx->stream);
+    if (!summary_knob) {
+        rows_of_groups();
+        if (e == hipSuccess) e = hipMemcpyAsync(sp->grp_of, grp_of_h.data(), n * 4, hipMemcpyHostToDevice, ctx->stream);
+    } else if (e == hipSuccess) {
+        e = mg::launch_dense_group_rows(sp->dgroups, (uint32_t)sp->dgroups_host.size(), (uint32_t)n, sp->grp_of, nullptr, ctx->stream);
+    }
     if (e == hipSuccess)
         e = mg::launch_dense_encode(sp->off, sp->code_img, sp->pos_img, sp->rs, sp->grp_of, sp->dgroups, sp->ulist, sp->upos, sp->gdata, sp->ext, sp->dn_xs,
                                     (uint32_t)n, sp->dn_wmax, ctx->stream, ctx_opt(ctx, "MASHGPU_DENSE_UL_LDS") ? atoi(ctx_opt(ctx, "MASHGPU_DENSE_UL_LDS")) : -1);
+    if (summary_knob) rows_of_groups();
     sp->grp_of_host.swap(grp_of_h);
     if (e != hipSuccess) {
         drop();
@@ -789,13 +897,20 @@
     return MG_OK;
 }
 
+
 int SparseIndexBuild::dense_groups()
 {
     if (!cand_groups.empty()) {
         auto t_dense = std::chrono::steady_clock::now();
         if (built && lead_ready && lead.overflowed() && ctx_opt(ctx, "MASHGPU_SPARSE_DBG"))
             fprintf(stderr, "compare dense: a list of leaders asked for %u entries, room for %u: no dense groups for this table\n", lead.tot[1], lead.cap);
-        std::vector<uint32_t> us(cand_groups.size(), 0), ue(cand_groups.size(), 0);
+        std::vector<uint32_t> us_v, ue_v;
+        uint32_t *us = p_us, *ue = p_ue;
+        if (!summary_knob || !us || !ue || cand_groups.size() > p_groups) {
+            us_v.assign(cand_groups.size(), 0);
+            ue_v.assign(cand_groups.size(), 0);
+            us = us_v.data(); ue = ue_v.data();
+        }
         const int rc = [&] {
             if (!lead_ready || (!built && !search_leaders())) return (int)MG_OK;
             if (lead.tot[0] == 0 || lead.overflowed()) return (int)MG_OK;
diff --git a/mash_amd/csrc/index_build.h b/mash_amd/csrc/index_build.h
--- a/mash_amd/csrc/index_build.h
+++ b/mash_amd/csrc/index_build.h
@@ -51,6 +51,25 @@
                                 uint32_t *flags, hipStream_t stream);
 hipError_t index_gather_rows(const IxPlan &plan, const uint64_t *hashes, const uint32_t *inv, const uint32_t *cnt_table, uint64_t *out, void *lb,
                              hipStream_t stream);
+struct IxRowSummary {
+    unsigned long long E_all;
+    unsigned long long maxv;
+    unsigned long long label_run;
+    uint32_t max_cnt;
+    uint32_t pad_hit;
+    uint32_t inv_identity;
+    uint32_t suspects;
+    double dens0;
+    double dens[65];
+};
+static_assert(sizeof(IxRowSummary) <= 1024, "the record is read back in one small copy");
+void index_row_summary_host(const uint32_t *nh, uint64_t cap, const uint64_t *last, const uint32_t *inv, const uint32_t *lab, uint64_t n, uint32_t *cnt_out,
+                            IxRowSummary *out);
+uint64_t index_longest_run(const uint32_t *lab, uint64_t n);
+size_t index_row_summary_scratch_bytes(uint32_t n);
+hipError_t index_row_summary(const uint32_t *cnt, const unsigned long long *last, const uint64_t *hashes, const uint32_t *nhash, uint64_t stride,
+                             const uint32_t *inv, const uint32_t *lab, const uint32_t *nflag, uint32_t n, void *scratch, IxRowSummary *out, hipStream_t stream);
+
 
 hipError_t index_verify_words(const uint32_t *a, const uint32_t *b, const uint32_t *cond, uint32_t mode, uint64_t count, unsigned long long *out2,
                               hipStream_t stream);
diff --git a/mash_amd/csrc/index_build.hip b/mash_amd/csrc/index_build.hip
--- a/mash_amd/csrc/index_build.hip
+++ b/mash_amd/csrc/index_build.hip
@@ -1194,6 +1194,226 @@
     return hipGetLastError();
 }
 
+constexpr uint32_t IXS_NT = 256;
+constexpr uint32_t IXS_PIECES = 512;
+constexpr uint32_t IXS_STRANDS = 15;
+constexpr uint32_t IXS_COLS = 66;
+constexpr uint32_t IXS_NT2 = 1024;
+constexpr uint64_t IXS_PAD = 0xFFFFFFFFFFFFFFFFull;
+static_assert(IXS_STRANDS * IXS_COLS <= IXS_NT2 && IXS_PIECES <= IXS_NT2 && IXS_NT2 % 64u == 0, "a work-item per strand and column, and per piece");
+
+struct IxSumPart {
+    unsigned long long E, maxv;
+    uint32_t max_cnt, pad_hit, not_identity, any_start, head, tail, inner, rows;
+    double col[IXS_COLS];
+};
+
+__device__ __forceinline__ uint32_t ixs_bit_length(uint64_t v) { return 64u - (uint32_t)__builtin_clzll(v | 1ull); }
+
+__global__ __launch_bounds__(IXS_NT) void ix_row_summary_kernel(const uint32_t *__restrict__ cnt, const unsigned long long *__restrict__ last,
+                                                                const uint64_t *__restrict__ H, const uint32_t *__restrict__ nhash, uint64_t stride,
+                                                                const uint32_t *__restrict__ inv, const uint32_t *__restrict__ lab, uint32_t n, uint32_t piece,
+                                                                IxSumPart *part)
+{
+    __shared__ double s_d[IXS_NT];
+    __shared__ uint32_t s_bin[IXS_NT];
+    __shared__ uint32_t s_lab[IXS_NT + 1];
+    __shared__ uint32_t s_first, s_last, s_inner, s_maxcnt, s_pad, s_notid;
+    __shared__ unsigned long long s_E, s_maxv;
+    const uint32_t tid = threadIdx.x;
+    const uint64_t p0 = (uint64_t)blockIdx.x * piece;
+    const uint64_t p1 = p0 + piece < (uint64_t)n ? p0 + piece : (uint64_t)n;
+    if (tid == 0) { s_maxcnt = 0; s_pad = 0; s_notid = 0; s_E = 0; s_maxv = 0; }
+    uint32_t any_start = 0, head = 0, carry = 0, inner = 0;
+    double col = 0.0;
+    unsigned long long my_E = 0, my_maxv = 0;
+    uint32_t my_maxcnt = 0, my_pad = 0, my_notid = 0;
+    for (uint64_t t0 = p0; t0 < p1; t0 += IXS_NT) {
+        const uint32_t len = (uint32_t)(p1 - t0 < IXS_NT ? p1 - t0 : IXS_NT);
+        const uint64_t a = t0 + tid;
+        if (tid == 0) { s_first = 0xFFFFFFFFu; s_last = 0; s_inner = 0; }
+        double d = 0.0;
+        uint32_t bin = 0xFFFFFFFFu;
+        if (tid < len) {
+            const uint32_t c = cnt[a];
+            my_E += c;
+            my_maxcnt = c > my_maxcnt ? c : my_maxcnt;
+            if (c) {
+                unsigned long long lv;
+                if (last) {
+                    lv = last[a];
+                } else {
+                    uint64_t k = nhash[a];
+                    if (k > stride) k = stride;
+                    lv = H[a * stride + k - 1u];
+                }
+                if (lv == IXS_PAD) my_pad = 1u;
+                my_maxv = lv > my_maxv ? lv : my_maxv;
+                d = (double)c / ((double)lv + 1.0);
+                bin = ixs_bit_length(lv);
+            }
+            if (inv && inv[a] != (uint32_t)a) my_notid = 1u;
+            if (lab) s_lab[tid] = lab[a];
+        }
+        s_d[tid] = d;
+        s_bin[tid] = bin;
+        __syncthreads();
+        if (lab && tid < len) {
+            const uint32_t mine = s_lab[tid];
+            const bool start = a == 0 || (tid ? s_lab[tid - 1u] : lab[a - 1u]) != mine;
+            if (start) {
+                uint32_t j = tid + 1u;
+                while (j < len && s_lab[j] == mine) j++;
+                atomicMin(&s_first, tid);
+                if (j < len) atomicMax(&s_inner, j - tid);
+                else atomicMax(&s_last, tid + 1u);
+            }
+        }
+        if (tid < IXS_COLS) {
+#pragma unroll 16
+            for (uint32_t j = 0; j < IXS_NT; j++) col += (tid == 65u || s_bin[j] == tid) ? s_d[j] : 0.0;
+        }
+        __syncthreads();
+        if (lab && tid == 0) {
+            if (s_first == 0xFFFFFFFFu) {
+                if (any_start) carry += len;
+                else head += len;
+            } else {
+                if (any_start) inner = carry + s_first > inner ? carry + s_first : inner;
+                else { head += s_first; any_start = 1u; }
+                inner = s_inner > inner ? s_inner : inner;
+                carry = len - (s_last - 1u);
+            }
+        }
+        __syncthreads();
+    }
+    if (my_E) atomicAdd(&s_E, my_E);
+    if (my_maxv) atomicMax(&s_maxv, my_maxv);
+    if (my_maxcnt) atomicMax(&s_maxcnt, my_maxcnt);
+    if (my_pad) atomicOr(&s_pad, 1u);
+    if (my_notid) atomicOr(&s_notid, 1u);
+    __syncthreads();
+    IxSumPart *o = part + blockIdx.x;
+    if (tid < IXS_COLS) o->col[tid] = col;
+    if (tid == 0) {
+        o->E = s_E; o->maxv = s_maxv; o->max_cnt = s_maxcnt; o->pad_hit = s_pad; o->not_identity = s_notid;
+        o->any_start = any_start; o->head = head; o->tail = carry; o->inner = inner; o->rows = (uint32_t)(p1 - p0);
+    }
+}
+
+__global__ __launch_bounds__(IXS_NT2) void ix_row_summary_final_kernel(const IxSumPart *__restrict__ part, uint32_t np, uint32_t has_inv, uint32_t has_lab,
+                                                                       const uint32_t *__restrict__ nflag, IxRowSummary *out)
+{
+    __shared__ double s_col[IXS_STRANDS * IXS_COLS];
+    __shared__ uint4 s_run[IXS_PIECES];
+    __shared__ unsigned long long s_E, s_maxv;
+    __shared__ uint32_t s_maxcnt, s_flags;
+    const uint32_t tid = threadIdx.x;
+    const uint32_t per = (np + IXS_STRANDS - 1u) / IXS_STRANDS;
+    if (tid == 0) { s_E = 0; s_maxv = 0; s_maxcnt = 0; s_flags = 0; }
+    __syncthreads();
+    if (tid < np) {
+        const IxSumPart &p = part[tid];
+        s_run[tid] = make_uint4((p.any_start ? 1u : 0u) | (p.rows << 1), p.head, p.tail, p.inner);
+        if (p.E) atomicAdd(&s_E, p.E);
+        if (p.maxv) atomicMax(&s_maxv, p.maxv);
+        if (p.max_cnt) atomicMax(&s_maxcnt, p.max_cnt);
+        if (p.pad_hit | p.not_identity) atomicOr(&s_flags, (p.pad_hit ? 1u : 0u) | (p.not_identity ? 2u : 0u));
+    }
+    if (tid < IXS_STRANDS * IXS_COLS) {
+        const uint32_t strand = tid / IXS_COLS, k = tid % IXS_COLS;
+        const uint32_t b0 = strand * per < np ? strand * per : np, b1 = b0 + per < np ? b0 + per : np;
+        double sum = 0.0;
+#pragma unroll 8
+        for (uint32_t b = b0; b < b1; b++) sum += part[b].col[k];
+        s_col[tid] = sum;
+    }
+    __syncthreads();
+    if (tid < IXS_COLS) {
+        double sum = 0.0;
+        for (uint32_t strand = 0; strand < IXS_STRANDS; strand++) sum += s_col[strand * IXS_COLS + tid];
+        if (tid < 65u) out->dens[tid] = sum;
+        else out->dens0 = sum;
+    } else if (tid == 128u) {
+        unsigned long long carry = 0, longest = 0;
+        uint32_t any = 0;
+        for (uint32_t b = 0; b < np; b++) {
+            const uint4 r = s_run[b];
+            if (!(r.x & 1u)) {
+                carry += r.x >> 1;
+            } else {
+                if (any) longest = carry + r.y > longest ? carry + r.y : longest;
+                any = 1u;
+                longest = r.w > longest ? r.w : longest;
+                carry = r.z;
+            }
+        }
+        longest = carry > longest ? carry : longest;
+        out->E_all = s_E;
+        out->maxv = s_maxv;
+        out->label_run = has_lab ? longest : 0ull;
+        out->max_cnt = s_maxcnt;
+        out->pad_hit = s_flags & 1u;
+        out->inv_identity = has_inv ? ((s_flags & 2u) ? 0u : 1u) : 1u;
+        out->suspects = nflag ? nflag[0] : 0u;
+    }
+}
+
+
+static uint32_t ixs_piece_rows(uint32_t n)
+{
+    const uint32_t tiles = (n + IXS_NT - 1u) / IXS_NT;
+    return ((tiles + IXS_PIECES - 1u) / IXS_PIECES) * IXS_NT;
+}
+
+size_t index_row_summary_scratch_bytes(uint32_t n) { return sizeof(IxSumPart) * (n ? (n + ixs_piece_rows(n) - 1u) / ixs_piece_rows(n) : 1u); }
+
+hipError_t index_row_summary(const uint32_t *cnt, const unsigned long long *last, const uint64_t *hashes, const uint32_t *nhash, uint64_t stride,
+                             const uint32_t *inv, const uint32_t *lab, const uint32_t *nflag, uint32_t n, void *scratch, IxRowSummary *out, hipStream_t stream)
+{
+    if (n == 0 || !cnt || !(last || (hashes && nhash)) || !scratch || !out) return hipErrorInvalidValue;
+    const uint32_t piece = ixs_piece_rows(n), np = (n + piece - 1u) / piece;
+    hipLaunchKernelGGL(ix_row_summary_kernel, dim3(np), dim3(IXS_NT), 0, stream, cnt, last, hashes, nhash, stride, inv, lab, n, piece, static_cast<IxSumPart *>(scratch));
+    hipLaunchKernelGGL(ix_row_summary_final_kernel, dim3(1), dim3(IXS_NT2), 0, stream, static_cast<const IxSumPart *>(scratch), np, inv ? 1u : 0u, lab ? 1u : 0u, nflag,
+                       out);
+    return hipGetLastError();
+}
+
+uint64_t index_longest_run(const uint32_t *lab, uint64_t n)
+{
+    if (!lab || n == 0) return 0;
+    uint64_t run = 1, longest = 1;
+    for (uint64_t a = 1; a < n; a++) {
+        run = lab[a] == lab[a - 1] ? run + 1 : 1;
+        longest = run > longest ? run : longest;
+    }
+    return longest;
+}
+
+void index_row_summary_host(const uint32_t *nh, uint64_t cap, const uint64_t *last, const uint32_t *inv, const uint32_t *lab, uint64_t n, uint32_t *cnt_out,
+                            IxRowSummary *out)
+{
+    IxRowSummary r;
+    memset(&r, 0, sizeof r);
+    for (uint64_t i = 0; i < n; i++) {
+        const uint32_t c = (uint32_t)((uint64_t)nh[i] < cap ? (uint64_t)nh[i] : cap);
+        if (cnt_out) cnt_out[i] = c;
+        r.E_all += c;
+        r.max_cnt = c > r.max_cnt ? c : r.max_cnt;
+        if (c) {
+            const uint64_t lv = last[i];
+            if (lv == IXS_PAD) r.pad_hit = 1u;
+            r.maxv = lv > r.maxv ? lv : r.maxv;
+            const double d = (double)c / ((double)lv + 1.0);
+            r.dens[64 - __builtin_clzll(lv | 1ull)] += d;
+            r.dens0 += d;
+        }
+    }
+    r.inv_identity = 1u;
+    for (uint64_t a = 0; inv && a < n && r.inv_identity; a++) r.inv_identity = inv[a] == a ? 1u : 0u;
+    r.label_run = index_longest_run(lab, n);
+    *out = r;
+}
 
 size_t index_stat_scratch_bytes() { return sizeof(IxStatSlot) * IX_STAT_SLOTS; }
 
```

New measurement: 450.8 billion pairs/s, median of 4. Within noise of the previous version (+0.1%).
